# piljoong-jeong/nerf_meets_mlx

Measured on AMD Instinct MI355X. Metric: train+render rays/sec on Lego 800x800 (synthetic), coarse+fine 64+128, higher is better.
Workload: dtype split16 (fp16x2 render / bf16x2 train MFMA operands ~ 22 / 16 significand bits; fp32 accumulate)

## Files before the change

### include/nerf_hip.h

```cpp
#ifndef NERF_HIP_H
#define NERF_HIP_H

#include <stddef.h>
#include <stdint.h>

#ifdef __cplusplus
extern "C" {
#endif

#define NERF_ABI_VERSION 3

#define NERF_OK 0
#define NERF_E_NULL (-1)
#define NERF_E_SHAPE (-2)
#define NERF_E_UNSUPPORTED (-3)
#define NERF_E_HIP (-4)
#define NERF_E_RCCL (-5)

int nerf_abi_version(void);
const char* nerf_last_error(void);

#define NERF_RAY_STRIDE 11

int nerf_pixel_permutation(int64_t* out_idx, int64_t n, int64_t domain, uint64_t seed, uint64_t offset,
// ... 26 lines not shown

int nerf_encode_freq(const float* x, int64_t M, int D, int n_freqs, int freq_mode, float* out, void* stream);

int nerf_encode_sinusoidal(const float* x, int64_t M, int D, int n_freqs, const float* freqs_host,
                           int include_input, float* out, void* stream);

int nerf_sh_encode(const float* dirs, int64_t M, int degree, float* out, void* stream);

int nerf_hashgrid_forward(const float* x, int64_t M, const float* tables, int L, int log2_T, int F,
                          const int* resolutions_host, float* out, void* stream);
int nerf_hashgrid_backward(const float* x, int64_t M, const float* d_out, int L, int log2_T, int F,
                           const int* resolutions_host, float* d_tables, void* stream);

int nerf_ngp_encode(const float* rays, const float* z, int64_t B, int n, const float* tables, int L, int log2_T,
                    int F, const int* resolutions_host, int sh_degree, float pos_scale, float pos_offset, float* x_out,
                    float* pts_out, void* stream);
int nerf_hashgrid_backward_rays(const float* rays, const float* z, int64_t B, int n, const float* d_out, int L,
                                int log2_T, int F, const int* resolutions_host, float pos_scale, float pos_offset,
                                float* d_tables, void* stream);

int nerf_hashgrid_backward_ex(const float* x, int64_t M, const float* d_out, int L, int log2_T, int F,
                              const int* resolutions_host, int level_lo, int level_hi, int fixed_point, void* d_tables,
                              void* stream);
int nerf_hashgrid_backward_rays_ex(const float* rays, const float* z, int64_t B, int n, const float* d_out, int L,
                                   int log2_T, int F, const int* resolutions_host, float pos_scale, float pos_offset,
                                   int level_lo, int level_hi, int fixed_point, void* d_tables, void* stream);

int nerf_hashgrid_forward_lw(const float* x, int64_t M, const float* tables, int L, int log2_T, int F,
                             const int* resolutions_host, const float* level_weights_host, float* out, void* stream);
int nerf_ngp_encode_lw(const float* rays, const float* z, int64_t B, int n, const float* tables, int L, int log2_T,
                       int F, const int* resolutions_host, const float* level_weights_host, int sh_degree,
                       float pos_scale, float pos_offset, float* x_out, float* pts_out, void* stream);
int nerf_hashgrid_backward_ex_lw(const float* x, int64_t M, const float* d_out, int L, int log2_T, int F,
                                 const int* resolutions_host, const float* level_weights_host, int level_lo,
                                 int level_hi, int fixed_point, void* d_tables, void* stream);
int nerf_hashgrid_backward_rays_ex_lw(const float* rays, const float* z, int64_t B, int n, const float* d_out, int L,
                                      int log2_T, int F, const int* resolutions_host, const float* level_weights_host,
                                      float pos_scale, float pos_offset, int level_lo, int level_hi, int fixed_point,
                                      void* d_tables, void* stream);

int nerf_composite_forward(const float* raw, const float* z, const float* rays, int64_t B, int n,
                           float raw_noise_std, const float* noise, int white_bkgd, float* rgb, float* disp,
                           float* acc, float* weights, float* depth, void* stream);

int nerf_composite_backward(const float* raw, const float* z, const float* rays, int64_t B, int n,
                            float raw_noise_std, const float* noise, int white_bkgd, const float* d_rgb,
                            const float* d_acc, const float* d_depth, float* d_raw, void* stream);

int nerf_mse_loss_grad(const float* pred, const float* target, int64_t count, float grad_scale, float* loss_out,
                       float* d_pred, void* stream);

int nerf_composite_mse_backward(const float* raw, const float* z, const float* rays, int64_t B, int n, int white_bkgd,
                                const float* target, float grad_scale, float* loss_out, float* rgb, float* d_raw,
                                void* stream);

int nerf_ssim_sums(const float* pred, const float* gt, int N, int C, int H, int W, const float* window_host,
                   int w_size, float c1, float c2, double* sums, void* stream);

typedef struct nerf_mlp_arch {
  int n_layers;
  int width;
  int in_pos;
  int in_dir;
  int skip_layer;
  int use_viewdirs;
  int out_ch;
  int precision;
} nerf_mlp_arch;

int64_t nerf_mlp_param_count(const nerf_mlp_arch* arch);
int64_t nerf_mlp_packed_bytes(const nerf_mlp_arch* arch);
int nerf_mlp_pack(const nerf_mlp_arch* arch, const float* params, void* packed, void* stream);

int64_t nerf_mlp_acts_bytes(const nerf_mlp_arch* arch, int64_t M);
int64_t nerf_mlp_dz_bytes(const nerf_mlp_arch* arch, int64_t M);

int nerf_mlp_forward(const nerf_mlp_arch* arch, const void* packed, const float* x, int64_t M, float* out,
                     void* stream);
int nerf_mlp_forward_train(const nerf_mlp_arch* arch, const void* packed, const float* x, int64_t M, float* out,
                           void* acts, void* stream);

int nerf_query_fused(const nerf_mlp_arch* arch, const void* packed, const float* rays, const float* z, int64_t B,
                     int n, int freq_mode, float* raw, void* acts, void* stream);

int nerf_mlp_backward(const nerf_mlp_arch* arch, const void* packed, const void* acts, const float* d_raw,
                      int64_t M, void* dz, float* grads, void* stream);
int nerf_mlp_backward_inputs(const nerf_mlp_arch* arch, const void* packed, const void* acts, const float* d_raw,
                             int64_t M, void* dz, float* grads, float* d_x, void* stream);

int nerf_mlp_debug_width(const nerf_mlp_arch* arch, int kind, int layer);
int nerf_mlp_debug_read(const nerf_mlp_arch* arch, const void* store, int kind, int layer, int64_t M, float* out,
                        void* stream);

int nerf_ngp_query_fused(const nerf_mlp_arch* arch, const void* packed, const float* rays, const float* z, int64_t B,
                         int n, const float* tables, int L, int log2_T, int F, const int* resolutions_host,
                         int sh_degree, float pos_scale, float pos_offset, float* raw, void* acts, void* stream);
int nerf_ngp_query_fused_h(const nerf_mlp_arch* arch, const void* packed, const float* rays, const float* z, int64_t B,
                           int n, const float* tables, const void* tables_half, int L, int log2_T, int F,
                           const int* resolutions_host, int sh_degree, float pos_scale, float pos_offset, float* raw,
                           void* acts, void* stream);
int nerf_ngp_query_fused_lw(const nerf_mlp_arch* arch, const void* packed, const float* rays, const float* z, int64_t B,
                            int n, const float* tables, const void* tables_half, int L, int log2_T, int F,
                            const int* resolutions_host, const float* level_weights_host, int sh_degree, float pos_scale,
                            float pos_offset, float* raw, void* acts, void* stream);


int nerf_occ_points(int log2_res, int64_t cell0, int64_t count, uint64_t seed, uint64_t update, float pos_scale,
                    float pos_offset, float* rays_out, float* z_out, void* stream);
int nerf_occ_merge(float* density, const float* raw, int64_t count, float decay, void* stream);
int64_t nerf_occ_finalize_workspace_bytes(int log2_res);
int nerf_occ_finalize(const float* density, int log2_res, float thr_cap, void* workspace, float* thr_out, uint32_t* bits,
                      void* stream);
int64_t nerf_occ_cull_workspace_bytes(int64_t B, int n);
int nerf_occ_cull(const float* rays, const float* z, int64_t B, int n, const uint32_t* bits, int log2_res, float pos_scale,
                  float pos_offset, void* workspace, int64_t* idx_out, int64_t* count_out, float* rays_out, float* z_out,
                  float* raw_fill, void* stream);
int nerf_scatter_rows(const float* src, const int64_t* idx, int64_t n, int channels, float* dst, int64_t n_dst, void* stream);

#define NERF_MARCH_MAX_STEPS 1024
int64_t nerf_occ_march_workspace_bytes(int64_t B);
int nerf_occ_march_count(const float* rays, int64_t B, const float* jitter, float jitter_const, const uint32_t* bits, int log2_res,
                         float pos_scale, float pos_offset, float step_world, int march_steps, void* workspace, int64_t* offsets,
                         void* stream);
int nerf_occ_march_write(const float* rays, int64_t B, const float* jitter, float jitter_const, const uint32_t* bits, int log2_res,
                         float pos_scale, float pos_offset, float step_world, int march_steps, void* workspace, int64_t* offsets,
                         float* rows_out, float* z_out, void* stream);
#define NERF_OCC_RELU 0
#define NERF_OCC_EXP 1
int nerf_occ_merge_ex(float* density, const float* raw, int64_t count, float decay, int activation, void* stream);

int nerf_composite_packed_forward(const float* raw, const float* z, const int64_t* offsets, int64_t B, int64_t K, float step_world,
                                  int white_bkgd, float* rgb, float* acc, float* depth, void* stream);
int nerf_composite_packed_mse_backward(const float* raw, const int64_t* offsets, int64_t B, int64_t K, float step_world,
                                       int white_bkgd, const float* target, float grad_scale, float* loss_out, float* rgb,
                                       float* d_raw, void* stream);

int nerf_composite_packed_distortion(const float* raw, const float* z, const int64_t* offsets, const float* rays, int64_t B,
                                     int64_t K, float step_world, int march_steps, int white_bkgd, float* rgb, float* acc,
                                     float* depth, float* dist, void* stream);
int nerf_composite_packed_mse_dist_backward(const float* raw, const float* z, const int64_t* offsets, const float* rays, int64_t B,
                                            int64_t K, float step_world, int march_steps, int white_bkgd, const float* target,
                                            float grad_scale, float dist_weight, float* loss_out, float* dist_out, float* rgb,
                                            float* d_raw, void* stream);

int nerf_composite_packed_forward_bg(const float* raw, const float* z, const int64_t* offsets, int64_t B, int64_t K, float step_world,
                                     const float* bg, int bg_stride, float* rgb, float* acc, float* depth, void* stream);
int nerf_composite_packed_distortion_bg(const float* raw, const float* z, const int64_t* offsets, const float* rays, int64_t B,
                                        int64_t K, float step_world, int march_steps, const float* bg, int bg_stride, float* rgb,
                                        float* acc, float* depth, float* dist, void* stream);
int nerf_composite_packed_mse_backward_bg(const float* raw, const int64_t* offsets, int64_t B, int64_t K, float step_world,
                                          const float* target_rgba, const float* bg, float grad_scale, float* loss_out, float* rgb,
                                          float* d_raw, void* stream);
int nerf_composite_packed_mse_dist_backward_bg(const float* raw, const float* z, const int64_t* offsets, const float* rays, int64_t B,
                                               int64_t K, float step_world, int march_steps, const float* target_rgba,
                                               const float* bg, float grad_scale, float dist_weight, float* loss_out,
                                               float* dist_out, float* rgb, float* d_raw, void* stream);

#define NERF_ERT_TERMINATED 1
int64_t nerf_ert_march_workspace_bytes(int64_t B);
int nerf_ert_init(int64_t B, int32_t* istate, float* fstate, int32_t* live, void* stream);
int nerf_ert_march_count(const float* rays, int64_t B, const float* jitter, float jitter_const, const uint32_t* bits, int log2_res,
                         float pos_scale, float pos_offset, float step_world, int march_steps, const int32_t* live, int64_t A,
                         const int32_t* istate, int max_new, void* workspace, int64_t* totals, void* stream);
int nerf_ert_march_write(const float* rays, int64_t B, const float* jitter, float jitter_const, const uint32_t* bits, int log2_res,
                         float pos_scale, float pos_offset, float step_world, int march_steps, const int32_t* live, int64_t A,
                         int32_t* istate, int max_new, void* workspace, int64_t* offsets, int32_t* live_out, float* rows_out,
                         float* z_out, void* stream);
int nerf_ert_fold(const float* raw, const float* z, const int64_t* offsets, const int32_t* live, int64_t A, int64_t B, int64_t K,
                  float step_world, float min_transmittance, int32_t* istate, float* fstate, void* stream);
int nerf_ert_finish(const int32_t* istate, const float* fstate, int64_t B, int white_bkgd, float* rgb, float* acc, float* depth,
                    int32_t* samples, void* stream);
int nerf_ert_finish_bg(const int32_t* istate, const float* fstate, int64_t B, const float* bg, int bg_stride, float* rgb, float* acc,
                       float* depth, int32_t* samples, void* stream);

#define NERF_MESH_MAX_RES 512
int64_t nerf_mesh_workspace_bytes(int res);
int nerf_mesh_points(int res, const float* lo_host, const float* hi_host, int64_t p0, int64_t count, float* rays_out, float* z_out,
                     void* stream);
int nerf_mesh_count(const float* vol, int res, float iso, void* workspace, int64_t* totals, void* stream);
int nerf_mesh_write_vertices(const float* vol, int res, float iso, const float* lo_host, const float* hi_host, void* workspace,
                             int64_t V, float* verts, float* normals, float* color_rows, void* stream);
int nerf_mesh_write_faces(const float* vol, int res, float iso, void* workspace, int64_t F, int32_t* faces, void* stream);

int64_t nerf_ccl_workspace_bytes(int res);
int nerf_ccl_label(const float* vol, int res, float iso, void* workspace, int32_t* labels, void* stream);
int nerf_ccl_sizes(const int32_t* labels, int res, int32_t* sizes, int64_t* stats, void* stream);
int nerf_ccl_filter(const float* vol, const int32_t* labels, const int32_t* sizes, const int64_t* stats, int res, float iso,
                    int64_t min_voxels, int largest_only, float* out, void* stream);

#define NERF_MORPH_MAX_RADIUS 16
int64_t nerf_morph_workspace_bytes(int res);
int nerf_morph_erode(const float* vol, int res, float iso, int radius, void* workspace, float* core, int64_t* stats2, void* stream);
int nerf_morph_reconstruct(const float* vol, const float* kept, int res, float iso, int radius, void* workspace, float* out,
                           int64_t* stats2, void* stream);

#define NERF_TSDF_MAX_VIEWS 16
typedef struct nerf_tsdf_view {
  float c2w[12];
  float fx, fy, cx, cy;
} nerf_tsdf_view;
int nerf_tsdf_reset(float* D, float* Wt, uint8_t* flags, int res, void* stream);
int nerf_tsdf_integrate(float* D, float* Wt, uint8_t* flags, int res, const float* lo_host, const float* hi_host,
                        const nerf_tsdf_view* views_host, int n, int H, int W, const float* depth, const float* acc, float trunc,
                        float acc_min, float far, int carve, void* stream);
int nerf_tsdf_volume(const float* D, const float* Wt, const uint8_t* flags, int res, int min_views, float* vol_out, void* stream);

int64_t nerf_render_workspace_bytes(int64_t B, int n, int N);
int nerf_render_rays_fused(const nerf_mlp_arch* arch, const void* packed_coarse, const void* packed_fine,
                           const float* rays, int64_t B, int n, int N, const float* u, int freq_mode, int white_bkgd,
                           void* workspace, float* rgb, float* disp, float* acc, float* rgb_coarse, float* disp_coarse,
                           float* acc_coarse, float* z_vals, float* weights, void* stream);

#define NERF_COMM_ID_BYTES 128
int nerf_comm_unique_id(char* id_out_host);
int nerf_comm_init(void** comm_out, int nranks, int rank, const char* id_host);
int nerf_allreduce_grads(void* comm, float* grads, int64_t count, void* stream);
int nerf_comm_destroy(void* comm);

#define NERF_OPTION_UNKNOWN (-2147483647 - 1)
int nerf_set_option(const char* key, int value);
int nerf_get_option(const char* key);

int nerf_adam_step(float* params, const float* grads, float* m, float* v, int64_t count, float lr, float beta1,
                   float beta2, float eps, int bias_correction, int step, float grad_scale, void* stream);
int nerf_adam_step_ex(float* params, void* grads, float* m, float* v, int64_t count, float lr, float beta1, float beta2,
                      float eps, int bias_correction, int step, float grad_scale, int grads_fixed_point, int zero_grads,
                      void* stream);
int nerf_adam_step_shadow(float* params, void* grads, float* m, float* v, int64_t count, float lr, float beta1, float beta2,
                          float eps, int bias_correction, int step, float grad_scale, int grads_fixed_point, int zero_grads,
                          void* params_half, void* stream);

#ifdef __cplusplus
}
#endif
#endif
```

### nerf_meets_mlx_amd/_native.py

```python
import ctypes as C
import os

import torch

_HERE = os.path.dirname(os.path.abspath(__file__))
LIB_PATH = os.environ.get("NERF_HIP_LIB", os.path.join(_HERE, "libnerf_hip.so"))

_P, _I64, _I, _F, _U64 = C.c_void_p, C.c_int64, C.c_int, C.c_float, C.c_uint64
SIGNATURES = {
    "nerf_abi_version": (_I, []),
    "nerf_last_error": (C.c_char_p, []),
    "nerf_pixel_permutation": (_I, [_P, _I64, _I64, _U64, _U64, _P]),
    "nerf_ray_gen": (_I, [_P, _I64, _I, _I, C.POINTER(C.c_double), C.POINTER(C.c_float), _F, _F, _P, _P, _P]),
    "nerf_sample_batch": (_I, [_I64, _I, _I, _U64, _U64, C.POINTER(C.c_double), C.POINTER(C.c_float), _F, _F, _P, _P, _P, _P, _P]),
    "nerf_sample_batch_rgba": (_I, [_I64, _I, _I, _U64, _U64, C.POINTER(C.c_double), C.POINTER(C.c_float), _F, _F, _P, _P, _P, _P, _P]),
    "nerf_gather_rows": (_I, [_P, _I64, _P, _I64, _I, _P, _P]),
    "nerf_ndc_rays": (_I, [_P, _I64, _I, _I, _F, _F, _P]),
    "nerf_sample_coarse": (_I, [_P, _I64, _I, _I, _F, _P, _P, _P]),
    "nerf_add_noise_z": (_I, [_P, _P, _I64, _I, _F, _P, _P]),
    "nerf_importance_sample": (_I, [_P, _P, _P, _I64, _I, _I, _F, _P, _P, _P, _P, _P]),
    "nerf_encode_freq": (_I, [_P, _I64, _I, _I, _I, _P, _P]),
    "nerf_encode_sinusoidal": (_I, [_P, _I64, _I, _I, C.POINTER(C.c_float), _I, _P, _P]),
    "nerf_sh_encode": (_I, [_P, _I64, _I, _P, _P]),
    "nerf_hashgrid_forward": (_I, [_P, _I64, _P, _I, _I, _I, C.POINTER(C.c_int), _P, _P]),
    "nerf_hashgrid_backward": (_I, [_P, _I64, _P, _I, _I, _I, C.POINTER(C.c_int), _P, _P]),
    "nerf_ngp_encode": (_I, [_P, _P, _I64, _I, _P, _I, _I, _I, C.POINTER(C.c_int), _I, C.c_float, C.c_float, _P, _P, _P]),
    "nerf_ngp_query_fused": (_I, [_P, _P, _P, _P, _I64, _I, _P, _I, _I, _I, C.POINTER(C.c_int), _I, C.c_float, C.c_float, _P, _P, _P]),
    "nerf_ngp_query_fused_h": (_I, [_P, _P, _P, _P, _I64, _I, _P, _P, _I, _I, _I, C.POINTER(C.c_int), _I, C.c_float, C.c_float, _P, _P, _P]),
    "nerf_hashgrid_backward_rays": (_I, [_P, _P, _I64, _I, _P, _I, _I, _I, C.POINTER(C.c_int), C.c_float, C.c_float, _P, _P]),
    "nerf_hashgrid_backward_ex": (_I, [_P, _I64, _P, _I, _I, _I, C.POINTER(C.c_int), _I, _I, _I, _P, _P]),
    "nerf_hashgrid_backward_rays_ex": (_I, [_P, _P, _I64, _I, _P, _I, _I, _I, C.POINTER(C.c_int), C.c_float, C.c_float, _I, _I, _I, _P, _P]),
    "nerf_hashgrid_forward_lw": (_I, [_P, _I64, _P, _I, _I, _I, C.POINTER(C.c_int), C.POINTER(C.c_float), _P, _P]),
    "nerf_ngp_encode_lw": (_I, [_P, _P, _I64, _I, _P, _I, _I, _I, C.POINTER(C.c_int), C.POINTER(C.c_float), _I, C.c_float, C.c_float, _P, _P, _P]),
    "nerf_ngp_query_fused_lw": (_I, [_P, _P, _P, _P, _I64, _I, _P, _P, _I, _I, _I, C.POINTER(C.c_int), C.POINTER(C.c_float), _I, C.c_float, C.c_float, _P, _P, _P]),
    "nerf_hashgrid_backward_ex_lw": (_I, [_P, _I64, _P, _I, _I, _I, C.POINTER(C.c_int), C.POINTER(C.c_float), _I, _I, _I, _P, _P]),
    "nerf_hashgrid_backward_rays_ex_lw": (_I, [_P, _P, _I64, _I, _P, _I, _I, _I, C.POINTER(C.c_int), C.POINTER(C.c_float), C.c_float, C.c_float, _I, _I, _I, _P, _P]),
    "nerf_composite_forward": (_I, [_P, _P, _P, _I64, _I, _F, _P, _I, _P, _P, _P, _P, _P, _P]),
    "nerf_composite_backward": (_I, [_P, _P, _P, _I64, _I, _F, _P, _I, _P, _P, _P, _P, _P]),
    "nerf_mse_loss_grad": (_I, [_P, _P, _I64, _F, _P, _P, _P]),
    "nerf_composite_mse_backward": (_I, [_P, _P, _P, _I64, _I, _I, _P, _F, _P, _P, _P, _P]),
    "nerf_ssim_sums": (_I, [_P, _P, _I, _I, _I, _I, C.POINTER(C.c_float), _I, _F, _F, _P, _P]),
    "nerf_mlp_param_count": (_I64, [_P]),
    "nerf_mlp_packed_bytes": (_I64, [_P]),
    "nerf_mlp_pack": (_I, [_P, _P, _P, _P]),
    "nerf_mlp_acts_bytes": (_I64, [_P, _I64]),
    "nerf_mlp_dz_bytes": (_I64, [_P, _I64]),
    "nerf_mlp_forward": (_I, [_P, _P, _P, _I64, _P, _P]),
    "nerf_mlp_forward_train": (_I, [_P, _P, _P, _I64, _P, _P, _P]),
    "nerf_query_fused": (_I, [_P, _P, _P, _P, _I64, _I, _I, _P, _P, _P]),
    "nerf_mlp_backward": (_I, [_P, _P, _P, _P, _I64, _P, _P, _P]),
    "nerf_mlp_backward_inputs": (_I, [_P, _P, _P, _P, _I64, _P, _P, _P, _P]),
    "nerf_mlp_debug_width": (_I, [_P, _I, _I]),
    "nerf_mlp_debug_read": (_I, [_P, _P, _I, _I, _I64, _P, _P]),
    "nerf_render_workspace_bytes": (_I64, [_I64, _I, _I]),
    "nerf_render_rays_fused": (_I, [_P, _P, _P, _P, _I64, _I, _I, _P, _I, _I, _P, _P, _P, _P, _P, _P, _P, _P, _P, _P]),
    "nerf_comm_unique_id": (_I, [C.c_char_p]),
    "nerf_comm_init": (_I, [C.POINTER(C.c_void_p), _I, _I, C.c_char_p]),
    "nerf_allreduce_grads": (_I, [_P, _P, _I64, _P]),
    "nerf_comm_destroy": (_I, [_P]),
    "nerf_set_option": (_I, [C.c_char_p, _I]),
    "nerf_get_option": (_I, [C.c_char_p]),
    "nerf_adam_step": (_I, [_P, _P, _P, _P, _I64, _F, _F, _F, _F, _I, _I, _F, _P]),
    "nerf_adam_step_ex": (_I, [_P, _P, _P, _P, _I64, _F, _F, _F, _F, _I, _I, _F, _I, _I, _P]),
    "nerf_adam_step_shadow": (_I, [_P, _P, _P, _P, _I64, _F, _F, _F, _F, _I, _I, _F, _I, _I, _P, _P]),
    "nerf_occ_points": (_I, [_I, _I64, _I64, _U64, _U64, _F, _F, _P, _P, _P]),
    "nerf_occ_merge": (_I, [_P, _P, _I64, _F, _P]),
    "nerf_occ_finalize_workspace_bytes": (_I64, [_I]),
    "nerf_occ_finalize": (_I, [_P, _I, _F, _P, _P, _P, _P]),
    "nerf_occ_cull_workspace_bytes": (_I64, [_I64, _I]),
    "nerf_occ_cull": (_I, [_P, _P, _I64, _I, _P, _I, _F, _F, _P, _P, _P, _P, _P, _P, _P]),
    "nerf_scatter_rows": (_I, [_P, _P, _I64, _I, _P, _I64, _P]),
    "nerf_occ_merge_ex": (_I, [_P, _P, _I64, _F, _I, _P]),
    "nerf_occ_march_workspace_bytes": (_I64, [_I64]),
    "nerf_occ_march_count": (_I, [_P, _I64, _P, _F, _P, _I, _F, _F, _F, _I, _P, _P, _P]),
    "nerf_occ_march_write": (_I, [_P, _I64, _P, _F, _P, _I, _F, _F, _F, _I, _P, _P, _P, _P, _P]),
    "nerf_composite_packed_forward": (_I, [_P, _P, _P, _I64, _I64, _F, _I, _P, _P, _P, _P]),
    "nerf_composite_packed_mse_backward": (_I, [_P, _P, _I64, _I64, _F, _I, _P, _F, _P, _P, _P, _P]),
    "nerf_composite_packed_distortion": (_I, [_P, _P, _P, _P, _I64, _I64, _F, _I, _I, _P, _P, _P, _P, _P]),
    "nerf_composite_packed_mse_dist_backward": (_I, [_P, _P, _P, _P, _I64, _I64, _F, _I, _I, _P, _F, _F, _P, _P, _P, _P, _P]),
    "nerf_composite_packed_forward_bg": (_I, [_P, _P, _P, _I64, _I64, _F, _P, _I, _P, _P, _P, _P]),
    "nerf_composite_packed_distortion_bg": (_I, [_P, _P, _P, _P, _I64, _I64, _F, _I, _P, _I, _P, _P, _P, _P, _P]),
    "nerf_composite_packed_mse_backward_bg": (_I, [_P, _P, _I64, _I64, _F, _P, _P, _F, _P, _P, _P, _P]),
    "nerf_composite_packed_mse_dist_backward_bg": (_I, [_P, _P, _P, _P, _I64, _I64, _F, _I, _P, _P, _F, _F, _P, _P, _P, _P, _P]),
    "nerf_ert_march_workspace_bytes": (_I64, [_I64]),
    "nerf_ert_init": (_I, [_I64, _P, _P, _P, _P]),
    "nerf_ert_march_count": (_I, [_P, _I64, _P, _F, _P, _I, _F, _F, _F, _I, _P, _I64, _P, _I, _P, _P, _P]),
    "nerf_ert_march_write": (_I, [_P, _I64, _P, _F, _P, _I, _F, _F, _F, _I, _P, _I64, _P, _I, _P, _P, _P, _P, _P, _P]),
    "nerf_ert_fold": (_I, [_P, _P, _P, _P, _I64, _I64, _I64, _F, _F, _P, _P, _P]),
    "nerf_ert_finish": (_I, [_P, _P, _I64, _I, _P, _P, _P, _P, _P]),
    "nerf_ert_finish_bg": (_I, [_P, _P, _I64, _P, _I, _P, _P, _P, _P, _P]),
    "nerf_mesh_workspace_bytes": (_I64, [_I]),
    "nerf_mesh_points": (_I, [_I, C.POINTER(C.c_float), C.POINTER(C.c_float), _I64, _I64, _P, _P, _P]),
    "nerf_mesh_count": (_I, [_P, _I, _F, _P, _P, _P]),
    "nerf_mesh_write_vertices": (_I, [_P, _I, _F, C.POINTER(C.c_float), C.POINTER(C.c_float), _P, _I64, _P, _P, _P, _P]),
    "nerf_mesh_write_faces": (_I, [_P, _I, _F, _P, _I64, _P, _P]),
    "nerf_ccl_workspace_bytes": (_I64, [_I]),
    "nerf_ccl_label": (_I, [_P, _I, _F, _P, _P, _P]),
    "nerf_ccl_sizes": (_I, [_P, _I, _P, _P, _P]),
    "nerf_ccl_filter": (_I, [_P, _P, _P, _P, _I, _F, _I64, _I, _P, _P]),
    "nerf_morph_workspace_bytes": (_I64, [_I]),
    "nerf_morph_erode": (_I, [_P, _I, _F, _I, _P, _P, _P, _P]),
    "nerf_morph_reconstruct": (_I, [_P, _P, _I, _F, _I, _P, _P, _P, _P]),
    "nerf_tsdf_reset": (_I, [_P, _P, _P, _I, _P]),
    "nerf_tsdf_integrate": (_I, [_P, _P, _P, _I, C.POINTER(C.c_float), C.POINTER(C.c_float), C.POINTER(C.c_float), _I, _I, _I, _P, _P,
                                _F, _F, _F, _I, _P]),
    "nerf_tsdf_volume": (_I, [_P, _P, _P, _I, _I, _P, _P]),
}


class MlpArch(C.Structure):
    _fields_ = [("n_layers", _I), ("width", _I), ("in_pos", _I), ("in_dir", _I), ("skip_layer", _I),
                ("use_viewdirs", _I), ("out_ch", _I), ("precision", _I)]


class NerfHipError(RuntimeError):
    pass


_lib = None


def lib():
    global _lib
    if _lib is None:
        if not os.path.exists(LIB_PATH):
            raise NerfHipError(
                f"{LIB_PATH} not found: build it with `python -c 'import __graft_entry__ as g; g.build()'` "
                "(hipcc --offload-arch=gfx950).  There is no CPU fallback.")
        L = C.CDLL(LIB_PATH)
        for name, (res, args) in SIGNATURES.items():
            fn = getattr(L, name)
            fn.restype, fn.argtypes = res, args
        _lib = L
    return _lib


def check(rc: int):
    if rc != 0:
# ... 27 lines not shown
```

### nerf_meets_mlx_amd/csrc/mlp.hip

```cpp
#include "common.h"
#include "mlp_ring.h"
#include "mlp_layout.h"
#include "mlp_frag.h"
#include "mlp_arch2.h"
#include "hash_common.h"
#include "mlp_params.h"
#include "mlp32.h"
#include "mlp22.h"
#include "mlp_s16.h"
#include "mlp_s16x.h"
#include <string.h>
#include <mutex>
#include <unordered_map>


namespace nerf {

extern int g_hash_combine_max_res;




constexpr int PACK_THREADS = (L::F_TOTAL + L::B_PADDED) * 64 + L::BI_TOTAL;
__device__ __forceinline__ void pack_part(int tid, const float* __restrict__ p, bf16x8* __restrict__ wf,
// ... 1299 lines not shown
      f32x16 acc;
      acc_init_bias(acc, ws, LN::BI_RGB, h);
#pragma unroll
      for (int ks = 0; ks < 2; ++ks) acc = __builtin_amdgcn_mfma_f32_32x32x16_bf16(ws.frag(LN::F_RGB + ks, lane), hd[0][ks], acc, 0, 0, 0);
      if (h == 0 && valid) {
        float4 o; o.x = acc[0]; o.y = acc[1]; o.z = acc[2]; o.w = alpha;
        *reinterpret_cast<float4*>(a.out + m * 4) = poison_raw(o, bad);
      }
    }
#undef SINK
#undef MASK_STORE
  }
}

__global__ void __launch_bounds__(512) mlp_small_bwd_kernel(SmallArgs a) {
  constexpr int ST = 1;
  lds_load_stream(a.wb, nullptr);
  const int lane0 = threadIdx.x & 63, wv = threadIdx.x >> 6;
  const int64_t ntiles = (a.M + 31) >> 5;
  LdsW ws;
  for (int64_t tile0 = (int64_t)blockIdx.x * 8 + wv; tile0 < ntiles; tile0 += (int64_t)gridDim.x * 8) {
    int lane = lane0;
    asm volatile("" : "+v"(lane));
    const int r = lane & 31, h = lane >> 5;
    const int64_t m = tile0 * 32 + r;
    float4 g = make_float4(0.f, 0.f, 0.f, 0.f);
    if (m < a.M && h == 0) g = *reinterpret_cast<const float4*>(a.d_raw + m * 4);
    bf16x8 zrgb[ST][1], zal[ST][1];
#pragma unroll
    for (int j = 0; j < 8; ++j) { zrgb[0][0][j] = (__bf16)0.0f; zal[0][0][j] = (__bf16)0.0f; }
    zrgb[0][0][0] = (__bf16)g.x; zrgb[0][0][1] = (__bf16)g.y; zrgb[0][0][2] = (__bf16)g.z;
    zal[0][0][0] = (__bf16)g.w;
    u32x4 mk[3][ST];
#pragma unroll
    for (int l = 0; l < 3; ++l)
      mk[l][0] = *reinterpret_cast<const u32x4*>(frag_ptr(const_cast<void*>(a.acts), tile0, a.astride, LN::A_MASK + l, r, h));
    store_frags<1>(a.dz, tile0, a.zstride, LN::Z_RGB, zrgb[0], r, h);
    store_frags<1>(a.dz, tile0, a.zstride, LN::Z_A, zal[0], r, h);
#define ZSINK(slot0) FragSink<true>{a.dz, tile0, a.zstride, slot0, r, h}
    bf16x8 zd[ST][2], zf[ST][4], z1[ST][4], z0[ST][4];
    layer_bwd<ST, 1, 1, true>(ws, LN::B_RGB, zrgb, zd, mk[2], lane, ZSINK(LN::Z_D));
    layer_bwd<ST, 2, 2, false>(ws, LN::B_DIR, zd, zf, mk[2], lane, ZSINK(LN::Z_F));
    {
      bf16x8 cat[ST][5];
#pragma unroll
      for (int k = 0; k < 4; ++k) cat[0][k] = zf[0][k];
      cat[0][4] = zal[0][0];
      layer_bwd<ST, 5, 2, true>(ws, LN::B_FA, cat, z1, mk[1], lane, ZSINK(LN::Z_L1));
    }
    layer_bwd<ST, 4, 2, true>(ws, LN::B_L1, z1, z0, mk[0], lane, ZSINK(LN::Z_L0));
#undef ZSINK
    if (a.d_x) {
      f32x16 acc;
#pragma unroll
      for (int i = 0; i < 16; ++i) acc[i] = 0.0f;
#pragma unroll
      for (int ns = 0; ns < 4; ++ns) acc = __builtin_amdgcn_mfma_f32_32x32x16_bf16(ws.frag(LN::B_L0 + ns, lane), z0[0][ns], acc, 0, 0, 0);
      if (m < a.M) {
#pragma unroll
        for (int q = 0; q < 4; ++q) {
          float4 o; o.x = acc[4 * q]; o.y = acc[4 * q + 1]; o.z = acc[4 * q + 2]; o.w = acc[4 * q + 3];
          *reinterpret_cast<float4*>(a.d_x + m * LN::CPOS + 8 * q + 4 * h) = o;
        }
      }
    }
  }
}

static int g_dw_wgs = 0;
static int g_dw_bias = -1;
static int g_bwd_stage = 0;
static int g_dw_ring_cap = 8;
static int g_dw_private = 4;
static int g_dw16_variant = 1;
static int g_dw_narrow_first = 1;
static int g_dw_job_mask = 0;
static int g_tile_pad16 = 0;
static inline int64_t astride16() { return (int64_t)L::A_SLOTS * 64 + g_tile_pad16; }
static inline int64_t zstride16() { return (int64_t)L::Z_SLOTS * 64 + g_tile_pad16; }
static int g_mlp_variant = 0;
static int g_ring_wgs = 0;
static int g_ngp_ray_major = 1;
int g_pass_queue = 1;
static int g_ring_split = 1;
static inline int arch_prec(const nerf_mlp_arch* a) { return a->precision == 32 ? 32 : a->precision == 22 ? 22 : 16; }
static inline bool arch_f32(const nerf_mlp_arch* a) { return a->precision == 32; }
static inline bool arch_s16(const nerf_mlp_arch* a) { return a->precision == 22; }
constexpr int MAX_DEVICES = 64;
static int cur_device() {
  int d = 0;
  if (hipGetDevice(&d) != hipSuccess || d < 0 || d >= MAX_DEVICES) d = 0;
  return d;
}
static int cu_count() {
  static int n[MAX_DEVICES] = {};
  const int dev = cur_device();
  if (n[dev] == 0) {
    int v = 0;
    n[dev] = (hipDeviceGetAttribute(&v, hipDeviceAttributeMultiprocessorCount, dev) == hipSuccess && v > 0) ? v : 256;
  }
  return n[dev];
}
static inline int ring_wgs() { return g_ring_wgs > 0 ? g_ring_wgs : cu_count(); }

template <class K>
static void ensure_lds(K kernel, int bytes) {
  (void)hipFuncSetAttribute(reinterpret_cast<const void*>(kernel), hipFuncAttributeMaxDynamicSharedMemorySize, bytes);
}

static int arch_kind(const nerf_mlp_arch* a) {
  if (!a) return -1;
  if (a->precision != 0 && a->precision != 16 && a->precision != 32 && a->precision != 22) return -1;
  if (arch_f32(a) && !(a->n_layers == 8 && a->width == 256)) return -1;
  if (a->n_layers == 2 && a->width == 64 && a->skip_layer < 0 && a->use_viewdirs == 1 && a->in_pos == 32 && a->in_dir == 16) return 2;
  if (a->n_layers != 8 || a->width != 256 || a->skip_layer != 4) return -1;
  if (a->use_viewdirs == 1 && a->in_pos == 63 && a->in_dir == 27) return 0;
  if (a->use_viewdirs == 0 && a->in_pos == 40 && a->out_ch >= 1 && a->out_ch <= 4) return 1;
  return -1;
}
static bool arch_ok(const nerf_mlp_arch* a) { return arch_kind(a) == 0; }
static inline int64_t img_astride16(bool split = false) { return (int64_t)(split ? s16x::IMG_A_SLOTS : LI::A_SLOTS) * 64 + g_tile_pad16; }
static inline int64_t img_zstride16(bool split = false) { return (int64_t)(split ? s16x::IMG_Z_SLOTS : LI::Z_SLOTS) * 64 + g_tile_pad16; }
static inline int64_t img_params(const nerf_mlp_arch* a) { return LI::P_WO + (int64_t)a->out_ch * 257; }
static inline int64_t small_astride16(bool split = false) { return (int64_t)(split ? s16x::SM_A_SLOTS : LN::A_SLOTS) * 64 + g_tile_pad16; }
static inline int64_t small_zstride16(bool split = false) { return (int64_t)(split ? s16x::SM_Z_SLOTS : LN::Z_SLOTS) * 64 + g_tile_pad16; }
constexpr int64_t IMG_BF16_BYTES = (int64_t)(LI::F_TOTAL + LI::B_PADDED) * 1024 + LI::BI_TOTAL * 4;
static inline const float* img_bias_of(const void* packed) {
  return reinterpret_cast<const float*>(static_cast<const char*>(packed) + (size_t)(LI::F_TOTAL + LI::B_PADDED) * 1024);
}
static inline const float* small_bias_of(const void* packed) {
  return reinterpret_cast<const float*>(static_cast<const char*>(packed) + (size_t)(LN::F_PADDED + LN::B_PADDED) * 1024);
}

}

using namespace nerf;

extern "C" int nerf_set_option(const char* key, int value) {
  NERF_REQUIRE(key, NERF_E_NULL, "nerf_set_option: key is NULL");
  if (!strcmp(key, "mlp_variant")) { g_mlp_variant = value; return NERF_OK; }
  if (!strcmp(key, "ring_split")) {
    NERF_REQUIRE(value == 1 || value == 2, NERF_E_UNSUPPORTED, "nerf_set_option: ring_split must be 1 or 2");
    g_ring_split = value;
    return NERF_OK;
  }
  NERF_REQUIRE(strcmp(key, "mlp_precision") != 0, NERF_E_UNSUPPORTED,
               "nerf_set_option: \"mlp_precision\" is gone (ABI 3): set nerf_mlp_arch.precision of the model instead");
  if (!strcmp(key, "ring_workgroups")) { g_ring_wgs = value > 0 ? value : 0; return NERF_OK; }
  if (!strcmp(key, "tile_pad16")) { g_tile_pad16 = value >= 0 ? value : 0; return NERF_OK; }
  if (!strcmp(key, "dw_workgroups")) { g_dw_wgs = value > 0 ? value : 0; return NERF_OK; }
  if (!strcmp(key, "dw_unit_bias")) { g_dw_bias = value >= 0 ? value : -1; return NERF_OK; }
  if (!strcmp(key, "bwd_stage")) { g_bwd_stage = value; return NERF_OK; }
  if (!strcmp(key, "dw_job_mask")) { g_dw_job_mask = value; return NERF_OK; }
  if (!strcmp(key, "hash_combine_max_res")) { g_hash_combine_max_res = value > 0 ? value : 0; return NERF_OK; }
  if (!strcmp(key, "ngp_ray_major")) { g_ngp_ray_major = value ? 1 : 0; return NERF_OK; }
  if (!strcmp(key, "dw22_variant")) { s16::g_dw_variant = value == 0 ? 0 : 1; return NERF_OK; }
  if (!strcmp(key, "dw16_variant")) { g_dw16_variant = value < 0 ? 0 : value > 3 ? 3 : value; return NERF_OK; }
  if (!strcmp(key, "dw_private_tiles")) { g_dw_private = value < 0 ? 0 : value > 4 ? 4 : value; return NERF_OK; }
  if (!strcmp(key, "dw_ring_cap")) { g_dw_ring_cap = value < 2 ? 2 : value > 16 ? 16 : value; return NERF_OK; }
  if (!strcmp(key, "pass_queue")) { g_pass_queue = value ? 1 : 0; return NERF_OK; }
  if (!strcmp(key, "dw_narrow_first")) { g_dw_narrow_first = value ? 1 : 0; return NERF_OK; }
  if (!strcmp(key, "f22_tiles")) {
    NERF_REQUIRE(value == 0 || value == 2 || value == 3, NERF_E_UNSUPPORTED, "nerf_set_option: f22_tiles must be 0 (automatic), 2 or 3");
    f22::g_tiles = value;
    return NERF_OK;
  }
  return fail(NERF_E_UNSUPPORTED, "nerf_set_option: unknown key '%s'", key);
}

extern "C" int nerf_get_option(const char* key) {
  if (!key) return NERF_OPTION_UNKNOWN;
  if (!strcmp(key, "mlp_variant")) return g_mlp_variant;
  if (!strcmp(key, "ring_workgroups")) return g_ring_wgs;
  if (!strcmp(key, "ring_split")) return g_ring_split;
  if (!strcmp(key, "dw_workgroups")) return g_dw_wgs;
  if (!strcmp(key, "hash_combine_max_res")) return g_hash_combine_max_res;
  if (!strcmp(key, "ngp_ray_major")) return g_ngp_ray_major;
  if (!strcmp(key, "dw22_variant")) return s16::g_dw_variant;
  if (!strcmp(key, "dw16_variant")) return g_dw16_variant;
  if (!strcmp(key, "tile_pad16")) return g_tile_pad16;
  if (!strcmp(key, "dw_unit_bias")) return g_dw_bias;
  if (!strcmp(key, "bwd_stage")) return g_bwd_stage;
  if (!strcmp(key, "dw_job_mask")) return g_dw_job_mask;
  if (!strcmp(key, "dw_private_tiles")) return g_dw_private;
  if (!strcmp(key, "dw_ring_cap")) return g_dw_ring_cap;
  if (!strcmp(key, "pass_queue")) return g_pass_queue;
  if (!strcmp(key, "dw_narrow_first")) return g_dw_narrow_first;
  if (!strcmp(key, "f22_tiles")) return f22::g_tiles;
  return NERF_OPTION_UNKNOWN;
}

extern "C" int64_t nerf_mlp_param_count(const nerf_mlp_arch* arch) {
  const int k = arch_kind(arch);
  return k == 0 ? L::P_TOTAL : k == 1 ? img_params(arch) : k == 2 ? LN::P_TOTAL : -1;
}
extern "C" int64_t nerf_mlp_packed_bytes(const nerf_mlp_arch* arch) {
  const int k = arch_kind(arch);
  return k == 0 ? L::PACKED_BYTES + (arch_f32(arch) ? f32::PACKED_BYTES : 0) + (arch_s16(arch) ? f22::PACKED_BYTES + s16::PACKED_BYTES : 0)
         : k == 1 ? IMG_BF16_BYTES + (arch_s16(arch) ? s16x::IMG_PACKED_BYTES : 0) + (arch_f32(arch) ? f32::PACKED_BYTES : 0)
         : k == 2 ? LN::PACKED_BYTES + (arch_s16(arch) ? s16x::SM_PACKED_BYTES : 0) : -1;
}
static inline const void* packed32_of(const void* packed) { return static_cast<const char*>(packed) + L::PACKED_BYTES; }
static inline const void* packed22_of(const void* packed) { return static_cast<const char*>(packed) + L::PACKED_BYTES; }
static inline const void* packed_s16_of(const void* packed) { return static_cast<const char*>(packed) + L::PACKED_BYTES + f22::PACKED_BYTES; }
static inline const float* bias_slots_of(const void* packed) {
  return reinterpret_cast<const float*>(static_cast<const char*>(packed) + (size_t)(L::F_TOTAL + L::B_PADDED) * 1024);
}
static inline int64_t s16_astride16() { return (int64_t)s16::A_SLOTS * 64 + g_tile_pad16; }
static inline int64_t s16_zstride16() { return (int64_t)s16::Z_SLOTS * 64 + g_tile_pad16; }
static inline int64_t padded_tiles(int64_t M) { return (((M + 31) / 32) + 7) / 8 * 8; }
extern "C" int64_t nerf_mlp_acts_bytes(const nerf_mlp_arch* arch, int64_t M) {
  const int k = arch_kind(arch);
  if (k < 0 || M < 0) return -1;
  const bool sp = arch_s16(arch);
  const int64_t b16 = padded_tiles(M) * (k == 0 ? astride16() : k == 1 ? img_astride16(sp) : small_astride16(sp)) * 16;
  if (k == 0 && arch_s16(arch)) return padded_tiles(M) * s16_astride16() * 16;
  return (k <= 1 && arch_f32(arch)) ? f32::acts_bytes(M) : b16;
}
extern "C" int64_t nerf_mlp_dz_bytes(const nerf_mlp_arch* arch, int64_t M) {
  const int k = arch_kind(arch);
  if (k < 0 || M < 0) return -1;
  const bool sp = arch_s16(arch);
  const int64_t b16 = padded_tiles(M) * (k == 0 ? zstride16() : k == 1 ? img_zstride16(sp) : small_zstride16(sp)) * 16
                      + DW_PARTIAL_BYTES;
  if (k == 0 && arch_s16(arch)) return padded_tiles(M) * s16_zstride16() * 16 + DW_PARTIAL_BYTES;
  return (k <= 1 && arch_f32(arch)) ? f32::dz_bytes(M) : b16;
}

#define NERF_ARCH_MSG ": HIP kernels exist for (8x256, skip 4) with in=63+27 view head, or in=40 / no view head / out_ch<=4, and for (2x64, no skip) with in=32+16 view head"
#define NERF_ARCH_CHECK(who) NERF_REQUIRE(arch_ok(arch), NERF_E_UNSUPPORTED, who NERF_ARCH_MSG)
#define NERF_ARCH_CHECK_ANY(who) NERF_REQUIRE(arch_kind(arch) >= 0, NERF_E_UNSUPPORTED, who NERF_ARCH_MSG)

extern "C" int nerf_mlp_pack(const nerf_mlp_arch* arch, const float* params, void* packed, void* stream) {
  NERF_ARCH_CHECK_ANY("nerf_mlp_pack");
  NERF_REQUIRE(params && packed, NERF_E_NULL, "nerf_mlp_pack: params/packed is NULL");
  char* base = static_cast<char*>(packed);
  if (arch_kind(arch) == 2) {
    const int tot = (LN::F_PADDED + LN::B_PADDED) * 64 + LN::BI_TOTAL;
    hipLaunchKernelGGL(pack_small_kernel, dim3((tot + 255) / 256), dim3(256), 0, as_stream(stream), params,
                       reinterpret_cast<bf16x8*>(base), reinterpret_cast<bf16x8*>(base + (size_t)LN::F_PADDED * 1024),
                       reinterpret_cast<float*>(base + (size_t)(LN::F_PADDED + LN::B_PADDED) * 1024));
    int rcn = check_launch("nerf_mlp_pack (2x64 model)");
    if (!rcn && arch_s16(arch)) rcn = s16x::small_pack(params, base + LN::PACKED_BYTES, as_stream(stream));
    return rcn;
  }
  if (arch_kind(arch) == 1) {
    bf16x8* wfi = reinterpret_cast<bf16x8*>(base);
    bf16x8* wbi = reinterpret_cast<bf16x8*>(base + (size_t)LI::F_TOTAL * 1024);
    float* bi = reinterpret_cast<float*>(base + (size_t)(LI::F_TOTAL + LI::B_PADDED) * 1024);
    const int tot = (LI::F_TOTAL + LI::B_PADDED) * 64 + LI::BI_TOTAL;
    hipLaunchKernelGGL(pack_img_kernel, dim3((tot + 255) / 256), dim3(256), 0, as_stream(stream), params, wfi, wbi, bi,
                       arch->out_ch);
    int rci = check_launch("nerf_mlp_pack (image model)");
    if (!rci && arch_s16(arch)) rci = s16x::img_pack(params, arch->out_ch, base + IMG_BF16_BYTES, as_stream(stream));
    if (!rci && arch_f32(arch)) rci = f32::pack(params, base + IMG_BF16_BYTES, arch->out_ch, as_stream(stream));
    return rci;
  }
  bf16x8* wf = reinterpret_cast<bf16x8*>(base);
  bf16x8* wb = reinterpret_cast<bf16x8*>(base + (size_t)L::F_TOTAL * 1024);
  float* bias = reinterpret_cast<float*>(base + (size_t)(L::F_TOTAL + L::B_PADDED) * 1024);
  hipLaunchKernelGGL(pack_kernel, dim3(PACK_BLOCKS + PACK16_BLOCKS), dim3(256), 0, as_stream(stream), params, wf, wb, bias,
                     reinterpret_cast<bf16x8*>(base + L::F16_OFFSET));
  int rc = check_launch("nerf_mlp_pack");
  if (rc) return rc;
  if (arch_f32(arch)) rc = f32::pack(params, base + L::PACKED_BYTES, 0, as_stream(stream));
  if (!rc && arch_s16(arch)) rc = f22::pack(params, base + L::PACKED_BYTES, as_stream(stream));
  if (!rc && arch_s16(arch)) rc = s16::pack(params, base + L::PACKED_BYTES + f22::PACKED_BYTES, as_stream(stream));
  return rc;
}

static void fill_freqs(PeFreq& fr, int mode) {
  for (int k = 0; k < 10; ++k) fr.pos[k] = mode == 0 ? (float)(k * k) : (float)(1 << k);
  for (int k = 0; k < 4; ++k) fr.dir[k] = mode == 0 ? (float)(k * k) : (float)(1 << k);
}

template <int MODE>
static int launch_fwd(const void* packed, const float* x, const float* rays, const float* z, int64_t M, int n,
                      int freq_mode, float* out, void* acts, void* stream) {
  FwdArgs a;
  a.queue = nullptr;
  const char* base = static_cast<const char*>(packed);
  a.wf = reinterpret_cast<const bf16x8*>(base);
  a.bias = reinterpret_cast<const float*>(base + (size_t)(L::F_TOTAL + L::B_PADDED) * 1024);
  a.x = x; a.rays = rays; a.z = z; a.M = M; a.n = n; a.out = out; a.acts = acts; a.astride = astride16();
  fill_freqs(a.fr, freq_mode);
  const int64_t ntiles = (M + 31) / 32;
  auto s = as_stream(stream);
  const int variant = (g_mlp_variant == 0) ? (MODE == 1 ? (acts ? 3 : 4) : 1) : g_mlp_variant;
  if ((variant == 4 || variant == 5) && MODE == 1 && !acts) {
    const int64_t nsuper = (M + 255) / 256;
    const dim3 g((unsigned)(nsuper < ring_wgs() ? nsuper : ring_wgs()));
    static DevOnce once16;
    once16.run([&] { ensure_lds(mlp_fwd_ring16_kernel<8, 2>, RING16_LDS_BYTES); ensure_lds(mlp_fwd_ring16_kernel<4, 4>, RING16_LDS_BYTES); });
    FwdArgs a16 = a;
    a16.queue = passq_slot();
    a16.wf = reinterpret_cast<const bf16x8*>(base + L::F16_OFFSET);
    if (variant == 4) hipLaunchKernelGGL((mlp_fwd_ring16_kernel<8, 2>), g, dim3(512), RING16_LDS_BYTES, s, a16);
    else hipLaunchKernelGGL((mlp_fwd_ring16_kernel<4, 4>), g, dim3(256), RING16_LDS_BYTES, s, a16);
    return check_launch("mlp forward (ring, 16x16x32)");
  }
  if (variant >= 3 && MODE == 1) {
    a.queue = passq_slot();
    if (acts && g_ring_split == 2) {
      const int64_t nsuper = (ntiles + SPLIT_NW - 1) / SPLIT_NW;
      const int64_t wgs = 2 * (int64_t)ring_wgs();
      static DevOnce once2;
      once2.run([&] { ensure_lds(mlp_fwd_ring_kernel<1, true, SPLIT_NW, SPLIT_CHUNK>, SPLIT_LDS_BYTES); });
      hipLaunchKernelGGL((mlp_fwd_ring_kernel<1, true, SPLIT_NW, SPLIT_CHUNK>), dim3((unsigned)(nsuper < wgs ? nsuper : wgs)),
                         dim3(64 * SPLIT_NW), SPLIT_LDS_BYTES, s, a);
      return check_launch("mlp forward (ring, 2 workgroups per CU)");
    }
    const int64_t nsuper = (ntiles + 7) / 8;
    const dim3 g((unsigned)(nsuper < ring_wgs() ? nsuper : ring_wgs())), b(512);
    static DevOnce once;
    once.run([&] { ensure_lds(mlp_fwd_ring_kernel<1, true>, RING_LDS_BYTES); ensure_lds(mlp_fwd_ring_kernel<1, false>, RING_LDS_BYTES); });
    if (acts) hipLaunchKernelGGL((mlp_fwd_ring_kernel<1, true>), g, b, RING_LDS_BYTES, s, a);
    else hipLaunchKernelGGL((mlp_fwd_ring_kernel<1, false>), g, b, RING_LDS_BYTES, s, a);
    return check_launch("mlp forward (ring)");
  }
  const int st = variant == 2 ? 2 : 1;
  const int64_t blocks = (ntiles + 4 * st - 1) / (4 * st);
  NERF_REQUIRE(blocks < (1ll << 31), NERF_E_SHAPE, "mlp forward: M too large");
  const dim3 g((unsigned)blocks), b(256);
  if (st == 1) {
    if (acts) hipLaunchKernelGGL((mlp_fwd_kernel<1, MODE, true>), g, b, 0, s, a);
    else hipLaunchKernelGGL((mlp_fwd_kernel<1, MODE, false>), g, b, 0, s, a);
  } else {
    if (acts) hipLaunchKernelGGL((mlp_fwd_kernel<2, MODE, true>), g, b, 0, s, a);
    else hipLaunchKernelGGL((mlp_fwd_kernel<2, MODE, false>), g, b, 0, s, a);
  }
  return check_launch("mlp forward");
}

static void img_args(ImgArgs& a, const nerf_mlp_arch* arch, const void* packed) {
  const char* base = static_cast<const char*>(packed);
  a.wf = reinterpret_cast<const bf16x8*>(base);
  a.wb = reinterpret_cast<const bf16x8*>(base + (size_t)LI::F_TOTAL * 1024);
  a.bias = reinterpret_cast<const float*>(base + (size_t)(LI::F_TOTAL + LI::B_PADDED) * 1024);
  a.out_ch = arch->out_ch; a.astride = img_astride16(); a.zstride = img_zstride16();
  a.x = nullptr; a.d_out = nullptr; a.out = nullptr; a.acts = nullptr; a.dz = nullptr; a.M = 0;
}

static void small_args(SmallArgs& a, const void* packed) {
  const char* base = static_cast<const char*>(packed);
  a.wf = reinterpret_cast<const bf16x8*>(base);
  a.wb = reinterpret_cast<const bf16x8*>(base + (size_t)LN::F_PADDED * 1024);
  a.bias = reinterpret_cast<const float*>(base + (size_t)(LN::F_PADDED + LN::B_PADDED) * 1024);
  a.x = nullptr; a.d_raw = nullptr; a.out = nullptr; a.d_x = nullptr; a.acts = nullptr; a.dz = nullptr; a.M = 0;
  a.astride = small_astride16(); a.zstride = small_zstride16();
  a.rays = nullptr; a.z = nullptr; a.n = 1; a.tables = nullptr; a.tables_h = nullptr; a.T = 0; a.pos_scale = 1.0f; a.pos_offset = 0.0f;
  a.ray_major = 0; a.B = 0;
  for (int l = 0; l < 32; ++l) a.lw.w[l] = 1.0f;
}

extern "C" int nerf_mlp_forward_train(const nerf_mlp_arch* arch, const void* packed, const float* x, int64_t M,
                                      float* out, void* acts, void* stream) {
  NERF_ARCH_CHECK_ANY("nerf_mlp_forward");
  if (M <= 0) return NERF_OK;
  NERF_REQUIRE(packed && x && out, NERF_E_NULL, "nerf_mlp_forward: NULL pointer");
  if (arch_kind(arch) == 2) {
    SmallArgs a;
    small_args(a, packed);
    if (arch_s16(arch))
      return s16x::small_forward(static_cast<const char*>(packed) + LN::PACKED_BYTES, small_bias_of(packed), x, M, out, acts,
                                 small_astride16(true), nullptr, as_stream(stream));
    a.x = x; a.out = out; a.acts = acts; a.M = M;
    const int64_t nwg = ((M + 31) / 32 + 7) / 8;
    const dim3 g((unsigned)(nwg < 2048 ? nwg : 2048)), b(512);
    if (acts) hipLaunchKernelGGL((mlp_small_fwd_kernel<true, false>), g, b, LN::LDS_BYTES, as_stream(stream), a);
    else hipLaunchKernelGGL((mlp_small_fwd_kernel<false, false>), g, b, LN::LDS_BYTES, as_stream(stream), a);
    return check_launch("mlp forward (2x64 model)");
  }
  if (arch_kind(arch) == 1) {
    if (arch_f32(arch))
      return f32::forward(static_cast<const char*>(packed) + IMG_BF16_BYTES, x, nullptr, nullptr, M, 1, 0, out, acts, arch->out_ch,
                          as_stream(stream));
    if (arch_s16(arch))
      return s16x::img_forward(static_cast<const char*>(packed) + IMG_BF16_BYTES, img_bias_of(packed), x, M, arch->out_ch, out, acts,
                               img_astride16(true), ring_wgs(), as_stream(stream));
    ImgArgs a;
    img_args(a, arch, packed);
    a.x = x; a.out = out; a.acts = acts; a.M = M;
    const int64_t nsuper = ((M + 31) / 32 + 7) / 8;
    static DevOnce once;
    once.run([&] { ensure_lds(mlp_img_fwd_ring_kernel<true>, RING_LDS_BYTES); ensure_lds(mlp_img_fwd_ring_kernel<false>, RING_LDS_BYTES); });
    const dim3 g((unsigned)(nsuper < ring_wgs() ? nsuper : ring_wgs())), b(512);
    if (acts) hipLaunchKernelGGL(mlp_img_fwd_ring_kernel<true>, g, b, RING_LDS_BYTES, as_stream(stream), a);
    else hipLaunchKernelGGL(mlp_img_fwd_ring_kernel<false>, g, b, RING_LDS_BYTES, as_stream(stream), a);
    return check_launch("mlp forward (image model)");
  }
  if (arch_s16(arch) && !acts)
    return f22::forward(packed22_of(packed), x, nullptr, nullptr, M, 1, 0, out, ring_wgs(), as_stream(stream));
  if (arch_s16(arch))
    return s16::forward(packed_s16_of(packed), bias_slots_of(packed), x, nullptr, nullptr, M, 1, 0, out, acts, s16_astride16(),
                        ring_wgs(), as_stream(stream));
  if (arch_f32(arch)) {
    return f32::forward(packed32_of(packed), x, nullptr, nullptr, M, 1, 0, out, acts, 0, as_stream(stream));
  }
  return launch_fwd<0>(packed, x, nullptr, nullptr, M, 1, 0, out, acts, stream);
}

extern "C" int nerf_mlp_forward(const nerf_mlp_arch* arch, const void* packed, const float* x, int64_t M, float* out,
                                void* stream) {
  return nerf_mlp_forward_train(arch, packed, x, M, out, nullptr, stream);
}

extern "C" int nerf_query_fused(const nerf_mlp_arch* arch, const void* packed, const float* rays, const float* z,
                                int64_t B, int n, int freq_mode, float* raw, void* acts, void* stream) {
  NERF_ARCH_CHECK("nerf_query_fused");
  NERF_REQUIRE(n >= 1, NERF_E_SHAPE, "nerf_query_fused: n must be >= 1");
  if (B <= 0) return NERF_OK;
  NERF_REQUIRE(packed && rays && z && raw, NERF_E_NULL, "nerf_query_fused: NULL pointer");
  NERF_REQUIRE(freq_mode == 0 || freq_mode == 1, NERF_E_UNSUPPORTED, "nerf_query_fused: freq_mode must be 0 or 1");
  NERF_REQUIRE(B * (int64_t)n < (1ll << 31), NERF_E_SHAPE, "nerf_query_fused: B*n must be < 2^31 samples per call");
  if (arch_s16(arch) && !acts)
    return f22::forward(packed22_of(packed), nullptr, rays, z, B * n, n, freq_mode, raw, ring_wgs(), as_stream(stream));
  if (arch_s16(arch))
    return s16::forward(packed_s16_of(packed), bias_slots_of(packed), nullptr, rays, z, B * n, n, freq_mode, raw, acts,
                        s16_astride16(), ring_wgs(), as_stream(stream));
  if (arch_f32(arch)) {
    return f32::forward(packed32_of(packed), nullptr, rays, z, B * n, n, freq_mode, raw, acts, 0, as_stream(stream));
  }
  return launch_fwd<1>(packed, nullptr, rays, z, B * n, n, freq_mode, raw, acts, stream);
}

static int launch_dw_part(DwArgs& d, int nj, int64_t ntiles, int64_t nparams, const void* acts, void* dz, int64_t astride,
                          int64_t zstride, float* grads, hipStream_t s, int kind, int a_lo, int z_lo, int slot_base, int max_wgs) {
  const bool split_bf16 = kind == 1 || kind == 2;
  int64_t units[DW_MAX_JOBS], total_units = 0;
  for (int j = 0; j < nj; ++j) {
    units[j] = d.jobs[j].nf + d.jobs[j].kf + (g_dw_bias >= 0 ? g_dw_bias : split_bf16 ? 2 : 128);
    total_units += units[j];
  }
  int target_wgs = g_dw_wgs > 0 ? g_dw_wgs : cu_count();
  if (target_wgs > max_wgs) target_wgs = max_wgs;
  const int64_t max_splits = (ntiles + 3) / 4;
  int nw = 0;
  double frac[DW_MAX_JOBS];
  for (int j = 0; j < DW_MAX_JOBS; ++j) d.splits[j] = 0;
  for (int j = 0; j < nj; ++j) {
    const double share = (double)units[j] * target_wgs / (double)total_units;
    int64_t sp = (int64_t)share;
    frac[j] = share - (double)sp;
    if (sp < 1) { sp = 1; frac[j] = 0.0; }
    if (sp > max_splits) { sp = max_splits; frac[j] = 0.0; }
    d.splits[j] = (int)sp;
    nw += (int)sp;
  }
  while (nw < target_wgs) {
    int best = -1;
    for (int j = 0; j < nj; ++j)
      if (d.splits[j] < max_splits && (best < 0 || frac[j] > frac[best])) best = j;
    if (best < 0 || frac[best] <= 0.0) break;
    d.splits[best] += 1; frac[best] = 0.0; nw += 1;
  }
  while (nw > target_wgs) {
    int big = 0;
    for (int j = 1; j < nj; ++j) if (d.splits[j] > d.splits[big]) big = j;
    if (d.splits[big] <= 1) break;
    d.splits[big] -= 1; nw -= 1;
  }
  NERF_REQUIRE(slot_base + nw <= DW_MAX_WGS, NERF_E_SHAPE, "nerf_mlp_backward: dw_workgroups must be <= %d", DW_MAX_WGS);
  bool all_tiny = true;
  for (int j = 0; j < nj; ++j) all_tiny = all_tiny && ((d.jobs[j].nf + 1) / 2) * ((d.jobs[j].kf + 1) / 2) <= 4;
  d.ntiles = (int)ntiles; d.astride = astride; d.zstride = zstride;
  d.acts = acts; d.dz = dz; d.grads = grads;
  d.a_lo = a_lo; d.z_lo = z_lo; d.ring_cap = g_dw_ring_cap; d.private_max_tiles = g_dw_private;
  d.partial = reinterpret_cast<float*>(static_cast<char*>(dz) + padded_tiles(ntiles * 32) * zstride * 16) + (size_t)slot_base * DW_SLOT_FLOATS;
  int rc;
  if (kind >= 2) {
    rc = launch_dw_wide_kernel(d, nw, kind == 2, s);
  } else if (kind == 1) {
    rc = s16::launch_dw_kernel(d, nw, true, s);
  } else if (g_dw16_variant == 3 || (g_dw16_variant == 1 && all_tiny)) {
    rc = s16::launch_dw_kernel(d, nw, false, s);
  } else {
    static DevOnce lds_attr_set;
    lds_attr_set.run([&] { (void)hipFuncSetAttribute(reinterpret_cast<const void*>(mlp_dw_kernel), hipFuncAttributeMaxDynamicSharedMemorySize, DW_LDS_BYTES); });
    hipLaunchKernelGGL(mlp_dw_kernel, dim3(nw), dim3(64 * DW_WAVES), DW_LDS_BYTES, s, d);
    rc = check_launch("mlp dW");
  }
  if (rc) return rc;
  hipLaunchKernelGGL(mlp_dw_reduce_kernel, dim3(257, nj), dim3(256), 0, s, d);
  return check_launch("mlp dW reduce");
}

static int launch_dw(DwArgs& d, int nj, int64_t ntiles, int64_t nparams, const void* acts, void* dz, int64_t astride,
                     int64_t zstride, float* grads, hipStream_t s, bool split_bf16 = false, int a_lo = 0, int z_lo = 0) {
  if (g_dw_job_mask) {
    hipError_t e = hipMemsetAsync(grads, 0, sizeof(float) * nparams, s);
    if (e != hipSuccess) return fail(NERF_E_HIP, "nerf_mlp_backward: memset: %s", hipGetErrorString(e));
  }
  if ((split_bf16 ? s16::g_dw_variant : g_dw16_variant) == 0)
    return launch_dw_part(d, nj, ntiles, nparams, acts, dz, astride, zstride, grads, s, split_bf16 ? 1 : 0, a_lo, z_lo, 0, DW_MAX_WGS);
  DwArgs wide = d, rest = d;
  int nwide = 0, nrest = 0;
  for (int j = 0; j < nj; ++j) {
    if (d.jobs[j].nf == 16 && d.jobs[j].kf == 16) wide.jobs[nwide++] = d.jobs[j];
    else rest.jobs[nrest++] = d.jobs[j];
  }
  const int half = DW_MAX_WGS / 2;
  for (int turn = 0; turn < 2; ++turn) {
    const bool do_wide = (turn == 0) != (g_dw_narrow_first != 0);
    if (do_wide && nwide) {
      const int rc = launch_dw_part(wide, nwide, ntiles, nparams, acts, dz, astride, zstride, grads, s, split_bf16 ? 2 : 3, a_lo, z_lo, half, half);
      if (rc) return rc;
    }
    if (!do_wide && nrest) {
// ... 317 lines not shown
```

### nerf_meets_mlx_amd/csrc/mlp22.h

```cpp
#pragma once
#include <hip/hip_runtime.h>
#include <stdint.h>

namespace nerf {
namespace f22 {

constexpr int F_PAIRS = 1172, F_FRAGS = 2 * F_PAIRS, F_PADDED = 2368, BIAS_FLOATS = 2496;
constexpr int64_t PACKED_BYTES = (int64_t)F_PADDED * 1024 + (int64_t)BIAS_FLOATS * 4;

extern int g_tiles;
int pack(const float* params, void* packed22, hipStream_t s);
int forward(const void* packed22, const float* x, const float* rays, const float* z, int64_t M, int n, int freq_mode,
            float* out, int persistent_wgs, hipStream_t s);

}
}
```

### nerf_meets_mlx_amd/csrc/mlp22.hip

```cpp
#include "mlp_layout.h"
#include "mlp22.h"

#ifndef NERF_F22_SINF
#define NERF_F22_SINF 0
#endif

#ifndef NERF_F22_PIN
#define NERF_F22_PIN 1
#endif
#ifndef NERF_F22_AGPR
#define NERF_F22_AGPR 1
#endif
#ifndef NERF_F22_MIXSUB
#define NERF_F22_MIXSUB 1
#endif
#ifndef NERF_F22_RG3
#define NERF_F22_RG3 4
#endif
#ifndef NERF_F22_IGLP
#define NERF_F22_IGLP 0
#endif

namespace nerf {
namespace f22 {

typedef _Float16 h8 __attribute__((ext_vector_type(8)));
typedef _Float16 h2 __attribute__((ext_vector_type(2)));
typedef float f32x2 __attribute__((ext_vector_type(2)));
typedef unsigned int u32x4 __attribute__((ext_vector_type(4)));

constexpr float LO_SCALE = 2048.0f, LO_INV = 1.0f / 2048.0f;
constexpr float F16_MIN_NORMAL = 6.103515625e-05f;
constexpr int CHUNKS = F_PADDED / RING_CHUNK;
static_assert(CHUNKS * RING_CHUNK == F_PADDED && F_FRAGS % 4 == 0 && F_PAIRS == L::F16_TOTAL, "f22 stream layout");

struct HiLo { unsigned hi, lo; };
__device__ __forceinline__ HiLo split2(float v0, float v1) {
  const f32x2 v = {v0, v1};
  const h2 hh = __builtin_convertvector(v, h2);
#if NERF_F22_MIXSUB
  const f32x2 r = {__builtin_fmaf((float)hh[0], -LO_SCALE, v0 * LO_SCALE), __builtin_fmaf((float)hh[1], -LO_SCALE, v1 * LO_SCALE)};
#else
  const f32x2 r = {(v0 - (float)hh[0]) * LO_SCALE, (v1 - (float)hh[1]) * LO_SCALE};
#endif
  return HiLo{__builtin_bit_cast(unsigned, hh), __builtin_bit_cast(unsigned, __builtin_convertvector(r, h2))};
}

constexpr int PACK_THREADS = (F_PADDED / 2) * 64 + BIAS_FLOATS;
__global__ void __launch_bounds__(256) pack22_kernel(const float* __restrict__ p, u32x4* __restrict__ wf,
                                                     float* __restrict__ bias) {
  const int t = blockIdx.x * 256 + threadIdx.x;
  if (t < (F_PADDED / 2) * 64) {
    const int fp = t >> 6, lane = t & 63;
    u32x4 hi = {0u, 0u, 0u, 0u}, lo = {0u, 0u, 0u, 0u};
    if (fp < F_PAIRS) {
#pragma unroll
      for (int j = 0; j < 8; j += 2) {
        float w[2];
        _Float16 wh[2], wl[2];
#pragma unroll
        for (int e = 0; e < 2; ++e) {
          w[e] = fwd_src16(p, fp, lane & 15, lane >> 4, j + e);
          wh[e] = __builtin_fabsf(w[e]) < F16_MIN_NORMAL ? (_Float16)0.0f : (_Float16)w[e];
          wl[e] = (_Float16)((w[e] - (float)wh[e]) * LO_SCALE);
        }
        const h2 a = {wh[0], wh[1]}, b = {wl[0], wl[1]};
        hi[j >> 1] = __builtin_bit_cast(unsigned, a);
        lo[j >> 1] = __builtin_bit_cast(unsigned, b);
      }
    }
    wf[(2 * fp) * 64 + lane] = hi;
    wf[(2 * fp + 1) * 64 + lane] = lo;
  } else if (t < PACK_THREADS) {
    const int s = t - (F_PADDED / 2) * 64;
    float v = 0.0f;
    if (s < 2048) v = p[L::pb(s >> 8) + (s & 255)];
    else if (s < L::BI_ALPHA) v = p[L::P_BF + (s - L::BI_FEAT)];
    else if (s < L::BI_DIR) v = (s == L::BI_ALPHA) ? p[L::P_BA] : 0.0f;
    else if (s < L::BI_RGB) v = p[L::P_BD + (s - L::BI_DIR)];
    else v = (s - L::BI_RGB) < 3 ? p[L::P_BR + (s - L::BI_RGB)] : 0.0f;
    bias[s] = v;
  }
}

__device__ __forceinline__ float sin_acc(float x, float f, float ph) {
  const float a = x * f;
#if NERF_F22_SINF
  return ph != 0.0f ? cosf(a) : sinf(a);
#else
  const float k = __builtin_rintf(a * 0.15915494309189535f);
  float r = __builtin_fmaf(-k, 6.2831854820251465f, a);
  r = __builtin_fmaf(-k, -1.7484556000744487e-07f, r);
  return __builtin_amdgcn_sinf(__builtin_fmaf(r, 0.15915494309189535f, ph));
#endif
}

struct Pe22 { float fa, fb, fc, phc, fd; int g; };
__device__ __forceinline__ Pe22 pe22_setup(const PeFreq& fr, int g) {
  Pe22 q;
  q.fa = g == 0 ? fr.pos[0] : g == 1 ? fr.pos[2] : g == 2 ? fr.pos[4] : fr.pos[6];
  q.fb = g == 0 ? fr.pos[1] : g == 1 ? fr.pos[3] : g == 2 ? fr.pos[5] : fr.pos[7];
  q.fc = g < 2 ? fr.pos[8] : fr.pos[9];
  q.phc = (g & 1) ? 0.25f : 0.0f;
  q.fd = g == 0 ? fr.dir[0] : g == 1 ? fr.dir[1] : g == 2 ? fr.dir[2] : fr.dir[3];
  q.g = g;
  return q;
}

template <int COUNT>
__device__ __forceinline__ void split_slots(const float (&v)[COUNT], u32x4* hi, u32x4* lo) {
#pragma unroll
  for (int j = 0; j < COUNT; j += 2) {
    const HiLo q = split2(v[j], v[j + 1]);
    hi[j >> 3][(j & 7) >> 1] = q.hi; lo[j >> 3][(j & 7) >> 1] = q.lo;
  }
}

__device__ __forceinline__ void pe22_pos(const Pe22& q, const float (&p)[3], u32x4 (&peh)[2], u32x4 (&pel)[2]) {
  float v[16];
#pragma unroll
  for (int sl = 0; sl < 12; ++sl) v[sl] = sin_acc(p[sl % 3], sl < 6 ? q.fa : q.fb, (sl % 6) >= 3 ? 0.25f : 0.0f);
#pragma unroll
  for (int k = 0; k < 3; ++k) v[12 + k] = sin_acc(p[k], q.fc, q.phc);
  v[15] = q.g == 0 ? p[0] : q.g == 1 ? p[1] : q.g == 2 ? p[2] : 0.0f;
  split_slots<16>(v, peh, pel);
}
__device__ __forceinline__ void pe22_dir(const Pe22& q, const float (&d)[3], u32x4 (&dph)[1], u32x4 (&dpl)[1]) {
  float w[8];
#pragma unroll
  for (int j = 0; j < 6; ++j) w[j] = sin_acc(d[j % 3], q.fd, j >= 3 ? 0.25f : 0.0f);
  w[6] = q.g == 0 ? d[0] : q.g == 1 ? d[1] : q.g == 2 ? d[2] : 0.0f;
  w[7] = 0.0f;
  split_slots<8>(w, dph, dpl);
}
__device__ __forceinline__ void pe22_encode(const Pe22& q, const float (&p)[3], const float (&d)[3], u32x4 (&peh)[2],
                                            u32x4 (&pel)[2], u32x4 (&dph)[1], u32x4 (&dpl)[1]) {
  pe22_pos(q, p, peh, pel);
  pe22_dir(q, d, dph, dpl);
}
__device__ __forceinline__ void pe22_row(const float* __restrict__ row, int g, u32x4 (&peh)[2], u32x4 (&pel)[2],
                                         u32x4 (&dph)[1], u32x4 (&dpl)[1]) {
  float v[16], w[8];
#pragma unroll
  for (int sl = 0; sl < 16; ++sl) {
    const int ch = pos_chan16(sl >> 3, g, sl & 7);
    v[sl] = ch >= 0 ? row[ch] : 0.0f;
  }
#pragma unroll
  for (int j = 0; j < 8; ++j) {
    const int ch = dir_chan16(g, j);
    w[j] = ch >= 0 ? row[63 + ch] : 0.0f;
  }
  split_slots<16>(v, peh, pel);
  split_slots<8>(w, dph, dpl);
}

__device__ __forceinline__ f32x4 mfma16(const u32x4& a, const u32x4& b, const f32x4& c) {
#if NERF_ABLATE == 41 || NERF_ABLATE == 42
  return c;
#endif
  return __builtin_amdgcn_mfma_f32_16x16x32_f16(__builtin_bit_cast(h8, a), __builtin_bit_cast(h8, b), c, 0, 0, 0);
}

template <int NS, int KS, int NT, bool RELU, class WS, bool PARK_LDS = false>
__device__ __forceinline__ void layer22(WS& ws, int pbase, int bias_slot, const u32x4 (&ih)[NS][KS], const u32x4 (&il)[NS][KS],
                                        u32x4 (&oh)[NS][NT / 2], u32x4 (&ol)[NS][NT / 2], int lane, unsigned park_addr = 0u) {
  const int g = lane >> 4;
  f32x4 pm[NS], pc[NS];
  if (PARK_LDS) asm volatile("ds_write_b128 %0, %1" :: "v"(park_addr), "v"(il[NS - 1][KS - 1]) : "memory");
#if NERF_F22_IGLP >= 0
  __builtin_amdgcn_iglp_opt(NERF_F22_IGLP);
#endif
  constexpr int NP = 2 * NS;
  auto piece = [&](int nt, int pcs, f32x4 (&m)[NS], f32x4 (&c)[NS]) {
    const int s = pcs >> 1, i = 2 * (pcs & 1);
#if NERF_ABLATE == 41 || NERF_ABLATE == 42
    return;
#endif
#if NERF_F22_PIN
    if (pcs == 0) {
#pragma unroll
      for (int t = 0; t < NS; ++t) asm volatile("" : "+v"(m[t]), "+v"(c[t]));
    }
#endif
    float v0 = __builtin_fmaf(c[s][i], LO_INV, m[s][i]), v1 = __builtin_fmaf(c[s][i + 1], LO_INV, m[s][i + 1]);
    if (RELU) { v0 = __builtin_elementwise_maximum(v0, 0.0f); v1 = __builtin_elementwise_maximum(v1, 0.0f); }
    const HiLo q = split2(v0, v1);
    oh[s][nt >> 1][2 * (nt & 1) + (i >> 1)] = q.hi; ol[s][nt >> 1][2 * (nt & 1) + (i >> 1)] = q.lo;
#if NERF_F22_AGPR
    if ((nt & 1) && i == 2) asm volatile("" : "+a"(oh[s][nt >> 1]), "+a"(ol[s][nt >> 1]));
#endif
  };
  auto piece_at = [](int q) { return NS == 2 ? (KS >= 8 ? 1 + 2 * q : (q * KS) / 4) : (KS >= 8 ? 1 + (q * (KS - 1)) / NP : (q * KS) / NP); };
#pragma unroll
  for (int nt = 0; nt < NT; ++nt) {
    const float4 b = ws.bias4(bias_slot + 16 * nt + 4 * g);
    f32x4 m[NS], c[NS];
    m[0][0] = b.x; m[0][1] = b.y; m[0][2] = b.z; m[0][3] = b.w;
    c[0] = f32x4{0.0f, 0.0f, 0.0f, 0.0f};
#pragma unroll
    for (int t = 1; t < NS; ++t) { m[t] = m[0]; c[t] = c[0]; }
#pragma unroll
    for (int ks = 0; ks < KS; ++ks) {
      const int fp = pbase + nt * KS + ks;
      const u32x4 ah = __builtin_bit_cast(u32x4, next_frag(ws, 2 * fp, lane));
      const u32x4 al = __builtin_bit_cast(u32x4, next_frag(ws, 2 * fp + 1, lane));
      if (NS == 2) {
        m[0] = mfma16(ah, ih[0][ks], m[0]);
        c[0] = mfma16(ah, il[0][ks], c[0]);
        m[1] = mfma16(ah, ih[1][ks], m[1]);
        c[1] = mfma16(ah, il[1][ks], c[1]);
        c[0] = mfma16(al, ih[0][ks], c[0]);
        c[1] = mfma16(al, ih[1][ks], c[1]);
      } else {
#pragma unroll
        for (int t = 0; t < NS; ++t) {
          m[t] = mfma16(ah, ih[t][ks], m[t]);
          if (PARK_LDS && t == NS - 1 && ks == KS - 1) {
            u32x4 b;
            asm volatile("ds_read_b128 %0, %1\n\ts_waitcnt lgkmcnt(0)" : "=v"(b) : "v"(park_addr) : "memory");
            c[t] = mfma16(ah, b, c[t]);
          } else {
            c[t] = mfma16(ah, il[t][ks], c[t]);
          }
        }
#pragma unroll
        for (int t = 0; t < NS; ++t) c[t] = mfma16(al, ih[t][ks], c[t]);
      }
      if (nt > 0) {
#pragma unroll
        for (int q = 0; q < NP; ++q)
          if (piece_at(q) == ks) piece(nt - 1, q, pm, pc);
      }
    }
#pragma unroll
    for (int t = 0; t < NS; ++t) { pm[t] = m[t]; pc[t] = c[t]; }
  }
#pragma unroll
  for (int q = 0; q < NP; ++q) piece(NT - 1, q, pm, pc);
}

template <int NS, int KS, class WS>
__device__ __forceinline__ void head22(WS& ws, int pbase, int bias_slot, const u32x4 (&ih)[NS][KS], const u32x4 (&il)[NS][KS],
                                       f32x4 (&out)[NS], int lane) {
  const int g = lane >> 4;
  const float4 b = ws.bias4(bias_slot + 4 * g);
  f32x4 m[NS], c[NS];
  m[0][0] = b.x; m[0][1] = b.y; m[0][2] = b.z; m[0][3] = b.w;
  c[0] = f32x4{0.0f, 0.0f, 0.0f, 0.0f};
#pragma unroll
  for (int t = 1; t < NS; ++t) { m[t] = m[0]; c[t] = c[0]; }
#pragma unroll
  for (int ks = 0; ks < KS; ++ks) {
    const u32x4 ah = __builtin_bit_cast(u32x4, next_frag(ws, 2 * (pbase + ks), lane));
    const u32x4 al = __builtin_bit_cast(u32x4, next_frag(ws, 2 * (pbase + ks) + 1, lane));
    if (NS == 2) {
      m[0] = mfma16(ah, ih[0][ks], m[0]);
      c[0] = mfma16(ah, il[0][ks], c[0]);
      m[1] = mfma16(ah, ih[1][ks], m[1]);
      c[1] = mfma16(ah, il[1][ks], c[1]);
      c[0] = mfma16(al, ih[0][ks], c[0]);
      c[1] = mfma16(al, ih[1][ks], c[1]);
    } else {
#pragma unroll
      for (int t = 0; t < NS; ++t) { m[t] = mfma16(ah, ih[t][ks], m[t]); c[t] = mfma16(ah, il[t][ks], c[t]); }
#pragma unroll
      for (int t = 0; t < NS; ++t) c[t] = mfma16(al, ih[t][ks], c[t]);
    }
  }
#pragma unroll
  for (int s = 0; s < NS; ++s)
#pragma unroll
    for (int i = 0; i < 4; ++i) out[s][i] = __builtin_fmaf(c[s][i], LO_INV, m[s][i]);
}

constexpr int NW22 = 4, NW22_ = NW22;
constexpr int PARK_OFF = RING_LDS_BYTES;
template <int NS> constexpr int park_bytes() { return NS > 2 ? (6 * NS + 4) * 64 * NW22_ * 4 : 0; }
template <int K> __device__ __forceinline__ void lds_put(unsigned addr, float v) {
  asm volatile("ds_write_b32 %0, %1 offset:%2" :: "v"(addr), "v"(v), "i"(1024 * K) : "memory");
}
template <int K> __device__ __forceinline__ float lds_get(unsigned addr) {
  float v;
  asm volatile("ds_read_b32 %0, %1 offset:%2\n\ts_waitcnt lgkmcnt(0)" : "=v"(v) : "v"(addr), "i"(1024 * K) : "memory");
  return v;
}
template <int S> __device__ __forceinline__ void park_put(unsigned park, const float (&p)[3], const float (&d)[3]) {
  lds_put<6 * S + 0>(park, p[0]); lds_put<6 * S + 1>(park, p[1]); lds_put<6 * S + 2>(park, p[2]);
  lds_put<6 * S + 3>(park, d[0]); lds_put<6 * S + 4>(park, d[1]); lds_put<6 * S + 5>(park, d[2]);
}
template <int S, int OFF> __device__ __forceinline__ void park_get(unsigned park, float (&v)[3]) {
  v[0] = lds_get<6 * S + OFF>(park); v[1] = lds_get<6 * S + OFF + 1>(park); v[2] = lds_get<6 * S + OFF + 2>(park);
}
__device__ __forceinline__ void park_put_s(int s, unsigned park, const float (&p)[3], const float (&d)[3]) {
  if (s == 0) park_put<0>(park, p, d); else if (s == 1) park_put<1>(park, p, d); else park_put<2>(park, p, d);
}
template <int OFF> __device__ __forceinline__ void park_get_s(int s, unsigned park, float (&v)[3]) {
  if (s == 0) park_get<0, OFF>(park, v); else if (s == 1) park_get<1, OFF>(park, v); else park_get<2, OFF>(park, v);
}

template <int NS, int MODE, class WS>
__device__ __forceinline__ void tiles22(const FwdArgs& a, WS& ws, int64_t wtile0, int64_t nwtiles, int lane, PassQueue& pq) {
  constexpr bool RECOMP = NS > 2;
  static_assert(!RECOMP || MODE == 1, "the 48-sample form takes rays + depths");
  const int c = lane & 15, g = lane >> 4;
  u32x4 peh[NS][2], pel[NS][2], dph[NS][1], dpl[NS][1];
  const unsigned park = ws.lds0 + PARK_OFF + 4u * (unsigned)(ws.wv * 64 + lane);
  pq.ask(ws.wv, lane);
  const Pe22 q = pe22_setup(a.fr, g);
  {
    const int64_t wt = wtile0 < nwtiles ? wtile0 : nwtiles - 1;
#pragma unroll
    for (int s = 0; s < NS; ++s) {
      int64_t m = wt * (16 * NS) + 16 * s + c; if (m >= a.M) m = a.M - 1;
      if (MODE == 0) {
        pe22_row(a.x + m * 90, g, peh[s], pel[s], dph[s], dpl[s]);
      } else {
        const int64_t ray = (int64_t)((unsigned)m / (unsigned)a.n);
        const float* rr = a.rays + ray * NERF_RAY_STRIDE;
        float p[3], d[3];
#if NERF_ABLATE == 3
        (void)rr;
#pragma unroll
        for (int k = 0; k < 3; ++k) { p[k] = 0.001f * (float)(m & 1023) + (float)k; d[k] = 0.5f; }
#else
        const float zv = a.z[m];
#pragma unroll
        for (int k = 0; k < 3; ++k) { p[k] = rr[k] + zv * rr[3 + k]; d[k] = rr[8 + k]; }
#endif
        if (RECOMP) {
          park_put_s(s, park, p, d);
          pe22_pos(q, p, peh[s], pel[s]);
        } else {
          pe22_encode(q, p, d, peh[s], pel[s], dph[s], dpl[s]);
        }
      }
    }
  }
  pq.publish(ws.wv);
  u32x4 hah[NS][8], hal[NS][8], hbh[NS][8], hbl[NS][8];
  layer22<NS, 2, 16, true>(ws, L16::F_L0, 0, peh, pel, hah, hal, lane);
  layer22<NS, 8, 16, true>(ws, L16::F_L1 + 0 * 128, 256, hah, hal, hbh, hbl, lane);
  layer22<NS, 8, 16, true>(ws, L16::F_L1 + 1 * 128, 512, hbh, hbl, hah, hal, lane);
  layer22<NS, 8, 16, true>(ws, L16::F_L1 + 2 * 128, 768, hah, hal, hbh, hbl, lane);
  layer22<NS, 8, 16, true>(ws, L16::F_L1 + 3 * 128, 1024, hbh, hbl, hah, hal, lane);
  {
    u32x4 cth[NS][10], ctl[NS][10];
#pragma unroll
    for (int s = 0; s < NS; ++s) {
      if (RECOMP) {
        float pp[3];
        park_get_s<0>(s, park, pp);
        pe22_pos(q, pp, peh[s], pel[s]);
      }
      cth[s][0] = peh[s][0]; cth[s][1] = peh[s][1]; ctl[s][0] = pel[s][0]; ctl[s][1] = pel[s][1];
#pragma unroll
      for (int k = 0; k < 8; ++k) { cth[s][2 + k] = hah[s][k]; ctl[s][2 + k] = hal[s][k]; }
    }
    layer22<NS, 10, 16, true, WS, (NS > 2)>(ws, L16::F_L5, 1280, cth, ctl, hbh, hbl, lane,
                                            ws.lds0 + PARK_OFF + 6 * NS * 64 * NW22 * 4 + 16u * (unsigned)(ws.wv * 64 + lane));
  }
  layer22<NS, 8, 16, true>(ws, L16::F_L6, 1536, hbh, hbl, hah, hal, lane);
  layer22<NS, 8, 16, true>(ws, L16::F_L7, 1792, hah, hal, hbh, hbl, lane);
  layer22<NS, 8, 16, false>(ws, L16::F_FA, L::BI_FEAT, hbh, hbl, hah, hal, lane);
  f32x4 alpha[NS];
  head22<NS, 8>(ws, L16::F_FA + 128, L::BI_ALPHA, hbh, hbl, alpha, lane);
  u32x4 hdh[NS][4], hdl[NS][4];
  {
    u32x4 cth[NS][9], ctl[NS][9];
#pragma unroll
    for (int s = 0; s < NS; ++s) {
#pragma unroll
      for (int k = 0; k < 8; ++k) { cth[s][k] = hah[s][k]; ctl[s][k] = hal[s][k]; }
      if (RECOMP) {
        float dd[3];
        park_get_s<3>(s, park, dd);
        pe22_dir(q, dd, dph[s], dpl[s]);
      }
      cth[s][8] = dph[s][0]; ctl[s][8] = dpl[s][0];
    }
    layer22<NS, 9, 8, true>(ws, L16::F_DIR, L::BI_DIR, cth, ctl, hdh, hdl, lane);
  }
  f32x4 rgb[NS];
  head22<NS, 4>(ws, L16::F_RGB, L::BI_RGB, hdh, hdl, rgb, lane);
#pragma unroll
  for (int s = 0; s < NS; ++s) {
    const int64_t m = wtile0 * (16 * NS) + 16 * s + c;
    if (g == 0 && wtile0 < nwtiles && m < a.M) {
      float4 o; o.x = rgb[s][0]; o.y = rgb[s][1]; o.z = rgb[s][2]; o.w = alpha[s][0];
      *reinterpret_cast<float4*>(a.out + m * 4) = o;
    }
  }
}

template <int MODE, int NS = 2>
__global__ void __launch_bounds__(64 * NW22) mlp22_fwd_kernel(FwdArgs a) {
  const int lane = threadIdx.x & 63;
  const int wv = __builtin_amdgcn_readfirstlane(threadIdx.x >> 6);
  const int64_t nwtiles = (a.M + 16 * NS - 1) / (16 * NS), nsuper = (nwtiles + NW22 - 1) / NW22;
  NERF_STAMP2_DECL();
  RingW<CHUNKS, F_FRAGS, (NS > 2 ? NERF_F22_RG3 : 4), NW22, RING_CHUNK, RING_STAGES, true, true> ws;
  ws.wsrc = reinterpret_cast<const char*>(a.wf);
  ws.lane16 = 16 * lane;
  ws.lds0 = __builtin_amdgcn_readfirstlane(lds_addr_of(ring_smem));
  ws.wv = wv;
  ws.start(lane);
  ring_load_bias(a.bias, BIAS_FLOATS);
  __syncthreads();
  NERF_STAMP2_LOOP();
  PassQueue pq;
  pq.init(a.queue, ws.lds0 + RING_BIAS_OFF);
  for (int64_t sp = blockIdx.x; sp < nsuper;) {
    int ln = lane;
    asm volatile("" : "+v"(ln));
    ws.new_pass();
    tiles22<NS, MODE>(a, ws, sp * NW22 + wv, nwtiles, ln, pq);
    NERF_STAMP2_PASS();
    sp = pq.next(sp);
  }
  NERF_STAMP2_END();
  ws.drain();
  pq.leave();
}

int pack(const float* params, void* packed22, hipStream_t s) {
  char* base = static_cast<char*>(packed22);
  hipLaunchKernelGGL(pack22_kernel, dim3((PACK_THREADS + 255) / 256), dim3(256), 0, s, params,
                     reinterpret_cast<u32x4*>(base), reinterpret_cast<float*>(base + (size_t)F_PADDED * 1024));
  return check_launch("nerf_mlp_pack (split-fp16 image)");
}

int g_tiles = 0;

int forward(const void* packed22, const float* x, const float* rays, const float* z, int64_t M, int n, int freq_mode,
            float* out, int persistent_wgs, hipStream_t s) {
  FwdArgs a;
  a.queue = passq_slot();
  const char* base = static_cast<const char*>(packed22);
  a.wf = reinterpret_cast<const bf16x8*>(base);
  a.bias = reinterpret_cast<const float*>(base + (size_t)F_PADDED * 1024);
  a.x = x; a.rays = rays; a.z = z; a.M = M; a.n = n; a.out = out; a.acts = nullptr; a.astride = 0;
  for (int k = 0; k < 10; ++k) a.fr.pos[k] = freq_mode == 0 ? (float)(k * k) : (float)(1 << k);
  for (int k = 0; k < 4; ++k) a.fr.dir[k] = freq_mode == 0 ? (float)(k * k) : (float)(1 << k);
  int tiles = g_tiles;
  if (tiles == 0) {
    const int64_t w = persistent_wgs > 0 ? persistent_wgs : 1;
    const int64_t p2 = (((M + 31) / 32 + NW22 - 1) / NW22 + w - 1) / w, p3 = (((M + 47) / 48 + NW22 - 1) / NW22 + w - 1) / w;
    tiles = 100 * p2 < 141 * p3 ? 2 : 3;
  }
  const int mode = x ? 0 : (tiles == 3 ? 2 : 1);
  const int ns = mode == 2 ? 3 : 2;
  const int64_t nsuper = ((M + 16 * ns - 1) / (16 * ns) + NW22 - 1) / NW22;
  const dim3 g((unsigned)(nsuper < persistent_wgs ? nsuper : persistent_wgs)), b(64 * NW22);
  static DevOnce once[3];
  once[mode].run([&] {
    const void* k = mode == 0 ? reinterpret_cast<const void*>(mlp22_fwd_kernel<0>) : mode == 1 ? reinterpret_cast<const void*>(mlp22_fwd_kernel<1>)
                                                                                                : reinterpret_cast<const void*>(mlp22_fwd_kernel<1, 3>);
    (void)hipFuncSetAttribute(k, hipFuncAttributeMaxDynamicSharedMemorySize, RING_LDS_BYTES + park_bytes<3>());
  });
  if (mode == 0) hipLaunchKernelGGL(mlp22_fwd_kernel<0>, g, b, RING_LDS_BYTES, s, a);
  else if (mode == 1) hipLaunchKernelGGL(mlp22_fwd_kernel<1>, g, b, RING_LDS_BYTES, s, a);
  else hipLaunchKernelGGL((mlp22_fwd_kernel<1, 3>), g, b, RING_LDS_BYTES + park_bytes<3>(), s, a);
  return check_launch("mlp forward (split fp16)");
}

}
}
NERF_STAMP2_EXPORT(nerf_debug_stamps2_mlp22)
```

### nerf_meets_mlx_amd/csrc/mlp_layout.h

```cpp
#pragma once
#include "mlp_ring.h"
#include "mlp_params.h"

namespace nerf {

namespace L {

constexpr int F_L0 = 0, F_L1 = 32, F_L5 = 544, F_L6 = 704, F_L7 = 832, F_FA = 960, F_DIR = 1104, F_RGB = 1176;
constexpr int F_TOTAL = 1184;
constexpr int B_RGB = 0, B_DIR = 4, B_FA = 68, B_L7 = 204, B_L6 = 332, B_L5 = 460, B_L4 = 588;
constexpr int B_TOTAL = 1100, B_PADDED = 1120;
constexpr int BI_FEAT = 2048, BI_ALPHA = 2304, BI_DIR = 2336, BI_RGB = 2464, BI_TOTAL = 2496;
constexpr int F16_TOTAL = 1172, F16_PADDED = 1184;
constexpr int64_t F16_OFFSET = (int64_t)(F_TOTAL + B_PADDED) * 1024 + BI_TOTAL * 4;
constexpr int64_t PACKED_BYTES = F16_OFFSET + (int64_t)F16_PADDED * 1024;

constexpr int A_PE = 0, A_DPE = 4, A_H0 = 6;
constexpr int A_FEAT = 134, A_HD = 150;
constexpr int A_MASK = 158, A_SLOTS = 167;
constexpr int Z_L0 = 0;
constexpr int Z_F = 128, Z_A = 144, Z_D = 145, Z_RGB = 153, Z_SLOTS = 154;
}

__host__ __device__ constexpr int kperm(int ks, int h, int j) { return 16 * ks + 8 * (j >> 2) + 4 * h + (j & 3); }

namespace L16 {
constexpr int F_L0 = 0, F_L1 = 32, F_L5 = 544, F_L6 = 704, F_L7 = 832, F_FA = 960, F_DIR = 1096, F_RGB = 1168;
constexpr int CHUNKS = L::F16_PADDED / RING_CHUNK;
}
__host__ __device__ constexpr int kperm16(int ks, int g, int j) { return 32 * ks + 16 * (j >> 2) + 4 * g + (j & 3); }
__host__ __device__ constexpr int pos_chan16(int ks, int g, int j) {
  const int sl = 8 * ks + j;
  if (sl < 12) return 3 + 6 * (2 * g + sl / 6) + (sl % 6);
  if (sl < 15) return 3 + 6 * (8 + (g >> 1)) + 3 * (g & 1) + (sl - 12);
  return g < 3 ? g : -1;
}
__host__ __device__ constexpr int dir_chan16(int g, int j) {
  if (j < 6) return 3 + 6 * g + j;
  return (j == 6 && g < 3) ? g : -1;
}

__device__ inline float fwd_src16(const float* __restrict__ p, int f, int i, int g, int j) {
  if (f < L16::F_L1) {
    const int nt = f / 2, ch = pos_chan16(f % 2, g, j);
    return ch >= 0 ? p[L::P_W0 + (16 * nt + i) * 63 + ch] : 0.0f;
  }
  if (f < L16::F_L5) {
    const int q = f - L16::F_L1, l = 1 + q / 128, r = q % 128;
    return p[L::pw(l) + (16 * (r / 8) + i) * 256 + kperm16(r % 8, g, j)];
  }
  if (f < L16::F_L6) {
    const int q = f - L16::F_L5, n = 16 * (q / 10) + i, ks = q % 10;
    if (ks < 2) { const int ch = pos_chan16(ks, g, j); return ch >= 0 ? p[L::P_W5 + n * 319 + ch] : 0.0f; }
    return p[L::P_W5 + n * 319 + 63 + kperm16(ks - 2, g, j)];
  }
  if (f < L16::F_FA) {
    const int q = f - L16::F_L6, l = 6 + q / 128, r = q % 128;
    return p[L::pw(l) + (16 * (r / 8) + i) * 256 + kperm16(r % 8, g, j)];
  }
  if (f < L16::F_DIR) {
    const int q = f - L16::F_FA;
    if (q < 128) return p[L::P_WF + (16 * (q / 8) + i) * 256 + kperm16(q % 8, g, j)];
    return i == 0 ? p[L::P_WA + kperm16(q - 128, g, j)] : 0.0f;
  }
  if (f < L16::F_RGB) {
    const int q = f - L16::F_DIR, n = 16 * (q / 9) + i, ks = q % 9;
    if (ks < 8) return p[L::P_WD + n * 283 + kperm16(ks, g, j)];
    const int ch = dir_chan16(g, j);
    return ch >= 0 ? p[L::P_WD + n * 283 + 256 + ch] : 0.0f;
  }
  if (f < L::F16_TOTAL) return i < 3 ? p[L::P_WR + i * 128 + kperm16(f - L16::F_RGB, g, j)] : 0.0f;
  return 0.0f;
}


}
```

### nerf_meets_mlx_amd/csrc/pipeline.hip

```cpp
#include "common.h"
#include <dlfcn.h>
#include <string.h>

using namespace nerf;

extern "C" int64_t nerf_render_workspace_bytes(int64_t B, int n, int N) {
  if (B < 0 || n < 1 || N < 0) return -1;
  const int64_t nf = n + N;
  return B * (int64_t)(n  + 4 * n  + n  + nf  + 4 * nf ) * (int64_t)sizeof(float);
}

extern "C" int nerf_render_rays_fused(const nerf_mlp_arch* arch, const void* packed_coarse, const void* packed_fine,
                                      const float* rays, int64_t B, int n, int N, const float* u, int freq_mode,
                                      int white_bkgd, void* workspace, float* rgb, float* disp, float* acc,
                                      float* rgb_coarse, float* disp_coarse, float* acc_coarse, float* z_vals,
                                      float* weights, void* stream) {
  NERF_REQUIRE(B >= 0 && n >= 2 && N >= 0, NERF_E_SHAPE, "nerf_render_rays_fused: bad B/n/N");
  if (B == 0) return NERF_OK;
  NERF_REQUIRE(arch && packed_coarse && rays && workspace && rgb, NERF_E_NULL, "nerf_render_rays_fused: NULL pointer");
  NERF_REQUIRE(N == 0 || u, NERF_E_NULL, "nerf_render_rays_fused: N > 0 needs the uniforms u [B,N]");
  float* ws = static_cast<float*>(workspace);
  float* z = ws;
  float* raw = z + B * n;
  float* w = raw + B * n * 4;
  float* zf = w + B * n;
  float* rawf = zf + B * (n + N);
  int rc;
  if ((rc = nerf_sample_coarse(rays, B, n, 0, 0.0f, nullptr, z, stream))) return rc;
  if ((rc = nerf_query_fused(arch, packed_coarse, rays, z, B, n, freq_mode, raw, nullptr, stream))) return rc;
  float* rgb_c = N > 0 ? (rgb_coarse ? rgb_coarse : rgb) : rgb;
  if ((rc = nerf_composite_forward(raw, z, rays, B, n, 0.0f, nullptr, white_bkgd, rgb_c, N > 0 ? disp_coarse : disp,
                                   N > 0 ? acc_coarse : acc, w, nullptr, stream))) return rc;
  hipStream_t s = as_stream(stream);
  if (z_vals && hipMemcpyAsync(z_vals, z, sizeof(float) * B * n, hipMemcpyDeviceToDevice, s) != hipSuccess)
    return fail(NERF_E_HIP, "nerf_render_rays_fused: copy of z_vals failed");
  if (weights && hipMemcpyAsync(weights, w, sizeof(float) * B * n, hipMemcpyDeviceToDevice, s) != hipSuccess)
    return fail(NERF_E_HIP, "nerf_render_rays_fused: copy of weights failed");
  if (N == 0) {
    if (rgb_coarse && rgb_coarse != rgb &&
        hipMemcpyAsync(rgb_coarse, rgb, sizeof(float) * B * 3, hipMemcpyDeviceToDevice, s) != hipSuccess)
      return fail(NERF_E_HIP, "nerf_render_rays_fused: copy of rgb failed");
    return NERF_OK;
  }
  if ((rc = nerf_importance_sample(z, w, u, B, n, N, 1e-5f, nullptr, zf, nullptr, nullptr, stream))) return rc;
  if ((rc = nerf_query_fused(arch, packed_fine ? packed_fine : packed_coarse, rays, zf, B, n + N, freq_mode, rawf,
                             nullptr, stream))) return rc;
  return nerf_composite_forward(rawf, zf, rays, B, n + N, 0.0f, nullptr, white_bkgd, rgb, disp, acc, nullptr, nullptr,
                                stream);
}

namespace {
typedef struct { char internal[128]; } rccl_unique_id;
typedef int (*fn_get_id)(rccl_unique_id*);
typedef int (*fn_init_rank)(void**, int, rccl_unique_id, int);
typedef int (*fn_allreduce)(const void*, void*, size_t, int, int, void*, hipStream_t);
typedef int (*fn_destroy)(void*);
typedef const char* (*fn_errstr)(int);
struct Rccl {
  void* h = nullptr; fn_get_id get_id = nullptr; fn_init_rank init_rank = nullptr; fn_allreduce allreduce = nullptr;
  fn_destroy destroy = nullptr; fn_errstr errstr = nullptr;
};
Rccl g_rccl;
int rccl_load() {
  if (g_rccl.h) return NERF_OK;
  const char* names[] = {"librccl.so.1", "librccl.so", "/opt/rocm/lib/librccl.so.1"};
  void* h = nullptr;
  for (const char* nm : names) if ((h = dlopen(nm, RTLD_NOW | RTLD_GLOBAL))) break;
  if (!h) return fail(NERF_E_RCCL, "RCCL not available: %s", dlerror());
  g_rccl.get_id = (fn_get_id)dlsym(h, "ncclGetUniqueId");
  g_rccl.init_rank = (fn_init_rank)dlsym(h, "ncclCommInitRank");
  g_rccl.allreduce = (fn_allreduce)dlsym(h, "ncclAllReduce");
  g_rccl.destroy = (fn_destroy)dlsym(h, "ncclCommDestroy");
  g_rccl.errstr = (fn_errstr)dlsym(h, "ncclGetErrorString");
  if (!g_rccl.get_id || !g_rccl.init_rank || !g_rccl.allreduce || !g_rccl.destroy)
    return fail(NERF_E_RCCL, "RCCL symbols missing in librccl");
  g_rccl.h = h;
  return NERF_OK;
}
int rccl_fail(const char* what, int code) {
  return fail(NERF_E_RCCL, "%s: %s", what, g_rccl.errstr ? g_rccl.errstr(code) : "rccl error");
}
}

extern "C" int nerf_comm_unique_id(char* id_out) {
  NERF_REQUIRE(id_out, NERF_E_NULL, "nerf_comm_unique_id: id_out is NULL");
  int rc = rccl_load();
  if (rc) return rc;
  rccl_unique_id id;
  const int e = g_rccl.get_id(&id);
  if (e) return rccl_fail("ncclGetUniqueId", e);
  memcpy(id_out, id.internal, 128);
  return NERF_OK;
}

extern "C" int nerf_comm_init(void** comm_out, int nranks, int rank, const char* id) {
  NERF_REQUIRE(comm_out && id, NERF_E_NULL, "nerf_comm_init: NULL pointer");
  NERF_REQUIRE(nranks >= 1 && rank >= 0 && rank < nranks, NERF_E_SHAPE, "nerf_comm_init: bad rank %d of %d", rank, nranks);
  int rc = rccl_load();
  if (rc) return rc;
  rccl_unique_id uid;
  memcpy(uid.internal, id, 128);
  const int e = g_rccl.init_rank(comm_out, nranks, uid, rank);
  return e ? rccl_fail("ncclCommInitRank", e) : NERF_OK;
}

extern "C" int nerf_allreduce_grads(void* comm, float* grads, int64_t count, void* stream) {
  NERF_REQUIRE(comm && grads, NERF_E_NULL, "nerf_allreduce_grads: NULL pointer");
  NERF_REQUIRE(count > 0, NERF_E_SHAPE, "nerf_allreduce_grads: count must be > 0");
  int rc = rccl_load();
  if (rc) return rc;
  const int e = g_rccl.allreduce(grads, grads, (size_t)count,  7,  0, comm, as_stream(stream));
  return e ? rccl_fail("ncclAllReduce", e) : NERF_OK;
// ... 10 lines not shown
```

### nerf_meets_mlx_amd/engine/trainer.py

```python
import os
from typing import Dict, Optional

import numpy as np
import torch

from .. import parallel, sampling
from ..models.NeRF import Adam, NeRF
from ..ops import index
from ..rendering import ray, render


class Trainer:
    def __init__(self, images: torch.Tensor, poses: torch.Tensor, K, near: float = 2.0, far: float = 6.0,
                 N_rand: int = 1024, n_depth_samples: int = 64, N_importance: int = 128, lrate: float = 5e-4,
                 lrate_decay: int = 500, white_bkgd: bool = True, ref_quirks: bool = True, seed: int = 0,
                 device="cuda", chunk: int = 1024 * 32, precision: int = 22, overlap_comm: bool = True):
        self.device = torch.device(device)
        self.images = images.to(self.device, torch.float32).contiguous()
        self.poses = poses.float().cpu()
        self.K = np.asarray(K, dtype=np.float64)
        self.H, self.W = int(images.shape[1]), int(images.shape[2])
        self.near, self.far = near, far
        self.N_rand, self.n, self.N = N_rand, n_depth_samples, N_importance
        self.lrate, self.lrate_decay = lrate, lrate_decay
        self.white_bkgd, self.q, self.chunk = white_bkgd, ref_quirks, chunk
        self.rank, self.world = parallel.world()
        self.seed = seed
        mk = lambda s: NeRF(channel_input=63, channel_input_views=27, is_use_view_directions=True,
                            device=self.device, seed=s, precision=precision)
        self.precision = precision
        self.coarse = mk(seed)
        self.fine = mk(seed + 1) if N_importance > 0 else None
        self.coarse.name = "coarse"
        if self.fine is not None:
            self.fine.name = "fine"
        self.opt = Adam(lrate, betas=(0.9, 0.999), shared_state=ref_quirks)
        self.it = 0
        self._comm = torch.cuda.Stream(device=self.device) if (self.world > 1 and overlap_comm) else None
        self.gen = torch.Generator(device=self.device)
        self.gen.manual_seed(parallel.rank_seed(seed, self.rank, 2))
        self._train_gen = torch.Generator(device=self.device)

    def _join_comm(self):
        if getattr(self, "_comm", None) is not None:
            torch.cuda.current_stream(self.device).wait_stream(self._comm)

    @property
    def fine(self):
        self._join_comm()
        return self._fine

    @fine.setter
    def fine(self, m):
        self._fine = m

    @property
    def opt(self):
        self._join_comm()
        return self._opt

    @opt.setter
    def opt(self, o):
        self._opt = o

    def image_choice(self) -> int:
        return parallel.counter_seed(self.seed, self.rank, 1, self.it) % int(self.images.shape[0])

    def train_uniforms(self, B: int) -> torch.Tensor:
        self._train_gen.manual_seed(parallel.counter_seed(self.seed, self.rank, 2, self.it))
        return torch.rand(B, self.N, device=self.device, generator=self._train_gen)

    def _step_net(self, model: NeRF, rays, z, target, white: bool, join: bool = True):
        raw = model.query(rays, z, ref_quirks=self.q, train=True)
        loss, d_raw, _ = render.composite_mse_backward(raw, z, rays, target, white)
        grads = model.backward(d_raw)
        if self._comm is None:
            parallel.allreduce_sum_(grads)
            self._opt.update(model, grads, grad_scale=1.0 / self.world)
            return loss
        cur = torch.cuda.current_stream(self.device)
        self._comm.wait_stream(cur)
        with torch.cuda.stream(self._comm):
            parallel.allreduce_sum_(grads)
            self._opt.update(model, grads, grad_scale=1.0 / self.world)
        if join:
            cur.wait_stream(self._comm)
        return loss

    def sample_batch(self, pixel_idx: Optional[torch.Tensor] = None, img_i: Optional[int] = None):
        if img_i is None:
            img_i = self.image_choice()
        if pixel_idx is None:
            return ray.sample_batch(self.H, self.W, self.K, self.poses[img_i, :3, :4], self.near, self.far,
                                    self.images[img_i], self.N_rand, parallel.counter_seed(self.seed, self.rank, 3, self.it))
        rays = ray.gen_rays(self.H, self.W, self.K, self.poses[img_i, :3, :4], self.near, self.far, pixel_idx)
        target = index.gather_rows(self.images[img_i].reshape(-1, self.images.shape[-1]), pixel_idx)
        return rays, target

    def train_step(self, rays=None, target=None, u=None) -> Dict[str, torch.Tensor]:
        if rays is None:
            rays, target = self.sample_batch()
        self._opt.learning_rate = self.lrate * (0.1 ** (self.it / (self.lrate_decay * 1000)))
        z = sampling.sample_coarse(rays, self.n)
        out = {"loss_coarse": self._step_net(self.coarse, rays, z, target, self.white_bkgd)}
        if self._fine is not None:
            raw = self.coarse.query(rays, z, ref_quirks=self.q)
            _, _, _, weights, _ = render.composite(raw, z, rays, 0.0, self.white_bkgd)
            if u is None:
                u = self.train_uniforms(rays.shape[0])
            _, z_fine = sampling.importance_sample(z, weights, self.N, u=u)
            white_fine = self.white_bkgd if not self.q else False
            out["loss_fine"] = self._step_net(self._fine, rays, z_fine, target, white_fine, join=False)
        self.it += 1
        return out

    def render_rays(self, rays: torch.Tensor, u=None, background=None):
        if background is not None:
            raise ValueError("Trainer.render_rays: background is a mode of NGPTrainer's march; this renderer composites onto white "
                             "or nothing (white_bkgd)")
        outs = []
        for s in range(0, rays.shape[0], self.chunk):
            r = rays[s:s + self.chunk]
            uu = None if u is None else u[s:s + self.chunk]
            if uu is None and self.N > 0:
                uu = torch.rand(r.shape[0], self.N, device=self.device, generator=self.gen)
            outs.append(render.render_rays_fused(r, self.coarse, self.fine, self.n, self.N, u=uu,
                                                 white_bkgd=self.white_bkgd, ref_quirks=self.q, with_coarse=False)["rgb_map"])
        return torch.cat(outs, 0)

    def render_frame(self, c2w, shard: bool = True, background=None) -> Optional[torch.Tensor]:
        lo, hi = parallel.shard_range(self.H * self.W, self.rank, self.world) if shard else (0, self.H * self.W)
        idx = torch.arange(lo, hi, device=self.device, dtype=torch.int64)
        rays = ray.gen_rays(self.H, self.W, self.K, np.asarray(c2w)[:3, :4], self.near, self.far, idx)
        if background is None:
            rgb = self.render_rays(rays)
        else:
            per_pixel = torch.is_tensor(background) and background.dim() == 2 and background.shape[0] == self.H * self.W
            rgb = self.render_rays(rays, background=background[lo:hi] if per_pixel else background)
        if shard and self.world > 1:
            rgb = parallel.gather_rows_to_rank0(rgb, self.H * self.W)
            if rgb is None:
                return None
        return rgb.reshape(self.H, self.W, 3)

    def psnr(self, c2w, gt: torch.Tensor, background=None) -> float:
        img = self.render_frame(c2w, shard=False, background=background)
        mse = torch.mean((img - gt.to(self.device)) ** 2)
        return float(10.0 * torch.log10(1.0 / mse))

    def _mesh_field(self):
        from .mesh import RELU
        model = self.fine if self.fine is not None else self.coarse
        return (lambda rays, z: model.query(rays, z, ref_quirks=self.q)), RELU

    def _mesh_box(self, aabb):
        if aabb is None:
            raise ValueError("Trainer mesh export: the 8 x 256 field has no scene box, pass aabb=(lo, hi)")
        lo, hi = aabb
        return [float(x) for x in lo], [float(x) for x in hi]

    def density_volume(self, resolution: int, aabb=None) -> torch.Tensor:
        from . import mesh
        lo, hi = self._mesh_box(aabb)
        query, act = self._mesh_field()
        return mesh.density_volume(query, act, resolution, lo, hi, device=self.device)

    def extract_mesh(self, resolution: int = 256, threshold: float = 2.5, aabb=None, colors: bool = True,
                     min_component: int = 0, largest_only: bool = False, opening_radius: int = 0):
        from . import mesh
        lo, hi = self._mesh_box(aabb)
        mesh.check_component_args(min_component, largest_only, mesh.check_mesh_args(resolution, lo, hi, threshold)[0])
        mesh.check_opening_args(opening_radius)
        query, act = self._mesh_field()
        return mesh.extract(query, act, resolution, threshold, lo, hi, colors=colors, device=self.device,
                            min_component=min_component, largest_only=largest_only, opening_radius=opening_radius)

    def _checkpoint_buffers(self):
        b = {"coarse": self.coarse}
        if self.fine is not None:
            b["fine"] = self.fine
        return b

    def sync_optimizer_state(self):
        self._join_comm()

    def state_dict(self):
        return {"it": self.it, "seed": int(self.seed),
                "params": {k: m.params.detach().cpu().clone() for k, m in self._checkpoint_buffers().items()},
                "adam": self.opt.state_dict()}
# ... 69 lines not shown
```

### nerf_meets_mlx_amd/models/NeRF.py

```python
import ctypes as C
import math
from typing import Dict, List, Optional

import numpy as np
import torch

from .. import _native as N
from . import embedding

_LAYERS = None


def layer_shapes(n_layers=8, width=256, cin=63, cdir=27, skips=(4,), use_viewdirs=True, cout=4):
    s = [("pos0", width, cin)]
    for i in range(n_layers - 1):
        s.append((f"pos{i + 1}", width, width + cin if i in skips else width))
    if use_viewdirs:
        s += [("feature", width, width), ("alpha", 1, width), ("dir0", width // 2, width + cdir), ("rgb", 3, width // 2)]
    else:
        s += [("output", cout, width)]
    return s


class NeRF:

    def __init__(self, n_layers=8, width_layers=256, channel_input=3, channel_input_views=3, channel_output=4,
                 list_skip_connection_layers=[4], is_use_view_directions=False, device="cuda", seed: Optional[int] = None,
                 precision: int = 22):
        self.D, self.W = n_layers, width_layers
        self.channel_input_pos, self.channel_input_dir = channel_input, channel_input_views
        self.list_skip_connection_layers = list(list_skip_connection_layers)
        self.is_use_view_directions = is_use_view_directions
        self.device = torch.device(device)
        self.shapes = layer_shapes(n_layers, width_layers, channel_input, channel_input_views,
                                   tuple(self.list_skip_connection_layers), is_use_view_directions, channel_output)
        self.n_params = sum(o * i + o for _, o, i in self.shapes)
        self.arch = N.MlpArch(n_layers, width_layers, channel_input, channel_input_views,
                              self.list_skip_connection_layers[0] if len(self.list_skip_connection_layers) == 1 else -1,
                              int(bool(is_use_view_directions)), channel_output, int(precision))
        if precision not in (16, 22, 32):
            raise ValueError("NeRF: precision must be 16 (bf16 MFMA operands), 32 (fp32 MFMA) or 22 (float32 tolerance on the "
                             "16-bit matrix pipe: split-bf16 training, split-fp16 inference)")
        self.precision = int(precision)
        self.out_dim = 4 if is_use_view_directions else channel_output
        rng = np.random.default_rng(seed)
        chunks = []
        for _, o, i in self.shapes:
            k = 1.0 / math.sqrt(i)
            chunks.append(rng.uniform(-k, k, size=(o, i)).astype(np.float32).reshape(-1))
            chunks.append(rng.uniform(-k, k, size=(o,)).astype(np.float32))
        self.params = torch.from_numpy(np.concatenate(chunks)).to(self.device)
        self.grads = torch.zeros_like(self.params)
        self._packed = None
        self._dirty = True
        self._packed_version = -1
        self._ws: Dict[str, torch.Tensor] = {}
        self.name: Optional[str] = None
        self._gen = 0
        self._acts_gen = -1
        self._acts_M = -1

    def parameters(self) -> Dict[str, object]:
        views, off = {}, 0
        for name, o, i in self.shapes:
            views[name] = {"weight": self.params[off:off + o * i].view(o, i), "bias": self.params[off + o * i:off + o * i + o]}
            off += o * i + o
        tree = {"list_linears_pos": [views[f"pos{l}"] for l in range(self.D)]}
        if self.is_use_view_directions:
            tree.update({"list_linears_dir": [views["dir0"]], "feature_linear": views["feature"],
                         "alpha_linear": views["alpha"], "rgb_linear": views["rgb"]})
        else:
            tree["output_linear"] = views["output"]
        return tree

    def trainable(self) -> torch.Tensor:
        if not self.params.requires_grad:
            self.params.requires_grad_(True)
        return self.params

    def load_flat(self, flat: torch.Tensor):
        assert flat.numel() == self.n_params
        with torch.no_grad():
            self.params.copy_(flat.to(self.device, torch.float32).reshape(-1))
        self._dirty = True

    def mark_updated(self):
        self._dirty = True

    def activation_generation(self) -> int:
        return self._acts_gen

    def packed(self) -> torch.Tensor:
        lib = N.lib()
        if self._packed is None:
            nbytes = lib.nerf_mlp_packed_bytes(C.byref(self.arch))
            if nbytes < 0:
                raise ValueError("libnerf_hip error -3: this NeRF architecture / precision has no HIP kernel (supported: "
                                 "n_layers=8, width=256, skips=[4] with in=63+27 + view head [precision 16, 22, 32], or in=40 without "
                                 "view head and out<=4 [16, 22, 32]; n_layers=2, width=64, skips=[] with in=32+16 + view head [16, 22])")
            self._packed = torch.empty(nbytes, dtype=torch.uint8, device=self.device)
        if self._dirty or self.params._version != self._packed_version:
            N.check(lib.nerf_mlp_pack(C.byref(self.arch), N.ptr(self.params), N.ptr(self._packed), N.stream()))
            self._dirty = False
            self._packed_version = self.params._version
        return self._packed

    def _begin_train_pass(self, M: int) -> torch.Tensor:
        acts = self._workspace("acts", N.lib().nerf_mlp_acts_bytes(C.byref(self.arch), M))
        self._gen += 1
        self._acts_gen, self._acts_M = self._gen, M
        return acts

    def _workspace(self, key: str, nbytes: int) -> torch.Tensor:
        t = self._ws.get(key)
        if t is None or t.numel() < nbytes:
            t = torch.empty(nbytes, dtype=torch.uint8, device=self.device)
            self._ws[key] = t
        return t

    def forward(self, x: torch.Tensor, train: bool = False) -> torch.Tensor:
        x = N.f32(x).reshape(-1, x.shape[-1])
        M = x.shape[0]
        out = torch.empty(M, self.out_dim, dtype=torch.float32, device=x.device)
        acts = None
        if train:
            acts = self._begin_train_pass(M)
        N.check(N.lib().nerf_mlp_forward_train(C.byref(self.arch), N.ptr(self.packed()), N.ptr(x), M, N.ptr(out),
                                               N.ptr(acts), N.stream()))
        return out

    __call__ = forward

    def query(self, rays: torch.Tensor, z: torch.Tensor, ref_quirks: bool = True, train: bool = False) -> torch.Tensor:
        B, n = z.shape
        raw = torch.empty(B, n, 4, dtype=torch.float32, device=z.device)
        acts = None
        if train:
            acts = self._begin_train_pass(B * n)
        N.check(N.lib().nerf_query_fused(C.byref(self.arch), N.ptr(self.packed()), N.ptr(rays), N.ptr(z), B, n,
                                         0 if ref_quirks else 1, N.ptr(raw), N.ptr(acts), N.stream()))
        return raw

    def backward(self, d_raw: torch.Tensor, need_input_grad: bool = False, generation: Optional[int] = None):
        d_raw = N.f32(d_raw)
        M = d_raw.numel() // self.out_dim
        if generation is not None and generation != self._acts_gen:
            raise RuntimeError(f"NeRF.backward: the activations of forward #{generation} were overwritten by train-mode "
                               f"forward #{self._acts_gen} of the same model (one activation workspace per model: run "
                               "backward before the next train-mode forward, or use a second model object)")
        assert M == self._acts_M, "backward() needs a matching query/forward(train=True) first"
        dz = self._workspace("dz", N.lib().nerf_mlp_dz_bytes(C.byref(self.arch), M))
        if need_input_grad:
            d_x = torch.empty(M, self.channel_input_pos, dtype=torch.float32, device=d_raw.device)
            N.check(N.lib().nerf_mlp_backward_inputs(C.byref(self.arch), N.ptr(self.packed()), N.ptr(self._ws["acts"]),
                                                     N.ptr(d_raw), M, N.ptr(dz), N.ptr(self.grads), N.ptr(d_x), N.stream()))
            return self.grads, d_x
        N.check(N.lib().nerf_mlp_backward(C.byref(self.arch), N.ptr(self.packed()), N.ptr(self._ws["acts"]),
                                          N.ptr(d_raw), M, N.ptr(dz), N.ptr(self.grads), N.stream()))
        return self.grads


def debug_layer(model: NeRF, kind: str, layer: int) -> torch.Tensor:
    k = {"acts": 0, "dz": 1}[kind]
    w = N.lib().nerf_mlp_debug_width(C.byref(model.arch), k, layer)
    if w < 0:
        raise ValueError("debug_layer: no such (kind, layer) in this model's training stores (include/nerf_hip.h, nerf_mlp_debug_read)")
    M = model._acts_M
    out = torch.empty(M, w, dtype=torch.float32, device=model.device)
    N.check(N.lib().nerf_mlp_debug_read(C.byref(model.arch), N.ptr(model._ws[kind]), k, layer, M, N.ptr(out), N.stream()))
    return out


class Adam:

    def __init__(self, learning_rate: float, betas=(0.9, 0.999), eps: float = 1e-8, bias_correction: bool = False,
                 shared_state: bool = True):
        self.learning_rate = learning_rate
        self.betas, self.eps = betas, eps
        self.bias_correction, self.shared_state = bias_correction, shared_state
        self.state: Dict[str, List[torch.Tensor]] = {}
        self.step_count: Dict[str, int] = {}
        self._auto_names: Dict[int, str] = {}

    def key_of(self, model) -> str:
        if self.shared_state:
            return "shared"
        name = getattr(model, "name", None)
        if name:
            return str(name)
        return self._auto_names.setdefault(id(model), f"model{len(self._auto_names)}")

    def update(self, model: NeRF, grads: Optional[torch.Tensor] = None, grad_scale: float = 1.0, zero_grads: bool = False):
        g = model.grads if grads is None else grads
        key = self.key_of(model)
        if key not in self.state:
            self.state[key] = [torch.zeros_like(model.params), torch.zeros_like(model.params)]
        self.step_count[key] = self.step_count.get(key, 0) + 1
        m, v = self.state[key]
        half = getattr(model, "half", None)
        if zero_grads or g.dtype == torch.int64 or half is not None:
            N.check(N.lib().nerf_adam_step_shadow(N.ptr(model.params), N.ptr(g), N.ptr(m), N.ptr(v), model.n_params,
                                                  float(self.learning_rate), float(self.betas[0]), float(self.betas[1]),
                                                  float(self.eps), int(self.bias_correction), self.step_count[key],
                                                  float(grad_scale), int(g.dtype == torch.int64), int(bool(zero_grads)),
                                                  N.ptr(half), N.stream()))
            if half is not None:
                model.mark_updated(shadow_written=True)
                return
        else:
            N.check(N.lib().nerf_adam_step(N.ptr(model.params), N.ptr(g), N.ptr(m), N.ptr(v), model.n_params,
                                           float(self.learning_rate), float(self.betas[0]), float(self.betas[1]),
                                           float(self.eps), int(self.bias_correction), self.step_count[key],
                                           float(grad_scale), N.stream()))
        model.mark_updated()

    def update_spans(self, model, spans, grad_scale: float = 1.0):
        key = self.key_of(model)
        if key not in self.state:
# ... 81 lines not shown
```

### nerf_meets_mlx_amd/rendering/render.py

```python
from typing import Dict, Optional

import torch

from .. import _native as N
from .. import sampling
from . import ray


def composite(raw, z_vals, rays, raw_noise_std=0.0, white_bkgd=False, noise=None, need_weights=True):
    B, n = z_vals.shape
    dev = raw.device
    rgb = torch.empty(B, 3, dtype=torch.float32, device=dev)
    disp = torch.empty(B, dtype=torch.float32, device=dev)
    acc = torch.empty(B, dtype=torch.float32, device=dev)
    depth = torch.empty(B, dtype=torch.float32, device=dev)
    weights = torch.empty(B, n, dtype=torch.float32, device=dev) if need_weights else None
    if raw_noise_std > 0.0 and noise is None:
        noise = torch.randn(B, n, dtype=torch.float32, device=dev)
    N.check(N.lib().nerf_composite_forward(N.ptr(raw), N.ptr(z_vals), N.ptr(rays), B, n, float(raw_noise_std),
                                           N.ptr(noise) if raw_noise_std > 0.0 else None, int(bool(white_bkgd)),
                                           N.ptr(rgb), N.ptr(disp), N.ptr(acc), N.ptr(weights), N.ptr(depth), N.stream()))
    return rgb, disp, acc, weights, depth


# ... 110 lines not shown
    return _packed_forward(raw, z, offsets, B, step_world, False, background_arg(background, B, offsets.device), None, None)[:3]


def composite_packed_distortion_bg(raw, z, offsets, rays, step_world: float, march_steps: int, background):
    B = rays.shape[0]
    return _packed_forward(raw, z, offsets, B, step_world, False, background_arg(background, B, offsets.device), rays, march_steps)


def composite_packed_mse_backward_bg(raw, offsets, B: int, step_world: float, target_rgba, background, grad_scale: float = 1.0,
                                     need_rgb: bool = False):
    target_rgba, bg = _rgba_and_bg(target_rgba, background, B, offsets.device)
    loss, _, d_raw, rgb = _packed_train(raw, None, offsets, B, step_world, target_rgba, False, bg, None, None, None, grad_scale, need_rgb)
    return loss, d_raw, rgb


def composite_packed_mse_dist_backward_bg(raw, z, offsets, rays, step_world: float, march_steps: int, target_rgba, background,
                                          dist_weight: float, grad_scale: float = 1.0, need_rgb: bool = False):
    target_rgba, bg = _rgba_and_bg(target_rgba, background, rays.shape[0], offsets.device)
    return _packed_train(raw, z, offsets, rays.shape[0], step_world, target_rgba, False, bg, rays, march_steps, dist_weight, grad_scale,
                         need_rgb)


def ert_init(istate, fstate, live, B: int):
    N.check(N.lib().nerf_ert_init(B, N.ptr(istate), N.ptr(fstate), N.ptr(live), N.stream()))


def ert_fold(raw, z, offsets, live, A: int, istate, fstate, step_world: float, min_transmittance: float):
    raw = N.f32(raw).reshape(-1, 4)
    z = N.f32(z).reshape(-1)
    K = raw.shape[0]
    B = istate.shape[0]
    N.check(N.lib().nerf_ert_fold(N.ptr(raw) if K else None, N.ptr(z) if K else None, N.ptr(offsets), N.ptr(live), A, B, K,
                                  float(step_world), float(min_transmittance), N.ptr(istate), N.ptr(fstate), N.stream()))


def _ert_finish(istate, fstate, white_bkgd, bg):
    B, dev = istate.shape[0], istate.device
    rgb = torch.empty(B, 3, dtype=torch.float32, device=dev)
    acc = torch.empty(B, dtype=torch.float32, device=dev)
    depth = torch.empty(B, dtype=torch.float32, device=dev)
    samples = torch.empty(B, dtype=torch.int32, device=dev)
    fn, mode = (N.lib().nerf_ert_finish, [int(bool(white_bkgd))]) if bg is None else (N.lib().nerf_ert_finish_bg, [N.ptr(bg[0]), bg[1]])
    N.check(fn(N.ptr(istate), N.ptr(fstate), B, *mode, N.ptr(rgb), N.ptr(acc), N.ptr(depth), N.ptr(samples), N.stream()))
    return rgb, acc, depth, samples


def ert_finish(istate, fstate, white_bkgd=False):
    return _ert_finish(istate, fstate, white_bkgd, None)


def ert_finish_bg(istate, fstate, background):
    return _ert_finish(istate, fstate, False, background_arg(background, istate.shape[0], istate.device))


def ert_finish_over(istate, fstate, white_bkgd=False, background=None):
    return ert_finish(istate, fstate, white_bkgd) if background is None else ert_finish_bg(istate, fstate, background)


_WS = {}


def render_rays_fused(rays, network_coarse, network_fine, n_depth_samples, N_importance, u=None, white_bkgd=False,
                      ref_quirks=True, with_coarse=True):
    import ctypes as C
    rays = N.f32(rays)
    B, n, Nn = rays.shape[0], int(n_depth_samples), int(N_importance or 0)
    dev = rays.device
    if Nn > 0 and u is None:
        u = torch.rand(B, Nn, dtype=torch.float32, device=dev)
    nbytes = N.lib().nerf_render_workspace_bytes(B, n, Nn)
    key = (dev, torch.cuda.current_stream(dev).cuda_stream)
    ws = _WS.get(key)
    if ws is None or ws.numel() < nbytes:
        ws = torch.empty(nbytes, dtype=torch.uint8, device=dev)
        _WS[key] = ws
    f = lambda *shape: torch.empty(*shape, dtype=torch.float32, device=dev)
    rgb, disp, acc = f(B, 3), f(B), f(B)
    ret = {}
    if with_coarse:
        ret = {"rgb_coarse": f(B, 3), "disp_coarse": f(B), "acc_coarse": f(B), "z_vals": f(B, n), "weights": f(B, n)}
    fine = network_fine if network_fine else network_coarse
    if getattr(fine, "precision", 16) != getattr(network_coarse, "precision", 16):
        raise ValueError("render_rays_fused: coarse and fine networks must have the same precision (one nerf_mlp_arch per call)")
    N.check(N.lib().nerf_render_rays_fused(
        C.byref(network_coarse.arch), N.ptr(network_coarse.packed()), N.ptr(fine.packed()), N.ptr(rays), B, n, Nn,
        N.ptr(u) if Nn > 0 else None, 0 if ref_quirks else 1, int(bool(white_bkgd)), N.ptr(ws), N.ptr(rgb), N.ptr(disp),
        N.ptr(acc), N.ptr(ret.get("rgb_coarse")), N.ptr(ret.get("disp_coarse")), N.ptr(ret.get("acc_coarse")),
        N.ptr(ret.get("z_vals")), N.ptr(ret.get("weights")), N.stream()))
    out = {"rgb_map": rgb, "disp_map": disp[:, None], "acc_map": acc[:, None]}
    if with_coarse:
        if Nn == 0:
            ret["disp_coarse"], ret["acc_coarse"] = disp, acc
        out.update({"rgb_coarse": ret["rgb_coarse"], "disp_coarse": ret["disp_coarse"][:, None],
                    "acc_coarse": ret["acc_coarse"][:, None], "z_vals": ret["z_vals"], "weights": ret["weights"][..., None]})
    return out


def raw2outputs(raw, z_vals, rays_d, raw_noise_std=0, white_bkgd=False, pytest=False, noise=None):
    raw, z_vals = N.f32(raw), N.f32(z_vals)
    B = z_vals.shape[0]
    rays = torch.zeros(B, 11, dtype=torch.float32, device=raw.device)
    rays[:, 3:6] = rays_d
    rgb, disp, acc, w, depth = composite(raw, z_vals, rays, float(raw_noise_std), white_bkgd, noise)
    return rgb, disp[:, None], acc[:, None], w[..., None], depth[:, None]


def decompose_ray_batch(rays_batch_linear, is_time_included: bool = False):
    r = rays_batch_linear
    rays_o, rays_d = r[:, 0:3], r[:, 3:6]
    bounds = r[..., 6:8 + int(is_time_included)].reshape(-1, 1, 2 + int(is_time_included))
    near, far = bounds[..., 0], bounds[..., 1]
    frame_time = bounds[..., 2] if is_time_included else None
    return rays_o, rays_d, near, far, r[:, -3:], frame_time


def _query(network_query_fn, rays, z, model):
    if hasattr(network_query_fn, "fused") and hasattr(model, "query"):
        return network_query_fn.fused(rays, z, model)
    o, d, _, _, viewdirs, _ = decompose_ray_batch(rays)
    pos = o[..., None, :] + z[..., :, None] * d[..., None, :]
    return network_query_fn(pos, viewdirs, model)


def _coarse_pass(rays, network_coarse, network_query_fn, n_depth_samples, retraw, lindisp, perturb, white_bkgd,
                 raw_noise_std):
    rays = N.f32(rays)
    z_vals = sampling.sample_coarse(rays, n_depth_samples, lindisp=lindisp, perturb=float(perturb or 0.0))
    raw = _query(network_query_fn, rays, z_vals, network_coarse)
    rgb, disp, acc, weights, depth = composite(raw, z_vals, rays, float(raw_noise_std or 0.0), white_bkgd)
    ret = {}
    if retraw:
        ret["raw"] = raw
    ret.update({"rgb_map": rgb, "disp_map": disp[:, None], "acc_map": acc[:, None], "rgb_coarse": rgb,
                "disp_coarse": disp[:, None], "acc_coarse": acc[:, None], "z_vals": z_vals,
                "weights": weights[..., None]})
    return rays, ret


def render_rays(rays_batch_linear, network_coarse, network_query_fn, n_depth_samples, retraw=False, lindisp=False,
                perturb=0.0, N_importance=0, network_fine=None, white_bkgd=False, raw_noise_std=0.0, verbose=False,
                pytest=False, **kwargs):
    return _coarse_pass(rays_batch_linear, network_coarse, network_query_fn, n_depth_samples, retraw, lindisp, perturb,
                        white_bkgd, raw_noise_std)[1]


def render_rays_eval(rays_batch_linear, network_coarse, network_query_fn, n_depth_samples, retraw=False, lindisp=False,
                     perturb=0.0, N_importance=0, network_fine=None, white_bkgd=False, raw_noise_std=0.0,
                     verbose=False, pytest=False, u=None, **kwargs):
    rays, ret = _coarse_pass(rays_batch_linear, network_coarse, network_query_fn, n_depth_samples, retraw, lindisp,
                             perturb, white_bkgd, raw_noise_std)
    if N_importance and N_importance > 0:
        _, z_fine = sampling.importance_sample(ret["z_vals"], ret["weights"], N_importance, u=u)
        run_fn = network_fine if network_fine else network_coarse
        raw = _query(network_query_fn, rays, z_fine, run_fn)
        rgb, disp, acc, _, _ = composite(raw, z_fine, rays, float(raw_noise_std or 0.0), white_bkgd, need_weights=False)
        ret["rgb_map"], ret["disp_map"], ret["acc_map"] = rgb, disp[:, None], acc[:, None]
    return ret


def batchify_rays(rays_linear, chunk=1024 * 32, **kwargs):
    render_rays_func = kwargs["render_rays_func"]
    u_all = kwargs.pop("u", None)
    results: Dict[str, list] = {}
    for i in range(0, rays_linear.shape[0], chunk):
        extra = {} if u_all is None else {"u": u_all[i:i + chunk]}
        out = render_rays_func(rays_linear[i:i + chunk], **kwargs, **extra)
        for k, v in out.items():
            results.setdefault(k, []).append(v)
# ... 31 lines not shown
```

Baseline: 1.233 million.

## Add density-only coarse requery path skipping view-dependent RGB head

Adds a separate packed weight image holding only the layers needed for density, plus a forward kernel that evaluates just those layers. It is used when the coarse network is requeried only to get weights for importance sampling (in training and in rendering without coarse outputs). This skips the direction encoding and the view and RGB layers, cutting MFMA work and weight streaming for that pass. In exchange it needs extra packing work and memory for the density image, and a stale-repack flag that can trigger additional pack launches.

Measured after the change: 1.236 million (median of 6 runs). No clear change (+0.3%).

```diff
diff --git a/include/nerf_hip.h b/include/nerf_hip.h
--- a/include/nerf_hip.h
+++ b/include/nerf_hip.h
@@ -132,6 +132,11 @@
 
 int nerf_query_fused(const nerf_mlp_arch* arch, const void* packed, const float* rays, const float* z, int64_t B,
                      int n, int freq_mode, float* raw, void* acts, void* stream);
+
+int64_t nerf_mlp_density_bytes(const nerf_mlp_arch* arch);
+int nerf_mlp_pack_density(const nerf_mlp_arch* arch, const float* params, void* packed, void* density, void* stream);
+int nerf_query_density(const nerf_mlp_arch* arch, const void* packed, const void* density, const float* rays, const float* z,
+                       int64_t B, int n, int freq_mode, float* raw, void* stream);
 
 int nerf_mlp_backward(const nerf_mlp_arch* arch, const void* packed, const void* acts, const float* d_raw,
                       int64_t M, void* dz, float* grads, void* stream);
@@ -260,6 +265,11 @@
                            const float* rays, int64_t B, int n, int N, const float* u, int freq_mode, int white_bkgd,
                            void* workspace, float* rgb, float* disp, float* acc, float* rgb_coarse, float* disp_coarse,
                            float* acc_coarse, float* z_vals, float* weights, void* stream);
+int nerf_render_rays_fused_density(const nerf_mlp_arch* arch, const void* packed_coarse, const void* packed_fine,
+                                   const void* density_coarse, const float* rays, int64_t B, int n, int N, const float* u,
+                                   int freq_mode, int white_bkgd, void* workspace, float* rgb, float* disp, float* acc,
+                                   float* rgb_coarse, float* disp_coarse, float* acc_coarse, float* z_vals, float* weights,
+                                   void* stream);
 
 #define NERF_COMM_ID_BYTES 128
 int nerf_comm_unique_id(char* id_out_host);
diff --git a/nerf_meets_mlx_amd/_native.py b/nerf_meets_mlx_amd/_native.py
--- a/nerf_meets_mlx_amd/_native.py
+++ b/nerf_meets_mlx_amd/_native.py
@@ -43,6 +43,9 @@
     "nerf_mlp_param_count": (_I64, [_P]),
     "nerf_mlp_packed_bytes": (_I64, [_P]),
     "nerf_mlp_pack": (_I, [_P, _P, _P, _P]),
+    "nerf_mlp_density_bytes": (_I64, [_P]),
+    "nerf_mlp_pack_density": (_I, [_P, _P, _P, _P, _P]),
+    "nerf_query_density": (_I, [_P, _P, _P, _P, _P, _I64, _I, _I, _P, _P]),
     "nerf_mlp_acts_bytes": (_I64, [_P, _I64]),
     "nerf_mlp_dz_bytes": (_I64, [_P, _I64]),
     "nerf_mlp_forward": (_I, [_P, _P, _P, _I64, _P, _P]),
@@ -54,6 +57,7 @@
     "nerf_mlp_debug_read": (_I, [_P, _P, _I, _I, _I64, _P, _P]),
     "nerf_render_workspace_bytes": (_I64, [_I64, _I, _I]),
     "nerf_render_rays_fused": (_I, [_P, _P, _P, _P, _I64, _I, _I, _P, _I, _I, _P, _P, _P, _P, _P, _P, _P, _P, _P, _P]),
+    "nerf_render_rays_fused_density": (_I, [_P, _P, _P, _P, _P, _I64, _I, _I, _P, _I, _I, _P, _P, _P, _P, _P, _P, _P, _P, _P, _P]),
     "nerf_comm_unique_id": (_I, [C.c_char_p]),
     "nerf_comm_init": (_I, [C.POINTER(C.c_void_p), _I, _I, C.c_char_p]),
     "nerf_allreduce_grads": (_I, [_P, _P, _I64, _P]),
diff --git a/nerf_meets_mlx_amd/csrc/mlp.hip b/nerf_meets_mlx_amd/csrc/mlp.hip
--- a/nerf_meets_mlx_amd/csrc/mlp.hip
+++ b/nerf_meets_mlx_amd/csrc/mlp.hip
@@ -1405,6 +1405,7 @@
 static int g_ring_wgs = 0;
 static int g_ngp_ray_major = 1;
 int g_pass_queue = 1;
+static int g_density_requery = 1;
 static int g_ring_split = 1;
 static inline int arch_prec(const nerf_mlp_arch* a) { return a->precision == 32 ? 32 : a->precision == 22 ? 22 : 16; }
 static inline bool arch_f32(const nerf_mlp_arch* a) { return a->precision == 32; }
@@ -1483,6 +1484,7 @@
   if (!strcmp(key, "dw_ring_cap")) { g_dw_ring_cap = value < 2 ? 2 : value > 16 ? 16 : value; return NERF_OK; }
   if (!strcmp(key, "pass_queue")) { g_pass_queue = value ? 1 : 0; return NERF_OK; }
   if (!strcmp(key, "dw_narrow_first")) { g_dw_narrow_first = value ? 1 : 0; return NERF_OK; }
+  if (!strcmp(key, "density_requery")) { g_density_requery = value ? 1 : 0; return NERF_OK; }
   if (!strcmp(key, "f22_tiles")) {
     NERF_REQUIRE(value == 0 || value == 2 || value == 3, NERF_E_UNSUPPORTED, "nerf_set_option: f22_tiles must be 0 (automatic), 2 or 3");
     f22::g_tiles = value;
@@ -1510,6 +1512,7 @@
   if (!strcmp(key, "pass_queue")) return g_pass_queue;
   if (!strcmp(key, "dw_narrow_first")) return g_dw_narrow_first;
   if (!strcmp(key, "f22_tiles")) return f22::g_tiles;
+  if (!strcmp(key, "density_requery")) return g_density_requery;
   return NERF_OPTION_UNKNOWN;
 }
 
@@ -1522,6 +1525,10 @@
   return k == 0 ? L::PACKED_BYTES + (arch_f32(arch) ? f32::PACKED_BYTES : 0) + (arch_s16(arch) ? f22::PACKED_BYTES + s16::PACKED_BYTES : 0)
          : k == 1 ? IMG_BF16_BYTES + (arch_s16(arch) ? s16x::IMG_PACKED_BYTES : 0) + (arch_f32(arch) ? f32::PACKED_BYTES : 0)
          : k == 2 ? LN::PACKED_BYTES + (arch_s16(arch) ? s16x::SM_PACKED_BYTES : 0) : -1;
+}
+extern "C" int64_t nerf_mlp_density_bytes(const nerf_mlp_arch* arch) {
+  const int k = arch_kind(arch);
+  return k < 0 ? -1 : (k == 0 && arch_s16(arch)) ? f22::DENSITY_BYTES : 0;
 }
 static inline const void* packed32_of(const void* packed) { return static_cast<const char*>(packed) + L::PACKED_BYTES; }
 static inline const void* packed22_of(const void* packed) { return static_cast<const char*>(packed) + L::PACKED_BYTES; }
@@ -1555,8 +1562,14 @@
 #define NERF_ARCH_CHECK_ANY(who) NERF_REQUIRE(arch_kind(arch) >= 0, NERF_E_UNSUPPORTED, who NERF_ARCH_MSG)
 
 extern "C" int nerf_mlp_pack(const nerf_mlp_arch* arch, const float* params, void* packed, void* stream) {
+  return nerf_mlp_pack_density(arch, params, packed, nullptr, stream);
+}
+
+extern "C" int nerf_mlp_pack_density(const nerf_mlp_arch* arch, const float* params, void* packed, void* density, void* stream) {
   NERF_ARCH_CHECK_ANY("nerf_mlp_pack");
   NERF_REQUIRE(params && packed, NERF_E_NULL, "nerf_mlp_pack: params/packed is NULL");
+  NERF_REQUIRE(!density || nerf_mlp_density_bytes(arch) > 0, NERF_E_UNSUPPORTED,
+               "nerf_mlp_pack_density: this model has no density-only image (nerf_mlp_density_bytes is 0)");
   char* base = static_cast<char*>(packed);
   if (arch_kind(arch) == 2) {
     const int tot = (LN::F_PADDED + LN::B_PADDED) * 64 + LN::BI_TOTAL;
@@ -1587,7 +1600,7 @@
   int rc = check_launch("nerf_mlp_pack");
   if (rc) return rc;
   if (arch_f32(arch)) rc = f32::pack(params, base + L::PACKED_BYTES, 0, as_stream(stream));
-  if (!rc && arch_s16(arch)) rc = f22::pack(params, base + L::PACKED_BYTES, as_stream(stream));
+  if (!rc && arch_s16(arch)) rc = f22::pack(params, base + L::PACKED_BYTES, density, as_stream(stream));
   if (!rc && arch_s16(arch)) rc = s16::pack(params, base + L::PACKED_BYTES + f22::PACKED_BYTES, as_stream(stream));
   return rc;
 }
@@ -1747,6 +1760,18 @@
   return launch_fwd<1>(packed, nullptr, rays, z, B * n, n, freq_mode, raw, acts, stream);
 }
 
+extern "C" int nerf_query_density(const nerf_mlp_arch* arch, const void* packed, const void* density, const float* rays,
+                                  const float* z, int64_t B, int n, int freq_mode, float* raw, void* stream) {
+  if (!arch_ok(arch) || !arch_s16(arch) || !g_density_requery)
+    return nerf_query_fused(arch, packed, rays, z, B, n, freq_mode, raw, nullptr, stream);
+  NERF_REQUIRE(n >= 1, NERF_E_SHAPE, "nerf_query_density: n must be >= 1");
+  if (B <= 0) return NERF_OK;
+  NERF_REQUIRE(packed && density && rays && z && raw, NERF_E_NULL, "nerf_query_density: NULL pointer");
+  NERF_REQUIRE(freq_mode == 0 || freq_mode == 1, NERF_E_UNSUPPORTED, "nerf_query_density: freq_mode must be 0 or 1");
+  NERF_REQUIRE(B * (int64_t)n < (1ll << 31), NERF_E_SHAPE, "nerf_query_density: B*n must be < 2^31 samples per call");
+  return f22::forward_density(packed22_of(packed), density, rays, z, B * n, n, freq_mode, raw, ring_wgs(), as_stream(stream));
+}
+
 static int launch_dw_part(DwArgs& d, int nj, int64_t ntiles, int64_t nparams, const void* acts, void* dz, int64_t astride,
                           int64_t zstride, float* grads, hipStream_t s, int kind, int a_lo, int z_lo, int slot_base, int max_wgs) {
   const bool split_bf16 = kind == 1 || kind == 2;
diff --git a/nerf_meets_mlx_amd/csrc/mlp22.h b/nerf_meets_mlx_amd/csrc/mlp22.h
--- a/nerf_meets_mlx_amd/csrc/mlp22.h
+++ b/nerf_meets_mlx_amd/csrc/mlp22.h
@@ -8,10 +8,15 @@
 constexpr int F_PAIRS = 1172, F_FRAGS = 2 * F_PAIRS, F_PADDED = 2368, BIAS_FLOATS = 2496;
 constexpr int64_t PACKED_BYTES = (int64_t)F_PADDED * 1024 + (int64_t)BIAS_FLOATS * 4;
 
+constexpr int D_PAIRS = 968, D_FRAGS = 2 * D_PAIRS, D_PADDED = 1952;
+constexpr int64_t DENSITY_BYTES = (int64_t)D_PADDED * 1024;
+
 extern int g_tiles;
-int pack(const float* params, void* packed22, hipStream_t s);
+int pack(const float* params, void* packed22, void* density22, hipStream_t s);
 int forward(const void* packed22, const float* x, const float* rays, const float* z, int64_t M, int n, int freq_mode,
             float* out, int persistent_wgs, hipStream_t s);
+int forward_density(const void* packed22, const void* density22, const float* rays, const float* z, int64_t M, int n,
+                    int freq_mode, float* out, int persistent_wgs, hipStream_t s);
 
 }
 }
diff --git a/nerf_meets_mlx_amd/csrc/mlp22.hip b/nerf_meets_mlx_amd/csrc/mlp22.hip
--- a/nerf_meets_mlx_amd/csrc/mlp22.hip
+++ b/nerf_meets_mlx_amd/csrc/mlp22.hip
@@ -1,74 +1,36 @@
-#include "mlp_layout.h"
-#include "mlp22.h"
-
-#ifndef NERF_F22_SINF
-#define NERF_F22_SINF 0
-#endif
-
-#ifndef NERF_F22_PIN
-#define NERF_F22_PIN 1
-#endif
-#ifndef NERF_F22_AGPR
-#define NERF_F22_AGPR 1
-#endif
-#ifndef NERF_F22_MIXSUB
-#define NERF_F22_MIXSUB 1
-#endif
-#ifndef NERF_F22_RG3
-#define NERF_F22_RG3 4
-#endif
-#ifndef NERF_F22_IGLP
-#define NERF_F22_IGLP 0
-#endif
+#include "mlp22_dev.h"
 
 namespace nerf {
 namespace f22 {
 
-typedef _Float16 h8 __attribute__((ext_vector_type(8)));
-typedef _Float16 h2 __attribute__((ext_vector_type(2)));
-typedef float f32x2 __attribute__((ext_vector_type(2)));
-typedef unsigned int u32x4 __attribute__((ext_vector_type(4)));
-
-constexpr float LO_SCALE = 2048.0f, LO_INV = 1.0f / 2048.0f;
-constexpr float F16_MIN_NORMAL = 6.103515625e-05f;
-constexpr int CHUNKS = F_PADDED / RING_CHUNK;
-static_assert(CHUNKS * RING_CHUNK == F_PADDED && F_FRAGS % 4 == 0 && F_PAIRS == L::F16_TOTAL, "f22 stream layout");
-
-struct HiLo { unsigned hi, lo; };
-__device__ __forceinline__ HiLo split2(float v0, float v1) {
-  const f32x2 v = {v0, v1};
-  const h2 hh = __builtin_convertvector(v, h2);
-#if NERF_F22_MIXSUB
-  const f32x2 r = {__builtin_fmaf((float)hh[0], -LO_SCALE, v0 * LO_SCALE), __builtin_fmaf((float)hh[1], -LO_SCALE, v1 * LO_SCALE)};
-#else
-  const f32x2 r = {(v0 - (float)hh[0]) * LO_SCALE, (v1 - (float)hh[1]) * LO_SCALE};
-#endif
-  return HiLo{__builtin_bit_cast(unsigned, hh), __builtin_bit_cast(unsigned, __builtin_convertvector(r, h2))};
+constexpr int PACK_THREADS = (F_PADDED / 2) * 64 + BIAS_FLOATS;
+constexpr int PACK_THREADS_D = (D_PADDED / 2) * 64;
+__device__ __forceinline__ void pack_pair(const float* __restrict__ p, int fp, int lane, u32x4& hi, u32x4& lo) {
+  hi = u32x4{0u, 0u, 0u, 0u}; lo = u32x4{0u, 0u, 0u, 0u};
+  if (fp < F_PAIRS) {
+#pragma unroll
+    for (int j = 0; j < 8; j += 2) {
+      float w[2];
+      _Float16 wh[2], wl[2];
+#pragma unroll
+      for (int e = 0; e < 2; ++e) {
+        w[e] = fwd_src16(p, fp, lane & 15, lane >> 4, j + e);
+        wh[e] = __builtin_fabsf(w[e]) < F16_MIN_NORMAL ? (_Float16)0.0f : (_Float16)w[e];
+        wl[e] = (_Float16)((w[e] - (float)wh[e]) * LO_SCALE);
+      }
+      const h2 a = {wh[0], wh[1]}, b = {wl[0], wl[1]};
+      hi[j >> 1] = __builtin_bit_cast(unsigned, a);
+      lo[j >> 1] = __builtin_bit_cast(unsigned, b);
+    }
+  }
 }
-
-constexpr int PACK_THREADS = (F_PADDED / 2) * 64 + BIAS_FLOATS;
 __global__ void __launch_bounds__(256) pack22_kernel(const float* __restrict__ p, u32x4* __restrict__ wf,
-                                                     float* __restrict__ bias) {
+                                                     float* __restrict__ bias, u32x4* __restrict__ wd) {
   const int t = blockIdx.x * 256 + threadIdx.x;
   if (t < (F_PADDED / 2) * 64) {
     const int fp = t >> 6, lane = t & 63;
-    u32x4 hi = {0u, 0u, 0u, 0u}, lo = {0u, 0u, 0u, 0u};
-    if (fp < F_PAIRS) {
-#pragma unroll
-      for (int j = 0; j < 8; j += 2) {
-        float w[2];
-        _Float16 wh[2], wl[2];
-#pragma unroll
-        for (int e = 0; e < 2; ++e) {
-          w[e] = fwd_src16(p, fp, lane & 15, lane >> 4, j + e);
-          wh[e] = __builtin_fabsf(w[e]) < F16_MIN_NORMAL ? (_Float16)0.0f : (_Float16)w[e];
-          wl[e] = (_Float16)((w[e] - (float)wh[e]) * LO_SCALE);
-        }
-        const h2 a = {wh[0], wh[1]}, b = {wl[0], wl[1]};
-        hi[j >> 1] = __builtin_bit_cast(unsigned, a);
-        lo[j >> 1] = __builtin_bit_cast(unsigned, b);
-      }
-    }
+    u32x4 hi, lo;
+    pack_pair(p, fp, lane, hi, lo);
     wf[(2 * fp) * 64 + lane] = hi;
     wf[(2 * fp + 1) * 64 + lane] = lo;
   } else if (t < PACK_THREADS) {
@@ -80,353 +42,21 @@
     else if (s < L::BI_RGB) v = p[L::P_BD + (s - L::BI_DIR)];
     else v = (s - L::BI_RGB) < 3 ? p[L::P_BR + (s - L::BI_RGB)] : 0.0f;
     bias[s] = v;
+  } else if (wd && t < PACK_THREADS + PACK_THREADS_D) {
+    const int dp = (t - PACK_THREADS) >> 6, lane = (t - PACK_THREADS) & 63;
+    const int fp = dp < L16::D_ALPHA ? dp : dp < D_PAIRS ? L16::F_FA + 128 + (dp - L16::D_ALPHA) : F_PAIRS;
+    u32x4 hi, lo;
+    pack_pair(p, fp, lane, hi, lo);
+    wd[(2 * dp) * 64 + lane] = hi;
+    wd[(2 * dp + 1) * 64 + lane] = lo;
   }
 }
 
-__device__ __forceinline__ float sin_acc(float x, float f, float ph) {
-  const float a = x * f;
-#if NERF_F22_SINF
-  return ph != 0.0f ? cosf(a) : sinf(a);
-#else
-  const float k = __builtin_rintf(a * 0.15915494309189535f);
-  float r = __builtin_fmaf(-k, 6.2831854820251465f, a);
-  r = __builtin_fmaf(-k, -1.7484556000744487e-07f, r);
-  return __builtin_amdgcn_sinf(__builtin_fmaf(r, 0.15915494309189535f, ph));
-#endif
-}
-
-struct Pe22 { float fa, fb, fc, phc, fd; int g; };
-__device__ __forceinline__ Pe22 pe22_setup(const PeFreq& fr, int g) {
-  Pe22 q;
-  q.fa = g == 0 ? fr.pos[0] : g == 1 ? fr.pos[2] : g == 2 ? fr.pos[4] : fr.pos[6];
-  q.fb = g == 0 ? fr.pos[1] : g == 1 ? fr.pos[3] : g == 2 ? fr.pos[5] : fr.pos[7];
-  q.fc = g < 2 ? fr.pos[8] : fr.pos[9];
-  q.phc = (g & 1) ? 0.25f : 0.0f;
-  q.fd = g == 0 ? fr.dir[0] : g == 1 ? fr.dir[1] : g == 2 ? fr.dir[2] : fr.dir[3];
-  q.g = g;
-  return q;
-}
-
-template <int COUNT>
-__device__ __forceinline__ void split_slots(const float (&v)[COUNT], u32x4* hi, u32x4* lo) {
-#pragma unroll
-  for (int j = 0; j < COUNT; j += 2) {
-    const HiLo q = split2(v[j], v[j + 1]);
-    hi[j >> 3][(j & 7) >> 1] = q.hi; lo[j >> 3][(j & 7) >> 1] = q.lo;
-  }
-}
-
-__device__ __forceinline__ void pe22_pos(const Pe22& q, const float (&p)[3], u32x4 (&peh)[2], u32x4 (&pel)[2]) {
-  float v[16];
-#pragma unroll
-  for (int sl = 0; sl < 12; ++sl) v[sl] = sin_acc(p[sl % 3], sl < 6 ? q.fa : q.fb, (sl % 6) >= 3 ? 0.25f : 0.0f);
-#pragma unroll
-  for (int k = 0; k < 3; ++k) v[12 + k] = sin_acc(p[k], q.fc, q.phc);
-  v[15] = q.g == 0 ? p[0] : q.g == 1 ? p[1] : q.g == 2 ? p[2] : 0.0f;
-  split_slots<16>(v, peh, pel);
-}
-__device__ __forceinline__ void pe22_dir(const Pe22& q, const float (&d)[3], u32x4 (&dph)[1], u32x4 (&dpl)[1]) {
-  float w[8];
-#pragma unroll
-  for (int j = 0; j < 6; ++j) w[j] = sin_acc(d[j % 3], q.fd, j >= 3 ? 0.25f : 0.0f);
-  w[6] = q.g == 0 ? d[0] : q.g == 1 ? d[1] : q.g == 2 ? d[2] : 0.0f;
-  w[7] = 0.0f;
-  split_slots<8>(w, dph, dpl);
-}
-__device__ __forceinline__ void pe22_encode(const Pe22& q, const float (&p)[3], const float (&d)[3], u32x4 (&peh)[2],
-                                            u32x4 (&pel)[2], u32x4 (&dph)[1], u32x4 (&dpl)[1]) {
-  pe22_pos(q, p, peh, pel);
-  pe22_dir(q, d, dph, dpl);
-}
-__device__ __forceinline__ void pe22_row(const float* __restrict__ row, int g, u32x4 (&peh)[2], u32x4 (&pel)[2],
-                                         u32x4 (&dph)[1], u32x4 (&dpl)[1]) {
-  float v[16], w[8];
-#pragma unroll
-  for (int sl = 0; sl < 16; ++sl) {
-    const int ch = pos_chan16(sl >> 3, g, sl & 7);
-    v[sl] = ch >= 0 ? row[ch] : 0.0f;
-  }
-#pragma unroll
-  for (int j = 0; j < 8; ++j) {
-    const int ch = dir_chan16(g, j);
-    w[j] = ch >= 0 ? row[63 + ch] : 0.0f;
-  }
-  split_slots<16>(v, peh, pel);
-  split_slots<8>(w, dph, dpl);
-}
-
-__device__ __forceinline__ f32x4 mfma16(const u32x4& a, const u32x4& b, const f32x4& c) {
-#if NERF_ABLATE == 41 || NERF_ABLATE == 42
-  return c;
-#endif
-  return __builtin_amdgcn_mfma_f32_16x16x32_f16(__builtin_bit_cast(h8, a), __builtin_bit_cast(h8, b), c, 0, 0, 0);
-}
-
-template <int NS, int KS, int NT, bool RELU, class WS, bool PARK_LDS = false>
-__device__ __forceinline__ void layer22(WS& ws, int pbase, int bias_slot, const u32x4 (&ih)[NS][KS], const u32x4 (&il)[NS][KS],
-                                        u32x4 (&oh)[NS][NT / 2], u32x4 (&ol)[NS][NT / 2], int lane, unsigned park_addr = 0u) {
-  const int g = lane >> 4;
-  f32x4 pm[NS], pc[NS];
-  if (PARK_LDS) asm volatile("ds_write_b128 %0, %1" :: "v"(park_addr), "v"(il[NS - 1][KS - 1]) : "memory");
-#if NERF_F22_IGLP >= 0
-  __builtin_amdgcn_iglp_opt(NERF_F22_IGLP);
-#endif
-  constexpr int NP = 2 * NS;
-  auto piece = [&](int nt, int pcs, f32x4 (&m)[NS], f32x4 (&c)[NS]) {
-    const int s = pcs >> 1, i = 2 * (pcs & 1);
-#if NERF_ABLATE == 41 || NERF_ABLATE == 42
-    return;
-#endif
-#if NERF_F22_PIN
-    if (pcs == 0) {
-#pragma unroll
-      for (int t = 0; t < NS; ++t) asm volatile("" : "+v"(m[t]), "+v"(c[t]));
-    }
-#endif
-    float v0 = __builtin_fmaf(c[s][i], LO_INV, m[s][i]), v1 = __builtin_fmaf(c[s][i + 1], LO_INV, m[s][i + 1]);
-    if (RELU) { v0 = __builtin_elementwise_maximum(v0, 0.0f); v1 = __builtin_elementwise_maximum(v1, 0.0f); }
-    const HiLo q = split2(v0, v1);
-    oh[s][nt >> 1][2 * (nt & 1) + (i >> 1)] = q.hi; ol[s][nt >> 1][2 * (nt & 1) + (i >> 1)] = q.lo;
-#if NERF_F22_AGPR
-    if ((nt & 1) && i == 2) asm volatile("" : "+a"(oh[s][nt >> 1]), "+a"(ol[s][nt >> 1]));
-#endif
-  };
-  auto piece_at = [](int q) { return NS == 2 ? (KS >= 8 ? 1 + 2 * q : (q * KS) / 4) : (KS >= 8 ? 1 + (q * (KS - 1)) / NP : (q * KS) / NP); };
-#pragma unroll
-  for (int nt = 0; nt < NT; ++nt) {
-    const float4 b = ws.bias4(bias_slot + 16 * nt + 4 * g);
-    f32x4 m[NS], c[NS];
-    m[0][0] = b.x; m[0][1] = b.y; m[0][2] = b.z; m[0][3] = b.w;
-    c[0] = f32x4{0.0f, 0.0f, 0.0f, 0.0f};
-#pragma unroll
-    for (int t = 1; t < NS; ++t) { m[t] = m[0]; c[t] = c[0]; }
-#pragma unroll
-    for (int ks = 0; ks < KS; ++ks) {
-      const int fp = pbase + nt * KS + ks;
-      const u32x4 ah = __builtin_bit_cast(u32x4, next_frag(ws, 2 * fp, lane));
-      const u32x4 al = __builtin_bit_cast(u32x4, next_frag(ws, 2 * fp + 1, lane));
-      if (NS == 2) {
-        m[0] = mfma16(ah, ih[0][ks], m[0]);
-        c[0] = mfma16(ah, il[0][ks], c[0]);
-        m[1] = mfma16(ah, ih[1][ks], m[1]);
-        c[1] = mfma16(ah, il[1][ks], c[1]);
-        c[0] = mfma16(al, ih[0][ks], c[0]);
-        c[1] = mfma16(al, ih[1][ks], c[1]);
-      } else {
-#pragma unroll
-        for (int t = 0; t < NS; ++t) {
-          m[t] = mfma16(ah, ih[t][ks], m[t]);
-          if (PARK_LDS && t == NS - 1 && ks == KS - 1) {
-            u32x4 b;
-            asm volatile("ds_read_b128 %0, %1\n\ts_waitcnt lgkmcnt(0)" : "=v"(b) : "v"(park_addr) : "memory");
-            c[t] = mfma16(ah, b, c[t]);
-          } else {
-            c[t] = mfma16(ah, il[t][ks], c[t]);
-          }
-        }
-#pragma unroll
-        for (int t = 0; t < NS; ++t) c[t] = mfma16(al, ih[t][ks], c[t]);
-      }
-      if (nt > 0) {
-#pragma unroll
-        for (int q = 0; q < NP; ++q)
-          if (piece_at(q) == ks) piece(nt - 1, q, pm, pc);
-      }
-    }
-#pragma unroll
-    for (int t = 0; t < NS; ++t) { pm[t] = m[t]; pc[t] = c[t]; }
-  }
-#pragma unroll
-  for (int q = 0; q < NP; ++q) piece(NT - 1, q, pm, pc);
-}
-
-template <int NS, int KS, class WS>
-__device__ __forceinline__ void head22(WS& ws, int pbase, int bias_slot, const u32x4 (&ih)[NS][KS], const u32x4 (&il)[NS][KS],
-                                       f32x4 (&out)[NS], int lane) {
-  const int g = lane >> 4;
-  const float4 b = ws.bias4(bias_slot + 4 * g);
-  f32x4 m[NS], c[NS];
-  m[0][0] = b.x; m[0][1] = b.y; m[0][2] = b.z; m[0][3] = b.w;
-  c[0] = f32x4{0.0f, 0.0f, 0.0f, 0.0f};
-#pragma unroll
-  for (int t = 1; t < NS; ++t) { m[t] = m[0]; c[t] = c[0]; }
-#pragma unroll
-  for (int ks = 0; ks < KS; ++ks) {
-    const u32x4 ah = __builtin_bit_cast(u32x4, next_frag(ws, 2 * (pbase + ks), lane));
-    const u32x4 al = __builtin_bit_cast(u32x4, next_frag(ws, 2 * (pbase + ks) + 1, lane));
-    if (NS == 2) {
-      m[0] = mfma16(ah, ih[0][ks], m[0]);
-      c[0] = mfma16(ah, il[0][ks], c[0]);
-      m[1] = mfma16(ah, ih[1][ks], m[1]);
-      c[1] = mfma16(ah, il[1][ks], c[1]);
-      c[0] = mfma16(al, ih[0][ks], c[0]);
-      c[1] = mfma16(al, ih[1][ks], c[1]);
-    } else {
-#pragma unroll
-      for (int t = 0; t < NS; ++t) { m[t] = mfma16(ah, ih[t][ks], m[t]); c[t] = mfma16(ah, il[t][ks], c[t]); }
-#pragma unroll
-      for (int t = 0; t < NS; ++t) c[t] = mfma16(al, ih[t][ks], c[t]);
-    }
-  }
-#pragma unroll
-  for (int s = 0; s < NS; ++s)
-#pragma unroll
-    for (int i = 0; i < 4; ++i) out[s][i] = __builtin_fmaf(c[s][i], LO_INV, m[s][i]);
-}
-
-constexpr int NW22 = 4, NW22_ = NW22;
-constexpr int PARK_OFF = RING_LDS_BYTES;
-template <int NS> constexpr int park_bytes() { return NS > 2 ? (6 * NS + 4) * 64 * NW22_ * 4 : 0; }
-template <int K> __device__ __forceinline__ void lds_put(unsigned addr, float v) {
-  asm volatile("ds_write_b32 %0, %1 offset:%2" :: "v"(addr), "v"(v), "i"(1024 * K) : "memory");
-}
-template <int K> __device__ __forceinline__ float lds_get(unsigned addr) {
-  float v;
-  asm volatile("ds_read_b32 %0, %1 offset:%2\n\ts_waitcnt lgkmcnt(0)" : "=v"(v) : "v"(addr), "i"(1024 * K) : "memory");
-  return v;
-}
-template <int S> __device__ __forceinline__ void park_put(unsigned park, const float (&p)[3], const float (&d)[3]) {
-  lds_put<6 * S + 0>(park, p[0]); lds_put<6 * S + 1>(park, p[1]); lds_put<6 * S + 2>(park, p[2]);
-  lds_put<6 * S + 3>(park, d[0]); lds_put<6 * S + 4>(park, d[1]); lds_put<6 * S + 5>(park, d[2]);
-}
-template <int S, int OFF> __device__ __forceinline__ void park_get(unsigned park, float (&v)[3]) {
-  v[0] = lds_get<6 * S + OFF>(park); v[1] = lds_get<6 * S + OFF + 1>(park); v[2] = lds_get<6 * S + OFF + 2>(park);
-}
-__device__ __forceinline__ void park_put_s(int s, unsigned park, const float (&p)[3], const float (&d)[3]) {
-  if (s == 0) park_put<0>(park, p, d); else if (s == 1) park_put<1>(park, p, d); else park_put<2>(park, p, d);
-}
-template <int OFF> __device__ __forceinline__ void park_get_s(int s, unsigned park, float (&v)[3]) {
-  if (s == 0) park_get<0, OFF>(park, v); else if (s == 1) park_get<1, OFF>(park, v); else park_get<2, OFF>(park, v);
-}
-
-template <int NS, int MODE, class WS>
-__device__ __forceinline__ void tiles22(const FwdArgs& a, WS& ws, int64_t wtile0, int64_t nwtiles, int lane, PassQueue& pq) {
-  constexpr bool RECOMP = NS > 2;
-  static_assert(!RECOMP || MODE == 1, "the 48-sample form takes rays + depths");
-  const int c = lane & 15, g = lane >> 4;
-  u32x4 peh[NS][2], pel[NS][2], dph[NS][1], dpl[NS][1];
-  const unsigned park = ws.lds0 + PARK_OFF + 4u * (unsigned)(ws.wv * 64 + lane);
-  pq.ask(ws.wv, lane);
-  const Pe22 q = pe22_setup(a.fr, g);
-  {
-    const int64_t wt = wtile0 < nwtiles ? wtile0 : nwtiles - 1;
-#pragma unroll
-    for (int s = 0; s < NS; ++s) {
-      int64_t m = wt * (16 * NS) + 16 * s + c; if (m >= a.M) m = a.M - 1;
-      if (MODE == 0) {
-        pe22_row(a.x + m * 90, g, peh[s], pel[s], dph[s], dpl[s]);
-      } else {
-        const int64_t ray = (int64_t)((unsigned)m / (unsigned)a.n);
-        const float* rr = a.rays + ray * NERF_RAY_STRIDE;
-        float p[3], d[3];
-#if NERF_ABLATE == 3
-        (void)rr;
-#pragma unroll
-        for (int k = 0; k < 3; ++k) { p[k] = 0.001f * (float)(m & 1023) + (float)k; d[k] = 0.5f; }
-#else
-        const float zv = a.z[m];
-#pragma unroll
-        for (int k = 0; k < 3; ++k) { p[k] = rr[k] + zv * rr[3 + k]; d[k] = rr[8 + k]; }
-#endif
-        if (RECOMP) {
-          park_put_s(s, park, p, d);
-          pe22_pos(q, p, peh[s], pel[s]);
-        } else {
-          pe22_encode(q, p, d, peh[s], pel[s], dph[s], dpl[s]);
-        }
-      }
-    }
-  }
-  pq.publish(ws.wv);
-  u32x4 hah[NS][8], hal[NS][8], hbh[NS][8], hbl[NS][8];
-  layer22<NS, 2, 16, true>(ws, L16::F_L0, 0, peh, pel, hah, hal, lane);
-  layer22<NS, 8, 16, true>(ws, L16::F_L1 + 0 * 128, 256, hah, hal, hbh, hbl, lane);
-  layer22<NS, 8, 16, true>(ws, L16::F_L1 + 1 * 128, 512, hbh, hbl, hah, hal, lane);
-  layer22<NS, 8, 16, true>(ws, L16::F_L1 + 2 * 128, 768, hah, hal, hbh, hbl, lane);
-  layer22<NS, 8, 16, true>(ws, L16::F_L1 + 3 * 128, 1024, hbh, hbl, hah, hal, lane);
-  {
-    u32x4 cth[NS][10], ctl[NS][10];
-#pragma unroll
-    for (int s = 0; s < NS; ++s) {
-      if (RECOMP) {
-        float pp[3];
-        park_get_s<0>(s, park, pp);
-        pe22_pos(q, pp, peh[s], pel[s]);
-      }
-      cth[s][0] = peh[s][0]; cth[s][1] = peh[s][1]; ctl[s][0] = pel[s][0]; ctl[s][1] = pel[s][1];
-#pragma unroll
-      for (int k = 0; k < 8; ++k) { cth[s][2 + k] = hah[s][k]; ctl[s][2 + k] = hal[s][k]; }
-    }
-    layer22<NS, 10, 16, true, WS, (NS > 2)>(ws, L16::F_L5, 1280, cth, ctl, hbh, hbl, lane,
-                                            ws.lds0 + PARK_OFF + 6 * NS * 64 * NW22 * 4 + 16u * (unsigned)(ws.wv * 64 + lane));
-  }
-  layer22<NS, 8, 16, true>(ws, L16::F_L6, 1536, hbh, hbl, hah, hal, lane);
-  layer22<NS, 8, 16, true>(ws, L16::F_L7, 1792, hah, hal, hbh, hbl, lane);
-  layer22<NS, 8, 16, false>(ws, L16::F_FA, L::BI_FEAT, hbh, hbl, hah, hal, lane);
-  f32x4 alpha[NS];
-  head22<NS, 8>(ws, L16::F_FA + 128, L::BI_ALPHA, hbh, hbl, alpha, lane);
-  u32x4 hdh[NS][4], hdl[NS][4];
-  {
-    u32x4 cth[NS][9], ctl[NS][9];
-#pragma unroll
-    for (int s = 0; s < NS; ++s) {
-#pragma unroll
-      for (int k = 0; k < 8; ++k) { cth[s][k] = hah[s][k]; ctl[s][k] = hal[s][k]; }
-      if (RECOMP) {
-        float dd[3];
-        park_get_s<3>(s, park, dd);
-        pe22_dir(q, dd, dph[s], dpl[s]);
-      }
-      cth[s][8] = dph[s][0]; ctl[s][8] = dpl[s][0];
-    }
-    layer22<NS, 9, 8, true>(ws, L16::F_DIR, L::BI_DIR, cth, ctl, hdh, hdl, lane);
-  }
-  f32x4 rgb[NS];
-  head22<NS, 4>(ws, L16::F_RGB, L::BI_RGB, hdh, hdl, rgb, lane);
-#pragma unroll
-  for (int s = 0; s < NS; ++s) {
-    const int64_t m = wtile0 * (16 * NS) + 16 * s + c;
-    if (g == 0 && wtile0 < nwtiles && m < a.M) {
-      float4 o; o.x = rgb[s][0]; o.y = rgb[s][1]; o.z = rgb[s][2]; o.w = alpha[s][0];
-      *reinterpret_cast<float4*>(a.out + m * 4) = o;
-    }
-  }
-}
-
-template <int MODE, int NS = 2>
-__global__ void __launch_bounds__(64 * NW22) mlp22_fwd_kernel(FwdArgs a) {
-  const int lane = threadIdx.x & 63;
-  const int wv = __builtin_amdgcn_readfirstlane(threadIdx.x >> 6);
-  const int64_t nwtiles = (a.M + 16 * NS - 1) / (16 * NS), nsuper = (nwtiles + NW22 - 1) / NW22;
-  NERF_STAMP2_DECL();
-  RingW<CHUNKS, F_FRAGS, (NS > 2 ? NERF_F22_RG3 : 4), NW22, RING_CHUNK, RING_STAGES, true, true> ws;
-  ws.wsrc = reinterpret_cast<const char*>(a.wf);
-  ws.lane16 = 16 * lane;
-  ws.lds0 = __builtin_amdgcn_readfirstlane(lds_addr_of(ring_smem));
-  ws.wv = wv;
-  ws.start(lane);
-  ring_load_bias(a.bias, BIAS_FLOATS);
-  __syncthreads();
-  NERF_STAMP2_LOOP();
-  PassQueue pq;
-  pq.init(a.queue, ws.lds0 + RING_BIAS_OFF);
-  for (int64_t sp = blockIdx.x; sp < nsuper;) {
-    int ln = lane;
-    asm volatile("" : "+v"(ln));
-    ws.new_pass();
-    tiles22<NS, MODE>(a, ws, sp * NW22 + wv, nwtiles, ln, pq);
-    NERF_STAMP2_PASS();
-    sp = pq.next(sp);
-  }
-  NERF_STAMP2_END();
-  ws.drain();
-  pq.leave();
-}
-
-int pack(const float* params, void* packed22, hipStream_t s) {
+int pack(const float* params, void* packed22, void* density22, hipStream_t s) {
   char* base = static_cast<char*>(packed22);
-  hipLaunchKernelGGL(pack22_kernel, dim3((PACK_THREADS + 255) / 256), dim3(256), 0, s, params,
-                     reinterpret_cast<u32x4*>(base), reinterpret_cast<float*>(base + (size_t)F_PADDED * 1024));
+  const int threads = PACK_THREADS + (density22 ? PACK_THREADS_D : 0);
+  hipLaunchKernelGGL(pack22_kernel, dim3((threads + 255) / 256), dim3(256), 0, s, params, reinterpret_cast<u32x4*>(base),
+                     reinterpret_cast<float*>(base + (size_t)F_PADDED * 1024), reinterpret_cast<u32x4*>(density22));
   return check_launch("nerf_mlp_pack (split-fp16 image)");
 }
 
@@ -435,20 +65,8 @@
 int forward(const void* packed22, const float* x, const float* rays, const float* z, int64_t M, int n, int freq_mode,
             float* out, int persistent_wgs, hipStream_t s) {
   FwdArgs a;
-  a.queue = passq_slot();
-  const char* base = static_cast<const char*>(packed22);
-  a.wf = reinterpret_cast<const bf16x8*>(base);
-  a.bias = reinterpret_cast<const float*>(base + (size_t)F_PADDED * 1024);
-  a.x = x; a.rays = rays; a.z = z; a.M = M; a.n = n; a.out = out; a.acts = nullptr; a.astride = 0;
-  for (int k = 0; k < 10; ++k) a.fr.pos[k] = freq_mode == 0 ? (float)(k * k) : (float)(1 << k);
-  for (int k = 0; k < 4; ++k) a.fr.dir[k] = freq_mode == 0 ? (float)(k * k) : (float)(1 << k);
-  int tiles = g_tiles;
-  if (tiles == 0) {
-    const int64_t w = persistent_wgs > 0 ? persistent_wgs : 1;
-    const int64_t p2 = (((M + 31) / 32 + NW22 - 1) / NW22 + w - 1) / w, p3 = (((M + 47) / 48 + NW22 - 1) / NW22 + w - 1) / w;
-    tiles = 100 * p2 < 141 * p3 ? 2 : 3;
-  }
-  const int mode = x ? 0 : (tiles == 3 ? 2 : 1);
+  fill_args(a, packed22, packed22, x, rays, z, M, n, freq_mode, out);
+  const int mode = x ? 0 : (pick_tiles(M, persistent_wgs) == 3 ? 2 : 1);
   const int ns = mode == 2 ? 3 : 2;
   const int64_t nsuper = ((M + 16 * ns - 1) / (16 * ns) + NW22 - 1) / NW22;
   const dim3 g((unsigned)(nsuper < persistent_wgs ? nsuper : persistent_wgs)), b(64 * NW22);
diff --git a/nerf_meets_mlx_amd/csrc/mlp22_dev.h b/nerf_meets_mlx_amd/csrc/mlp22_dev.h
--- /dev/null
+++ b/nerf_meets_mlx_amd/csrc/mlp22_dev.h
@@ -0,0 +1,428 @@
+#pragma once
+#include "mlp_layout.h"
+#include "mlp22.h"
+
+#ifndef NERF_F22_SINF
+#define NERF_F22_SINF 0
+#endif
+
+#ifndef NERF_F22_PIN
+#define NERF_F22_PIN 1
+#endif
+#ifndef NERF_F22_AGPR
+#define NERF_F22_AGPR 1
+#endif
+#ifndef NERF_F22_MIXSUB
+#define NERF_F22_MIXSUB 1
+#endif
+#ifndef NERF_F22_RG3
+#define NERF_F22_RG3 4
+#endif
+#ifndef NERF_F22_IGLP
+#define NERF_F22_IGLP 0
+#endif
+
+namespace nerf {
+namespace f22 {
+
+typedef _Float16 h8 __attribute__((ext_vector_type(8)));
+typedef _Float16 h2 __attribute__((ext_vector_type(2)));
+typedef float f32x2 __attribute__((ext_vector_type(2)));
+typedef unsigned int u32x4 __attribute__((ext_vector_type(4)));
+
+constexpr float LO_SCALE = 2048.0f, LO_INV = 1.0f / 2048.0f;
+constexpr float F16_MIN_NORMAL = 6.103515625e-05f;
+constexpr int CHUNKS = F_PADDED / RING_CHUNK;
+static_assert(CHUNKS * RING_CHUNK == F_PADDED && F_FRAGS % 4 == 0 && F_PAIRS == L::F16_TOTAL, "f22 stream layout");
+constexpr int D_CHUNKS = D_PADDED / RING_CHUNK;
+static_assert(D_PAIRS == L16::D_TOTAL && L16::D_ALPHA == L16::F_FA && L16::F_FA == L16::F_L7 + 128, "density stream = trunk L0 .. L7 + alpha head");
+static_assert(D_CHUNKS * RING_CHUNK == D_PADDED && (D_CHUNKS - 1) * RING_CHUNK < D_FRAGS && D_FRAGS <= D_PADDED && D_FRAGS % 4 == 0,
+              "density stream: whole ring chunks, the last one not empty, whole fragment groups");
+
+struct HiLo { unsigned hi, lo; };
+__device__ __forceinline__ HiLo split2(float v0, float v1) {
+  const f32x2 v = {v0, v1};
+  const h2 hh = __builtin_convertvector(v, h2);
+#if NERF_F22_MIXSUB
+  const f32x2 r = {__builtin_fmaf((float)hh[0], -LO_SCALE, v0 * LO_SCALE), __builtin_fmaf((float)hh[1], -LO_SCALE, v1 * LO_SCALE)};
+#else
+  const f32x2 r = {(v0 - (float)hh[0]) * LO_SCALE, (v1 - (float)hh[1]) * LO_SCALE};
+#endif
+  return HiLo{__builtin_bit_cast(unsigned, hh), __builtin_bit_cast(unsigned, __builtin_convertvector(r, h2))};
+}
+
+__device__ __forceinline__ float sin_acc(float x, float f, float ph) {
+  const float a = x * f;
+#if NERF_F22_SINF
+  return ph != 0.0f ? cosf(a) : sinf(a);
+#else
+  const float k = __builtin_rintf(a * 0.15915494309189535f);
+  float r = __builtin_fmaf(-k, 6.2831854820251465f, a);
+  r = __builtin_fmaf(-k, -1.7484556000744487e-07f, r);
+  return __builtin_amdgcn_sinf(__builtin_fmaf(r, 0.15915494309189535f, ph));
+#endif
+}
+
+struct Pe22 { float fa, fb, fc, phc, fd; int g; };
+__device__ __forceinline__ Pe22 pe22_setup(const PeFreq& fr, int g) {
+  Pe22 q;
+  q.fa = g == 0 ? fr.pos[0] : g == 1 ? fr.pos[2] : g == 2 ? fr.pos[4] : fr.pos[6];
+  q.fb = g == 0 ? fr.pos[1] : g == 1 ? fr.pos[3] : g == 2 ? fr.pos[5] : fr.pos[7];
+  q.fc = g < 2 ? fr.pos[8] : fr.pos[9];
+  q.phc = (g & 1) ? 0.25f : 0.0f;
+  q.fd = g == 0 ? fr.dir[0] : g == 1 ? fr.dir[1] : g == 2 ? fr.dir[2] : fr.dir[3];
+  q.g = g;
+  return q;
+}
+
+template <int COUNT>
+__device__ __forceinline__ void split_slots(const float (&v)[COUNT], u32x4* hi, u32x4* lo) {
+#pragma unroll
+  for (int j = 0; j < COUNT; j += 2) {
+    const HiLo q = split2(v[j], v[j + 1]);
+    hi[j >> 3][(j & 7) >> 1] = q.hi; lo[j >> 3][(j & 7) >> 1] = q.lo;
+  }
+}
+
+__device__ __forceinline__ void pe22_pos(const Pe22& q, const float (&p)[3], u32x4 (&peh)[2], u32x4 (&pel)[2]) {
+  float v[16];
+#pragma unroll
+  for (int sl = 0; sl < 12; ++sl) v[sl] = sin_acc(p[sl % 3], sl < 6 ? q.fa : q.fb, (sl % 6) >= 3 ? 0.25f : 0.0f);
+#pragma unroll
+  for (int k = 0; k < 3; ++k) v[12 + k] = sin_acc(p[k], q.fc, q.phc);
+  v[15] = q.g == 0 ? p[0] : q.g == 1 ? p[1] : q.g == 2 ? p[2] : 0.0f;
+  split_slots<16>(v, peh, pel);
+}
+__device__ __forceinline__ void pe22_dir(const Pe22& q, const float (&d)[3], u32x4 (&dph)[1], u32x4 (&dpl)[1]) {
+  float w[8];
+#pragma unroll
+  for (int j = 0; j < 6; ++j) w[j] = sin_acc(d[j % 3], q.fd, j >= 3 ? 0.25f : 0.0f);
+  w[6] = q.g == 0 ? d[0] : q.g == 1 ? d[1] : q.g == 2 ? d[2] : 0.0f;
+  w[7] = 0.0f;
+  split_slots<8>(w, dph, dpl);
+}
+__device__ __forceinline__ void pe22_encode(const Pe22& q, const float (&p)[3], const float (&d)[3], u32x4 (&peh)[2],
+                                            u32x4 (&pel)[2], u32x4 (&dph)[1], u32x4 (&dpl)[1]) {
+  pe22_pos(q, p, peh, pel);
+  pe22_dir(q, d, dph, dpl);
+}
+__device__ __forceinline__ void pe22_row(const float* __restrict__ row, int g, u32x4 (&peh)[2], u32x4 (&pel)[2],
+                                         u32x4 (&dph)[1], u32x4 (&dpl)[1]) {
+  float v[16], w[8];
+#pragma unroll
+  for (int sl = 0; sl < 16; ++sl) {
+    const int ch = pos_chan16(sl >> 3, g, sl & 7);
+    v[sl] = ch >= 0 ? row[ch] : 0.0f;
+  }
+#pragma unroll
+  for (int j = 0; j < 8; ++j) {
+    const int ch = dir_chan16(g, j);
+    w[j] = ch >= 0 ? row[63 + ch] : 0.0f;
+  }
+  split_slots<16>(v, peh, pel);
+  split_slots<8>(w, dph, dpl);
+}
+
+__device__ __forceinline__ f32x4 mfma16(const u32x4& a, const u32x4& b, const f32x4& c) {
+#if NERF_ABLATE == 41 || NERF_ABLATE == 42
+  return c;
+#endif
+  return __builtin_amdgcn_mfma_f32_16x16x32_f16(__builtin_bit_cast(h8, a), __builtin_bit_cast(h8, b), c, 0, 0, 0);
+}
+
+template <int NS, int KS, int NT, bool RELU, class WS, bool PARK_LDS = false>
+__device__ __forceinline__ void layer22(WS& ws, int pbase, int bias_slot, const u32x4 (&ih)[NS][KS], const u32x4 (&il)[NS][KS],
+                                        u32x4 (&oh)[NS][NT / 2], u32x4 (&ol)[NS][NT / 2], int lane, unsigned park_addr = 0u) {
+  const int g = lane >> 4;
+  f32x4 pm[NS], pc[NS];
+  if (PARK_LDS) asm volatile("ds_write_b128 %0, %1" :: "v"(park_addr), "v"(il[NS - 1][KS - 1]) : "memory");
+#if NERF_F22_IGLP >= 0
+  __builtin_amdgcn_iglp_opt(NERF_F22_IGLP);
+#endif
+  constexpr int NP = 2 * NS;
+  auto piece = [&](int nt, int pcs, f32x4 (&m)[NS], f32x4 (&c)[NS]) {
+    const int s = pcs >> 1, i = 2 * (pcs & 1);
+#if NERF_ABLATE == 41 || NERF_ABLATE == 42
+    return;
+#endif
+#if NERF_F22_PIN
+    if (pcs == 0) {
+#pragma unroll
+      for (int t = 0; t < NS; ++t) asm volatile("" : "+v"(m[t]), "+v"(c[t]));
+    }
+#endif
+    float v0 = __builtin_fmaf(c[s][i], LO_INV, m[s][i]), v1 = __builtin_fmaf(c[s][i + 1], LO_INV, m[s][i + 1]);
+    if (RELU) { v0 = __builtin_elementwise_maximum(v0, 0.0f); v1 = __builtin_elementwise_maximum(v1, 0.0f); }
+    const HiLo q = split2(v0, v1);
+    oh[s][nt >> 1][2 * (nt & 1) + (i >> 1)] = q.hi; ol[s][nt >> 1][2 * (nt & 1) + (i >> 1)] = q.lo;
+#if NERF_F22_AGPR
+    if ((nt & 1) && i == 2) asm volatile("" : "+a"(oh[s][nt >> 1]), "+a"(ol[s][nt >> 1]));
+#endif
+  };
+  auto piece_at = [](int q) { return NS == 2 ? (KS >= 8 ? 1 + 2 * q : (q * KS) / 4) : (KS >= 8 ? 1 + (q * (KS - 1)) / NP : (q * KS) / NP); };
+#pragma unroll
+  for (int nt = 0; nt < NT; ++nt) {
+    const float4 b = ws.bias4(bias_slot + 16 * nt + 4 * g);
+    f32x4 m[NS], c[NS];
+    m[0][0] = b.x; m[0][1] = b.y; m[0][2] = b.z; m[0][3] = b.w;
+    c[0] = f32x4{0.0f, 0.0f, 0.0f, 0.0f};
+#pragma unroll
+    for (int t = 1; t < NS; ++t) { m[t] = m[0]; c[t] = c[0]; }
+#pragma unroll
+    for (int ks = 0; ks < KS; ++ks) {
+      const int fp = pbase + nt * KS + ks;
+      const u32x4 ah = __builtin_bit_cast(u32x4, next_frag(ws, 2 * fp, lane));
+      const u32x4 al = __builtin_bit_cast(u32x4, next_frag(ws, 2 * fp + 1, lane));
+      if (NS == 2) {
+        m[0] = mfma16(ah, ih[0][ks], m[0]);
+        c[0] = mfma16(ah, il[0][ks], c[0]);
+        m[1] = mfma16(ah, ih[1][ks], m[1]);
+        c[1] = mfma16(ah, il[1][ks], c[1]);
+        c[0] = mfma16(al, ih[0][ks], c[0]);
+        c[1] = mfma16(al, ih[1][ks], c[1]);
+      } else {
+#pragma unroll
+        for (int t = 0; t < NS; ++t) {
+          m[t] = mfma16(ah, ih[t][ks], m[t]);
+          if (PARK_LDS && t == NS - 1 && ks == KS - 1) {
+            u32x4 b;
+            asm volatile("ds_read_b128 %0, %1\n\ts_waitcnt lgkmcnt(0)" : "=v"(b) : "v"(park_addr) : "memory");
+            c[t] = mfma16(ah, b, c[t]);
+          } else {
+            c[t] = mfma16(ah, il[t][ks], c[t]);
+          }
+        }
+#pragma unroll
+        for (int t = 0; t < NS; ++t) c[t] = mfma16(al, ih[t][ks], c[t]);
+      }
+      if (nt > 0) {
+#pragma unroll
+        for (int q = 0; q < NP; ++q)
+          if (piece_at(q) == ks) piece(nt - 1, q, pm, pc);
+      }
+    }
+#pragma unroll
+    for (int t = 0; t < NS; ++t) { pm[t] = m[t]; pc[t] = c[t]; }
+  }
+#pragma unroll
+  for (int q = 0; q < NP; ++q) piece(NT - 1, q, pm, pc);
+}
+
+template <int NS, int KS, class WS>
+__device__ __forceinline__ void head22(WS& ws, int pbase, int bias_slot, const u32x4 (&ih)[NS][KS], const u32x4 (&il)[NS][KS],
+                                       f32x4 (&out)[NS], int lane) {
+  const int g = lane >> 4;
+  const float4 b = ws.bias4(bias_slot + 4 * g);
+  f32x4 m[NS], c[NS];
+  m[0][0] = b.x; m[0][1] = b.y; m[0][2] = b.z; m[0][3] = b.w;
+  c[0] = f32x4{0.0f, 0.0f, 0.0f, 0.0f};
+#pragma unroll
+  for (int t = 1; t < NS; ++t) { m[t] = m[0]; c[t] = c[0]; }
+#pragma unroll
+  for (int ks = 0; ks < KS; ++ks) {
+    const u32x4 ah = __builtin_bit_cast(u32x4, next_frag(ws, 2 * (pbase + ks), lane));
+    const u32x4 al = __builtin_bit_cast(u32x4, next_frag(ws, 2 * (pbase + ks) + 1, lane));
+    if (NS == 2) {
+      m[0] = mfma16(ah, ih[0][ks], m[0]);
+      c[0] = mfma16(ah, il[0][ks], c[0]);
+      m[1] = mfma16(ah, ih[1][ks], m[1]);
+      c[1] = mfma16(ah, il[1][ks], c[1]);
+      c[0] = mfma16(al, ih[0][ks], c[0]);
+      c[1] = mfma16(al, ih[1][ks], c[1]);
+    } else {
+#pragma unroll
+      for (int t = 0; t < NS; ++t) { m[t] = mfma16(ah, ih[t][ks], m[t]); c[t] = mfma16(ah, il[t][ks], c[t]); }
+#pragma unroll
+      for (int t = 0; t < NS; ++t) c[t] = mfma16(al, ih[t][ks], c[t]);
+    }
+  }
+#pragma unroll
+  for (int s = 0; s < NS; ++s)
+#pragma unroll
+    for (int i = 0; i < 4; ++i) out[s][i] = __builtin_fmaf(c[s][i], LO_INV, m[s][i]);
+}
+
+constexpr int NW22 = 4, NW22_ = NW22;
+constexpr int PARK_OFF = RING_LDS_BYTES;
+template <int NS> constexpr int park_bytes() { return NS > 2 ? (6 * NS + 4) * 64 * NW22_ * 4 : 0; }
+template <int K> __device__ __forceinline__ void lds_put(unsigned addr, float v) {
+  asm volatile("ds_write_b32 %0, %1 offset:%2" :: "v"(addr), "v"(v), "i"(1024 * K) : "memory");
+}
+template <int K> __device__ __forceinline__ float lds_get(unsigned addr) {
+  float v;
+  asm volatile("ds_read_b32 %0, %1 offset:%2\n\ts_waitcnt lgkmcnt(0)" : "=v"(v) : "v"(addr), "i"(1024 * K) : "memory");
+  return v;
+}
+template <int S, bool DIR> __device__ __forceinline__ void park_put(unsigned park, const float (&p)[3], const float (&d)[3]) {
+  lds_put<6 * S + 0>(park, p[0]); lds_put<6 * S + 1>(park, p[1]); lds_put<6 * S + 2>(park, p[2]);
+  if (DIR) { lds_put<6 * S + 3>(park, d[0]); lds_put<6 * S + 4>(park, d[1]); lds_put<6 * S + 5>(park, d[2]); }
+}
+template <int S, int OFF> __device__ __forceinline__ void park_get(unsigned park, float (&v)[3]) {
+  v[0] = lds_get<6 * S + OFF>(park); v[1] = lds_get<6 * S + OFF + 1>(park); v[2] = lds_get<6 * S + OFF + 2>(park);
+}
+template <bool DIR> __device__ __forceinline__ void park_put_s(int s, unsigned park, const float (&p)[3], const float (&d)[3]) {
+  if (s == 0) park_put<0, DIR>(park, p, d); else if (s == 1) park_put<1, DIR>(park, p, d); else park_put<2, DIR>(park, p, d);
+}
+template <int OFF> __device__ __forceinline__ void park_get_s(int s, unsigned park, float (&v)[3]) {
+  if (s == 0) park_get<0, OFF>(park, v); else if (s == 1) park_get<1, OFF>(park, v); else park_get<2, OFF>(park, v);
+}
+
+template <int NS, int MODE, bool DENS, class WS>
+__device__ __forceinline__ void tiles22(const FwdArgs& a, WS& ws, int64_t wtile0, int64_t nwtiles, int lane, PassQueue& pq) {
+  constexpr bool RECOMP = NS > 2;
+  static_assert(!RECOMP || MODE == 1, "the 48-sample form takes rays + depths");
+  static_assert(!DENS || MODE == 1, "the density-only form takes rays + depths");
+  const int c = lane & 15, g = lane >> 4;
+  u32x4 peh[NS][2], pel[NS][2], dph[NS][1], dpl[NS][1];
+  const unsigned park = ws.lds0 + PARK_OFF + 4u * (unsigned)(ws.wv * 64 + lane);
+  pq.ask(ws.wv, lane);
+  const Pe22 q = pe22_setup(a.fr, g);
+  {
+    const int64_t wt = wtile0 < nwtiles ? wtile0 : nwtiles - 1;
+#pragma unroll
+    for (int s = 0; s < NS; ++s) {
+      int64_t m = wt * (16 * NS) + 16 * s + c; if (m >= a.M) m = a.M - 1;
+      if (MODE == 0) {
+        pe22_row(a.x + m * 90, g, peh[s], pel[s], dph[s], dpl[s]);
+      } else {
+        const int64_t ray = (int64_t)((unsigned)m / (unsigned)a.n);
+        const float* rr = a.rays + ray * NERF_RAY_STRIDE;
+        float p[3], d[3];
+#if NERF_ABLATE == 3
+        (void)rr;
+#pragma unroll
+        for (int k = 0; k < 3; ++k) { p[k] = 0.001f * (float)(m & 1023) + (float)k; d[k] = 0.5f; }
+#else
+        const float zv = a.z[m];
+#pragma unroll
+        for (int k = 0; k < 3; ++k) { p[k] = rr[k] + zv * rr[3 + k]; d[k] = rr[8 + k]; }
+#endif
+        if (RECOMP) {
+          park_put_s<!DENS>(s, park, p, d);
+          pe22_pos(q, p, peh[s], pel[s]);
+        } else if (DENS) {
+          pe22_pos(q, p, peh[s], pel[s]);
+        } else {
+          pe22_encode(q, p, d, peh[s], pel[s], dph[s], dpl[s]);
+        }
+      }
+    }
+  }
+  pq.publish(ws.wv);
+  u32x4 hah[NS][8], hal[NS][8], hbh[NS][8], hbl[NS][8];
+  layer22<NS, 2, 16, true>(ws, L16::F_L0, 0, peh, pel, hah, hal, lane);
+  layer22<NS, 8, 16, true>(ws, L16::F_L1 + 0 * 128, 256, hah, hal, hbh, hbl, lane);
+  layer22<NS, 8, 16, true>(ws, L16::F_L1 + 1 * 128, 512, hbh, hbl, hah, hal, lane);
+  layer22<NS, 8, 16, true>(ws, L16::F_L1 + 2 * 128, 768, hah, hal, hbh, hbl, lane);
+  layer22<NS, 8, 16, true>(ws, L16::F_L1 + 3 * 128, 1024, hbh, hbl, hah, hal, lane);
+  {
+    u32x4 cth[NS][10], ctl[NS][10];
+#pragma unroll
+    for (int s = 0; s < NS; ++s) {
+      if (RECOMP) {
+        float pp[3];
+        park_get_s<0>(s, park, pp);
+        pe22_pos(q, pp, peh[s], pel[s]);
+      }
+      cth[s][0] = peh[s][0]; cth[s][1] = peh[s][1]; ctl[s][0] = pel[s][0]; ctl[s][1] = pel[s][1];
+#pragma unroll
+      for (int k = 0; k < 8; ++k) { cth[s][2 + k] = hah[s][k]; ctl[s][2 + k] = hal[s][k]; }
+    }
+    layer22<NS, 10, 16, true, WS, (NS > 2)>(ws, L16::F_L5, 1280, cth, ctl, hbh, hbl, lane,
+                                            ws.lds0 + PARK_OFF + 6 * NS * 64 * NW22 * 4 + 16u * (unsigned)(ws.wv * 64 + lane));
+  }
+  layer22<NS, 8, 16, true>(ws, L16::F_L6, 1536, hbh, hbl, hah, hal, lane);
+  layer22<NS, 8, 16, true>(ws, L16::F_L7, 1792, hah, hal, hbh, hbl, lane);
+  if (DENS) {
+    f32x4 alpha[NS];
+    head22<NS, 8>(ws, L16::D_ALPHA, L::BI_ALPHA, hbh, hbl, alpha, lane);
+#pragma unroll
+    for (int s = 0; s < NS; ++s) {
+      const int64_t m = wtile0 * (16 * NS) + 16 * s + c;
+      if (g == 0 && wtile0 < nwtiles && m < a.M) {
+        float4 o; o.x = 0.0f; o.y = 0.0f; o.z = 0.0f; o.w = alpha[s][0];
+        *reinterpret_cast<float4*>(a.out + m * 4) = o;
+      }
+    }
+    return;
+  }
+  layer22<NS, 8, 16, false>(ws, L16::F_FA, L::BI_FEAT, hbh, hbl, hah, hal, lane);
+  f32x4 alpha[NS];
+  head22<NS, 8>(ws, L16::F_FA + 128, L::BI_ALPHA, hbh, hbl, alpha, lane);
+  u32x4 hdh[NS][4], hdl[NS][4];
+  {
+    u32x4 cth[NS][9], ctl[NS][9];
+#pragma unroll
+    for (int s = 0; s < NS; ++s) {
+#pragma unroll
+      for (int k = 0; k < 8; ++k) { cth[s][k] = hah[s][k]; ctl[s][k] = hal[s][k]; }
+      if (RECOMP) {
+        float dd[3];
+        park_get_s<3>(s, park, dd);
+        pe22_dir(q, dd, dph[s], dpl[s]);
+      }
+      cth[s][8] = dph[s][0]; ctl[s][8] = dpl[s][0];
+    }
+    layer22<NS, 9, 8, true>(ws, L16::F_DIR, L::BI_DIR, cth, ctl, hdh, hdl, lane);
+  }
+  f32x4 rgb[NS];
+  head22<NS, 4>(ws, L16::F_RGB, L::BI_RGB, hdh, hdl, rgb, lane);
+#pragma unroll
+  for (int s = 0; s < NS; ++s) {
+    const int64_t m = wtile0 * (16 * NS) + 16 * s + c;
+    if (g == 0 && wtile0 < nwtiles && m < a.M) {
+      float4 o; o.x = rgb[s][0]; o.y = rgb[s][1]; o.z = rgb[s][2]; o.w = alpha[s][0];
+      *reinterpret_cast<float4*>(a.out + m * 4) = o;
+    }
+  }
+}
+
+template <int MODE, int NS = 2, bool DENS = false>
+__global__ void __launch_bounds__(64 * NW22) mlp22_fwd_kernel(FwdArgs a) {
+  const int lane = threadIdx.x & 63;
+  const int wv = __builtin_amdgcn_readfirstlane(threadIdx.x >> 6);
+  const int64_t nwtiles = (a.M + 16 * NS - 1) / (16 * NS), nsuper = (nwtiles + NW22 - 1) / NW22;
+  NERF_STAMP2_DECL();
+  RingW<(DENS ? D_CHUNKS : CHUNKS), (DENS ? D_FRAGS : F_FRAGS), (NS > 2 ? NERF_F22_RG3 : 4), NW22, RING_CHUNK, RING_STAGES, true, true> ws;
+  ws.wsrc = reinterpret_cast<const char*>(a.wf);
+  ws.lane16 = 16 * lane;
+  ws.lds0 = __builtin_amdgcn_readfirstlane(lds_addr_of(ring_smem));
+  ws.wv = wv;
+  ws.start(lane);
+  ring_load_bias(a.bias, BIAS_FLOATS);
+  __syncthreads();
+  NERF_STAMP2_LOOP();
+  PassQueue pq;
+  pq.init(a.queue, ws.lds0 + RING_BIAS_OFF);
+  for (int64_t sp = blockIdx.x; sp < nsuper;) {
+    int ln = lane;
+    asm volatile("" : "+v"(ln));
+    ws.new_pass();
+    tiles22<NS, MODE, DENS>(a, ws, sp * NW22 + wv, nwtiles, ln, pq);
+    NERF_STAMP2_PASS();
+    sp = pq.next(sp);
+  }
+  NERF_STAMP2_END();
+  ws.drain();
+  pq.leave();
+}
+
+static inline void fill_args(FwdArgs& a, const void* wf, const void* packed22, const float* x, const float* rays, const float* z,
+                             int64_t M, int n, int freq_mode, float* out) {
+  a.queue = passq_slot();
+  a.wf = reinterpret_cast<const bf16x8*>(wf);
+  a.bias = reinterpret_cast<const float*>(static_cast<const char*>(packed22) + (size_t)F_PADDED * 1024);
+  a.x = x; a.rays = rays; a.z = z; a.M = M; a.n = n; a.out = out; a.acts = nullptr; a.astride = 0;
+  for (int k = 0; k < 10; ++k) a.fr.pos[k] = freq_mode == 0 ? (float)(k * k) : (float)(1 << k);
+  for (int k = 0; k < 4; ++k) a.fr.dir[k] = freq_mode == 0 ? (float)(k * k) : (float)(1 << k);
+}
+
+static inline int pick_tiles(int64_t M, int persistent_wgs) {
+  if (g_tiles != 0) return g_tiles;
+  const int64_t w = persistent_wgs > 0 ? persistent_wgs : 1;
+  const int64_t p2 = (((M + 31) / 32 + NW22 - 1) / NW22 + w - 1) / w, p3 = (((M + 47) / 48 + NW22 - 1) / NW22 + w - 1) / w;
+  return 100 * p2 < 141 * p3 ? 2 : 3;
+}
+
+}
+}
diff --git a/nerf_meets_mlx_amd/csrc/mlp22d.hip b/nerf_meets_mlx_amd/csrc/mlp22d.hip
--- /dev/null
+++ b/nerf_meets_mlx_amd/csrc/mlp22d.hip
@@ -0,0 +1,24 @@
+#include "mlp22_dev.h"
+
+namespace nerf {
+namespace f22 {
+
+int forward_density(const void* packed22, const void* density22, const float* rays, const float* z, int64_t M, int n,
+                    int freq_mode, float* out, int persistent_wgs, hipStream_t s) {
+  FwdArgs a;
+  fill_args(a, density22, packed22, nullptr, rays, z, M, n, freq_mode, out);
+  const int ns = pick_tiles(M, persistent_wgs);
+  const int64_t nsuper = ((M + 16 * ns - 1) / (16 * ns) + NW22 - 1) / NW22;
+  const dim3 g((unsigned)(nsuper < persistent_wgs ? nsuper : persistent_wgs)), b(64 * NW22);
+  static DevOnce once[2];
+  once[ns - 2].run([&] {
+    const void* k = ns == 2 ? reinterpret_cast<const void*>(mlp22_fwd_kernel<1, 2, true>) : reinterpret_cast<const void*>(mlp22_fwd_kernel<1, 3, true>);
+    (void)hipFuncSetAttribute(k, hipFuncAttributeMaxDynamicSharedMemorySize, RING_LDS_BYTES + park_bytes<3>());
+  });
+  if (ns == 2) hipLaunchKernelGGL((mlp22_fwd_kernel<1, 2, true>), g, b, RING_LDS_BYTES, s, a);
+  else hipLaunchKernelGGL((mlp22_fwd_kernel<1, 3, true>), g, b, RING_LDS_BYTES + park_bytes<3>(), s, a);
+  return check_launch("mlp density forward (split fp16)");
+}
+
+}
+}
diff --git a/nerf_meets_mlx_amd/csrc/mlp_layout.h b/nerf_meets_mlx_amd/csrc/mlp_layout.h
--- a/nerf_meets_mlx_amd/csrc/mlp_layout.h
+++ b/nerf_meets_mlx_amd/csrc/mlp_layout.h
@@ -27,6 +27,7 @@
 namespace L16 {
 constexpr int F_L0 = 0, F_L1 = 32, F_L5 = 544, F_L6 = 704, F_L7 = 832, F_FA = 960, F_DIR = 1096, F_RGB = 1168;
 constexpr int CHUNKS = L::F16_PADDED / RING_CHUNK;
+constexpr int D_ALPHA = 960, D_TOTAL = 968;
 }
 __host__ __device__ constexpr int kperm16(int ks, int g, int j) { return 32 * ks + 16 * (j >> 2) + 4 * g + (j & 3); }
 __host__ __device__ constexpr int pos_chan16(int ks, int g, int j) {
diff --git a/nerf_meets_mlx_amd/csrc/pipeline.hip b/nerf_meets_mlx_amd/csrc/pipeline.hip
--- a/nerf_meets_mlx_amd/csrc/pipeline.hip
+++ b/nerf_meets_mlx_amd/csrc/pipeline.hip
@@ -15,6 +15,15 @@
                                       int white_bkgd, void* workspace, float* rgb, float* disp, float* acc,
                                       float* rgb_coarse, float* disp_coarse, float* acc_coarse, float* z_vals,
                                       float* weights, void* stream) {
+  return nerf_render_rays_fused_density(arch, packed_coarse, packed_fine, nullptr, rays, B, n, N, u, freq_mode, white_bkgd, workspace,
+                                        rgb, disp, acc, rgb_coarse, disp_coarse, acc_coarse, z_vals, weights, stream);
+}
+
+extern "C" int nerf_render_rays_fused_density(const nerf_mlp_arch* arch, const void* packed_coarse, const void* packed_fine,
+                                              const void* density_coarse, const float* rays, int64_t B, int n, int N,
+                                              const float* u, int freq_mode, int white_bkgd, void* workspace, float* rgb,
+                                              float* disp, float* acc, float* rgb_coarse, float* disp_coarse, float* acc_coarse,
+                                              float* z_vals, float* weights, void* stream) {
   NERF_REQUIRE(B >= 0 && n >= 2 && N >= 0, NERF_E_SHAPE, "nerf_render_rays_fused: bad B/n/N");
   if (B == 0) return NERF_OK;
   NERF_REQUIRE(arch && packed_coarse && rays && workspace && rgb, NERF_E_NULL, "nerf_render_rays_fused: NULL pointer");
@@ -27,7 +36,9 @@
   float* rawf = zf + B * (n + N);
   int rc;
   if ((rc = nerf_sample_coarse(rays, B, n, 0, 0.0f, nullptr, z, stream))) return rc;
-  if ((rc = nerf_query_fused(arch, packed_coarse, rays, z, B, n, freq_mode, raw, nullptr, stream))) return rc;
+  if (density_coarse && N > 0 && !rgb_coarse) {
+    if ((rc = nerf_query_density(arch, packed_coarse, density_coarse, rays, z, B, n, freq_mode, raw, stream))) return rc;
+  } else if ((rc = nerf_query_fused(arch, packed_coarse, rays, z, B, n, freq_mode, raw, nullptr, stream))) return rc;
   float* rgb_c = N > 0 ? (rgb_coarse ? rgb_coarse : rgb) : rgb;
   if ((rc = nerf_composite_forward(raw, z, rays, B, n, 0.0f, nullptr, white_bkgd, rgb_c, N > 0 ? disp_coarse : disp,
                                    N > 0 ? acc_coarse : acc, w, nullptr, stream))) return rc;
diff --git a/nerf_meets_mlx_amd/engine/trainer.py b/nerf_meets_mlx_amd/engine/trainer.py
--- a/nerf_meets_mlx_amd/engine/trainer.py
+++ b/nerf_meets_mlx_amd/engine/trainer.py
@@ -104,7 +104,7 @@
         z = sampling.sample_coarse(rays, self.n)
         out = {"loss_coarse": self._step_net(self.coarse, rays, z, target, self.white_bkgd)}
         if self._fine is not None:
-            raw = self.coarse.query(rays, z, ref_quirks=self.q)
+            raw = self.coarse.query(rays, z, ref_quirks=self.q, density_only=True)
             _, _, _, weights, _ = render.composite(raw, z, rays, 0.0, self.white_bkgd)
             if u is None:
                 u = self.train_uniforms(rays.shape[0])
diff --git a/nerf_meets_mlx_amd/models/NeRF.py b/nerf_meets_mlx_amd/models/NeRF.py
--- a/nerf_meets_mlx_amd/models/NeRF.py
+++ b/nerf_meets_mlx_amd/models/NeRF.py
@@ -54,6 +54,8 @@
         self._packed = None
         self._dirty = True
         self._packed_version = -1
+        self._density = None
+        self._density_stale = True
         self._ws: Dict[str, torch.Tensor] = {}
         self.name: Optional[str] = None
         self._gen = 0
@@ -90,8 +92,14 @@
     def activation_generation(self) -> int:
         return self._acts_gen
 
-    def packed(self) -> torch.Tensor:
+    def wants_density(self) -> bool:
         lib = N.lib()
+        return lib.nerf_mlp_density_bytes(C.byref(self.arch)) > 0 and lib.nerf_get_option(b"density_requery") == 1
+
+    def packed(self, density: bool = False) -> torch.Tensor:
+        lib = N.lib()
+        if density and self._density is None:
+            self._density = torch.empty(lib.nerf_mlp_density_bytes(C.byref(self.arch)), dtype=torch.uint8, device=self.device)
         if self._packed is None:
             nbytes = lib.nerf_mlp_packed_bytes(C.byref(self.arch))
             if nbytes < 0:
@@ -99,8 +107,10 @@
                                  "n_layers=8, width=256, skips=[4] with in=63+27 + view head [precision 16, 22, 32], or in=40 without "
                                  "view head and out<=4 [16, 22, 32]; n_layers=2, width=64, skips=[] with in=32+16 + view head [16, 22])")
             self._packed = torch.empty(nbytes, dtype=torch.uint8, device=self.device)
-        if self._dirty or self.params._version != self._packed_version:
-            N.check(lib.nerf_mlp_pack(C.byref(self.arch), N.ptr(self.params), N.ptr(self._packed), N.stream()))
+        if self._dirty or self.params._version != self._packed_version or (density and self._density_stale):
+            N.check(lib.nerf_mlp_pack_density(C.byref(self.arch), N.ptr(self.params), N.ptr(self._packed),
+                                              N.ptr(self._density) if density else None, N.stream()))
+            self._density_stale = not density
             self._dirty = False
             self._packed_version = self.params._version
         return self._packed
@@ -131,9 +141,15 @@
 
     __call__ = forward
 
-    def query(self, rays: torch.Tensor, z: torch.Tensor, ref_quirks: bool = True, train: bool = False) -> torch.Tensor:
+    def query(self, rays: torch.Tensor, z: torch.Tensor, ref_quirks: bool = True, train: bool = False,
+              density_only: bool = False) -> torch.Tensor:
         B, n = z.shape
         raw = torch.empty(B, n, 4, dtype=torch.float32, device=z.device)
+        if density_only and not train and self.wants_density():
+            packed = self.packed(density=True)
+            N.check(N.lib().nerf_query_density(C.byref(self.arch), N.ptr(packed), N.ptr(self._density), N.ptr(rays), N.ptr(z), B, n,
+                                               0 if ref_quirks else 1, N.ptr(raw), N.stream()))
+            return raw
         acts = None
         if train:
             acts = self._begin_train_pass(B * n)
diff --git a/nerf_meets_mlx_amd/rendering/render.py b/nerf_meets_mlx_amd/rendering/render.py
--- a/nerf_meets_mlx_amd/rendering/render.py
+++ b/nerf_meets_mlx_amd/rendering/render.py
@@ -216,8 +216,11 @@
     fine = network_fine if network_fine else network_coarse
     if getattr(fine, "precision", 16) != getattr(network_coarse, "precision", 16):
         raise ValueError("render_rays_fused: coarse and fine networks must have the same precision (one nerf_mlp_arch per call)")
-    N.check(N.lib().nerf_render_rays_fused(
-        C.byref(network_coarse.arch), N.ptr(network_coarse.packed()), N.ptr(fine.packed()), N.ptr(rays), B, n, Nn,
+    density = (not with_coarse) and Nn > 0 and getattr(network_coarse, "wants_density", lambda: False)()
+    packed_coarse = network_coarse.packed(density=True) if density else network_coarse.packed()
+    N.check(N.lib().nerf_render_rays_fused_density(
+        C.byref(network_coarse.arch), N.ptr(packed_coarse), N.ptr(fine.packed()),
+        N.ptr(network_coarse._density) if density else None, N.ptr(rays), B, n, Nn,
         N.ptr(u) if Nn > 0 else None, 0 if ref_quirks else 1, int(bool(white_bkgd)), N.ptr(ws), N.ptr(rgb), N.ptr(disp),
         N.ptr(acc), N.ptr(ret.get("rgb_coarse")), N.ptr(ret.get("disp_coarse")), N.ptr(ret.get("acc_coarse")),
         N.ptr(ret.get("z_vals")), N.ptr(ret.get("weights")), N.stream()))
```
